# serycjon/MFT

Measured on AMD Instinct MI355X. Metric: tracked frames/sec at 512x512, 12 RAFT iters; flow EPE vs reference, higher is better.
Workload: dtype f32 (update-block products as split fp16 x 3 on the fp16 matrix cores, fp32 accumulation; error per product <= ~2^-23, see DESIGN.md section 4 and parity below); 1 GPU; MFT.track on synthetic 512x512 video, deltas [inf,1,2,4,8,16,32], 7/7.00/7 (min/mean/max) flow pairs per timed frame, 12 RAFT iters, seeded synthetic weights (BASELINE.json configs[1]); parallelism=single GPU, frames_resident_in_hbm=True, preroll_frames=32

## Files before the change

### include/mftx.h

```cpp
#ifndef MFTX_H
#define MFTX_H

#include <stddef.h>
#include <stdint.h>

#ifdef __cplusplus
extern "C" {
#endif

#define MFTX_VERSION 400

#define MFTX_E_ARG (-1)
#define MFTX_E_ALIGN (-2)
#define MFTX_E_WORKSPACE (-3)
#define MFTX_E_STATE (-4)

#define MFTX_MAX_CANDIDATES 16

int mftx_version(void);
const char *mftx_last_error_string(void);

#define MFTX_PROFILE_CATEGORIES 14
int mftx_profile_begin(void);
int mftx_profile_end(double *ms, double *work, long long *count, int n);
// ... 27 lines not shown
typedef struct mftx_conv_desc {
    const float *a0; int lda0; int c0;
    const float *a1; int lda1; int c1;
    const float *wpk; const float *bias;
    float *out; int ldo;
    int P, h, w;
    int N;
    int kh, kw;
    int act;
    float out_scale;
    const float *addend; int ld_addend;
    int stride, hin, win, pad_y, pad_x, residual_mode;
    int arith;
    int a_split, out_split;
} mftx_conv_desc;
#define MFTX_ARITH_F32 0
#define MFTX_ARITH_SPLIT 1
int mftx_conv2d(const mftx_conv_desc *d, void *stream);
int mftx_conv2d_tile(const mftx_conv_desc *d, int tile, void *stream);

int mftx_pack_tile_conv_weights(const float *wpk, int N, int taps, int cin, int cin_pad, void *wtile, void *stream);
int mftx_tile_conv2d(const mftx_conv_desc *d, const void *wtile, void *stream);
#define MFTX_OU_HEADS_WTILE_BYTES 6635520
int mftx_pack_ou_heads_weights(const float *w1pk, int cin_pad, const float *w2pk, void *wtile, void *wproj, void *stream);
int mftx_ou_heads(const float *a_split, int lda, int P, int h, int w, const void *wtile, const float *b1, const void *wproj, const float *b2,
                  float *T, float *out, int ld_out, void *stream);
int mftx_gru_half(const float *h_in, int ld_hin, const float *motion, int ld_mo, const void *wzr, const void *wq, const float *pre_zr,
                  const float *pre_q, float *z, const float *hf_in, float *hf_out, float *h_out, int ld_hout, int P, int h, int w, int pass,
                  void *stream);
int mftx_tile_conv_fills_chip(int P, int h, int w);
#define MFTX_FLOW_HEAD_WEIGHT_BYTES 32768
int mftx_pack_flow_head_weights(const float *w2pk, void *wproj, void *stream);
int mftx_flow_head(const float *hsplit, int ld_h, int P, int h, int w, const void *wtile, const float *b1, const void *wproj,
                   const float *b2, float *T, float *delta, float *coords, void *stream);
int mftx_split_weights(const float *wpk, void *out, long long n_floats, void *stream);
#define MFTX_SPLIT_LIMIT 65504.0f
int mftx_count_not_below(const float *x, long long n, float limit, unsigned *count, void *stream);

typedef struct mftx_raft mftx_raft;
#define MFTX_RAFT_NUM_WEIGHTS 34
int mftx_raft_create(const float *const *weights, int n_weights, mftx_raft **out);
void mftx_raft_destroy(mftx_raft *r);
size_t mftx_raft_workspace_bytes(int P, int h, int w);
int mftx_raft_set_ondemand(mftx_raft *r, int on);
int mftx_raft_set_split_weights(mftx_raft *r, const void *const *split, int n);
int mftx_raft_arith(const mftx_raft *r);
int mftx_raft_set_lookup_fused(mftx_raft *r, const void *wfused);
int mftx_raft_set_flow_fused(mftx_raft *r, const void *wflow);
int mftx_raft_set_tile_weights(mftx_raft *r, const void *const *tile, int n);
int mftx_raft_set_flow_head(mftx_raft *r, const void *wproj);
int mftx_raft_set_ou_heads(mftx_raft *r, const void *wtile, const void *wproj);
int mftx_raft_set_coords_trace(mftx_raft *r, float *trace);
#define MFTX_RAFT_OPT_FORK 0
#define MFTX_RAFT_OPT_PRESPLIT 1
#define MFTX_RAFT_OPT_GROUP 2
#define MFTX_RAFT_OPT_FUSE_LOOKUP 3
#define MFTX_RAFT_OPT_GRAPH 4
#define MFTX_RAFT_OPT_FUSE_FLOW 5
#define MFTX_RAFT_OPT_TILE_CONV 6
#define MFTX_RAFT_OPT_FUSE_HEAD 7
#define MFTX_RAFT_OPT_TILE_VOLUME 8
#define MFTX_RAFT_OPT_FUSE_GRU 9
#define MFTX_RAFT_OPT_TILE_CELLS 10
#define MFTX_RAFT_OPT_FUSE_OU 11
#define MFTX_RAFT_OPT_TILE_CONV2P 12
int mftx_raft_set_option(mftx_raft *r, int option, int value);
int mftx_raft_set_nonfinite_counter(mftx_raft *r, unsigned *counter);
int mftx_raft_clear_graphs(mftx_raft *r);
int mftx_raft_graph_stats(const mftx_raft *r, unsigned long long *captures, unsigned long long *replays);
size_t mftx_raft_workspace_bytes_for(const mftx_raft *r, int P, int h, int w);
int mftx_raft_workspace_layout(int P, int h, int w, size_t *offsets, int n);
int mftx_raft_workspace_layout_for(const mftx_raft *r, int P, int h, int w, size_t *offsets, int n);
int mftx_raft_refine(mftx_raft *r, int P, int h, int w, int iters,
                     const float *fmap1, const float *fmap2, const float *net, const float *inp,
                     const float *flow_init,
                     int pad_left, int pad_right, int pad_top, int pad_bottom,
                     float *flow, float *occl, float *sigma, float *packed, float *flow_lr,
                     void *workspace, size_t workspace_bytes, void *stream);
int mftx_raft_refine_gather(mftx_raft *r, int P, int h, int w, int iters, const float *const *fmap1,
                            const float *const *fmap2, const float *const *net, const float *const *inp,
                            const float *flow_init, int pad_left, int pad_right, int pad_top, int pad_bottom,
                            float *flow, float *occl, float *sigma, float *packed, float *flow_lr_out,
                            void *workspace, size_t workspace_bytes, void *stream);

typedef struct mftx_encoder mftx_encoder;
int mftx_encoder_create(const float *const *weights, int n_weights, int instance_norm, mftx_encoder **out);
int mftx_encoder_set_split_weights(mftx_encoder *e, const void *const *split, int n);
int mftx_encoder_set_graph(mftx_encoder *e, int on);
void mftx_encoder_destroy(mftx_encoder *e);
size_t mftx_encoder_workspace_bytes(int H0, int W0);
int mftx_encoder_forward(mftx_encoder *e, const uint8_t *img, int H0, int W0, float *out0, float *out1,
                         void *workspace, size_t workspace_bytes, void *stream);

int mftx_convex_upsample(const float *flow_lr, const float *ou, int ld_ou, const float *mask,
                         int P, int h, int w,
                         int pad_left, int pad_right, int pad_top, int pad_bottom,
                         float *flow, float *occl, float *sigma, float *packed, void *stream);

int mftx_chain(const float *flowL, const float *occlL, const float *sigmaL,
               const float *flowR, const float *occlR, const float *sigmaR,
               int H, int W, float *flowO, float *occlO, float *sigmaO, void *stream);

int mftx_warp_backward(const float *flow, const float *img, int C, int H, int W, float *out, void *stream);

int mftx_select(int K, const float *const *flow, const float *const *occl, const float *const *sigma,
                float thr, int H, int W,
                float *flowO, float *occlO, float *sigmaO, int8_t *chosen, void *stream);

int mftx_chain_select(int K,
                      const float *const *flowL, const float *const *occlL, const float *const *sigmaL,
                      const float *const *flowR, const float *const *occlR, const float *const *sigmaR,
                      float thr, int H, int W,
                      float *flowO, float *occlO, float *sigmaO, int8_t *chosen, void *stream);

int mftx_chain_select_packed(int K,
                             const float *const *flowL, const float *const *occlL, const float *const *sigmaL,
                             const float *const *packedR,
                             float thr, int H, int W,
                             float *flowO, float *occlO, float *sigmaO, int8_t *chosen, void *stream);

int mftx_chain_select_multi(int T, const int *K,
                            const float *const *flowL, const float *const *occlL, const float *const *sigmaL,
                            const float *const *packedR,
                            float thr, int H, int W,
                            float *const *flowO, float *const *occlO, float *const *sigmaO, int8_t *const *chosen,
                            void *stream);

int mftx_sample_points(int T, const float *const *flow, const float *const *occl, const float *const *sigma,
                       int H, int W, int N, const int *tmpl, const float *xy,
                       float *table, long long row_stride, int column, void *stream);

size_t mftx_quantize_workspace_bytes(void);
int mftx_quantize_u16(const float *x, long long n, uint16_t *q, float *lohi,
                      void *workspace, size_t workspace_bytes, void *stream);
int mftx_dequantize_u16(const uint16_t *q, long long n, float lo, float hi, float *x, void *stream);

int mftx_copy_bytes(const void *src, void *dst, long long n, void *stream);

int mftx_png_unfilter(uint8_t *rows, int height, int row_bytes, int bpp);

#ifdef __cplusplus
}
#endif
#endif
```

### mft_amd/_lib.py

```python
from __future__ import annotations

import ctypes as C
import os
from pathlib import Path

_HERE = Path(__file__).resolve().parent
LIB_PATH = _HERE / "libmftx.so"

MAX_CANDIDATES = 16
NUM_RAFT_WEIGHTS = 34
LOOKUP_CONVC1_WEIGHT_BYTES = 393216
FLOW_BRANCH_WEIGHT_BYTES = 352256
FLOW_HEAD_WEIGHT_BYTES = 32768
OU_HEADS_WTILE_BYTES = 6635520
SPLIT_LIMIT = 65504.0


class ConvDesc(C.Structure):
    _fields_ = [("a0", C.c_void_p), ("lda0", C.c_int), ("c0", C.c_int),
                ("a1", C.c_void_p), ("lda1", C.c_int), ("c1", C.c_int),
                ("wpk", C.c_void_p), ("bias", C.c_void_p),
                ("out", C.c_void_p), ("ldo", C.c_int),
                ("P", C.c_int), ("h", C.c_int), ("w", C.c_int),
                ("N", C.c_int), ("kh", C.c_int), ("kw", C.c_int),
                ("act", C.c_int), ("out_scale", C.c_float),
                ("addend", C.c_void_p), ("ld_addend", C.c_int),
                ("stride", C.c_int), ("hin", C.c_int), ("win", C.c_int), ("pad_y", C.c_int), ("pad_x", C.c_int),
                ("residual_mode", C.c_int), ("arith", C.c_int), ("a_split", C.c_int), ("out_split", C.c_int)]


_PP = C.POINTER(C.c_void_p)

SIGNATURES = {
    "mftx_version": (C.c_int, []),
    "mftx_last_error_string": (C.c_char_p, []),
    "mftx_profile_begin": (C.c_int, []),
    "mftx_profile_end": (C.c_int, [C.POINTER(C.c_double), C.POINTER(C.c_double), C.POINTER(C.c_longlong), C.c_int]),
    "mftx_corr_pyramid": (C.c_int, [C.c_void_p, C.c_void_p, C.c_int, C.c_int, C.c_int, C.c_int,
                                    C.c_void_p, C.c_void_p, C.c_void_p, C.c_void_p, C.c_void_p]),
    "mftx_corr_pyramid_split": (C.c_int, [C.c_void_p, C.c_void_p, C.c_int, C.c_int, C.c_int, C.c_int,
                                          C.c_void_p, C.c_void_p, C.c_void_p, C.c_void_p, C.c_void_p, C.c_void_p]),
    "mftx_corr_pyramid_layout": (C.c_int, [C.c_int, C.c_int, C.POINTER(C.c_longlong), C.POINTER(C.c_int)]),
    "mftx_corr_lookup": (C.c_int, [C.c_void_p] * 5 + [C.c_int] * 4 + [C.c_void_p, C.c_int, C.c_void_p]),
    "mftx_fmap_pyramid": (C.c_int, [C.c_void_p] + [C.c_int] * 4 + [C.c_void_p] * 4),
    "mftx_corr_lookup_ondemand": (C.c_int, [C.c_void_p] * 6 + [C.c_int] * 5 + [C.c_void_p, C.c_int, C.c_void_p]),
    "mftx_raft_set_ondemand": (C.c_int, [C.c_void_p, C.c_int]),
    "mftx_raft_workspace_bytes_for": (C.c_size_t, [C.c_void_p, C.c_int, C.c_int, C.c_int]),
    "mftx_conv2d": (C.c_int, [C.POINTER(ConvDesc), C.c_void_p]),
    "mftx_conv2d_tile": (C.c_int, [C.POINTER(ConvDesc), C.c_int, C.c_void_p]),
    "mftx_encoder_set_split_weights": (C.c_int, [C.c_void_p, _PP, C.c_int]),
    "mftx_raft_set_split_weights": (C.c_int, [C.c_void_p, _PP, C.c_int]),
    "mftx_raft_arith": (C.c_int, [C.c_void_p]),
    "mftx_raft_set_lookup_fused": (C.c_int, [C.c_void_p, C.c_void_p]),
    "mftx_raft_set_flow_fused": (C.c_int, [C.c_void_p, C.c_void_p]),
    "mftx_raft_set_tile_weights": (C.c_int, [C.c_void_p, _PP, C.c_int]),
    "mftx_raft_set_flow_head": (C.c_int, [C.c_void_p, C.c_void_p]),
    "mftx_raft_set_ou_heads": (C.c_int, [C.c_void_p, C.c_void_p, C.c_void_p]),
    "mftx_pack_ou_heads_weights": (C.c_int, [C.c_void_p, C.c_int, C.c_void_p, C.c_void_p, C.c_void_p, C.c_void_p]),
    "mftx_ou_heads": (C.c_int, [C.c_void_p, C.c_int, C.c_int, C.c_int, C.c_int, C.c_void_p, C.c_void_p, C.c_void_p, C.c_void_p, C.c_void_p,
                                C.c_void_p, C.c_int, C.c_void_p]),
    "mftx_pack_flow_head_weights": (C.c_int, [C.c_void_p, C.c_void_p, C.c_void_p]),
    "mftx_flow_head": (C.c_int, [C.c_void_p, C.c_int, C.c_int, C.c_int, C.c_int] + [C.c_void_p] * 8),
    "mftx_pack_tile_conv_weights": (C.c_int, [C.c_void_p, C.c_int, C.c_int, C.c_int, C.c_int, C.c_void_p, C.c_void_p]),
    "mftx_tile_conv2d": (C.c_int, [C.POINTER(ConvDesc), C.c_void_p, C.c_void_p]),
    "mftx_pack_flow_branch_weights": (C.c_int, [C.c_void_p, C.c_void_p, C.c_void_p, C.c_void_p]),
    "mftx_flow_branch": (C.c_int, [C.c_void_p, C.c_int, C.c_int, C.c_int, C.c_void_p, C.c_void_p, C.c_void_p, C.c_void_p,
                                   C.c_int, C.c_void_p, C.c_int, C.c_void_p]),
    "mftx_raft_set_option": (C.c_int, [C.c_void_p, C.c_int, C.c_int]),
    "mftx_raft_set_coords_trace": (C.c_int, [C.c_void_p, C.c_void_p]),
    "mftx_gru_half": (C.c_int, [C.c_void_p, C.c_int, C.c_void_p, C.c_int, C.c_void_p, C.c_void_p, C.c_void_p, C.c_void_p, C.c_void_p, C.c_void_p,
                                C.c_void_p, C.c_void_p, C.c_int, C.c_int, C.c_int, C.c_int, C.c_int, C.c_void_p]),
    "mftx_tile_conv_fills_chip": (C.c_int, [C.c_int, C.c_int, C.c_int]),
    "mftx_raft_clear_graphs": (C.c_int, [C.c_void_p]),
    "mftx_raft_set_nonfinite_counter": (C.c_int, [C.c_void_p, C.c_void_p]),
    "mftx_raft_graph_stats": (C.c_int, [C.c_void_p, C.POINTER(C.c_ulonglong), C.POINTER(C.c_ulonglong)]),
    "mftx_pack_lookup_convc1_weights": (C.c_int, [C.c_void_p, C.c_int, C.c_void_p, C.c_void_p]),
    "mftx_corr_lookup_convc1": (C.c_int, [C.c_void_p] * 5 + [C.c_int] * 3 + [C.c_void_p, C.c_void_p, C.c_void_p,
                                                                            C.c_int, C.c_int, C.c_void_p]),
    "mftx_split_weights": (C.c_int, [C.c_void_p, C.c_void_p, C.c_longlong, C.c_void_p]),
    "mftx_count_not_below": (C.c_int, [C.c_void_p, C.c_longlong, C.c_float, C.c_void_p, C.c_void_p]),
    "mftx_raft_create": (C.c_int, [_PP, C.c_int, C.POINTER(C.c_void_p)]),
    "mftx_raft_destroy": (None, [C.c_void_p]),
    "mftx_raft_workspace_bytes": (C.c_size_t, [C.c_int, C.c_int, C.c_int]),
    "mftx_raft_workspace_layout": (C.c_int, [C.c_int, C.c_int, C.c_int, C.POINTER(C.c_size_t), C.c_int]),
    "mftx_raft_workspace_layout_for": (C.c_int, [C.c_void_p, C.c_int, C.c_int, C.c_int, C.POINTER(C.c_size_t), C.c_int]),
    "mftx_raft_refine": (C.c_int, [C.c_void_p, C.c_int, C.c_int, C.c_int, C.c_int,
                                   C.c_void_p, C.c_void_p, C.c_void_p, C.c_void_p, C.c_void_p,
                                   C.c_int, C.c_int, C.c_int, C.c_int,
                                   C.c_void_p, C.c_void_p, C.c_void_p, C.c_void_p, C.c_void_p,
                                   C.c_void_p, C.c_size_t, C.c_void_p]),
    "mftx_raft_refine_gather": (C.c_int, [C.c_void_p, C.c_int, C.c_int, C.c_int, C.c_int,
                                          _PP, _PP, _PP, _PP, C.c_void_p,
                                          C.c_int, C.c_int, C.c_int, C.c_int,
                                          C.c_void_p, C.c_void_p, C.c_void_p, C.c_void_p, C.c_void_p,
                                          C.c_void_p, C.c_size_t, C.c_void_p]),
    "mftx_encoder_create": (C.c_int, [_PP, C.c_int, C.c_int, C.POINTER(C.c_void_p)]),
    "mftx_encoder_destroy": (None, [C.c_void_p]),
    "mftx_encoder_set_graph": (C.c_int, [C.c_void_p, C.c_int]),
    "mftx_encoder_workspace_bytes": (C.c_size_t, [C.c_int, C.c_int]),
    "mftx_encoder_forward": (C.c_int, [C.c_void_p, C.c_void_p, C.c_int, C.c_int, C.c_void_p, C.c_void_p,
                                       C.c_void_p, C.c_size_t, C.c_void_p]),
    "mftx_convex_upsample": (C.c_int, [C.c_void_p, C.c_void_p, C.c_int, C.c_void_p] + [C.c_int] * 7
                             + [C.c_void_p] * 5),
    "mftx_chain": (C.c_int, [C.c_void_p] * 6 + [C.c_int, C.c_int] + [C.c_void_p] * 4),
    "mftx_warp_backward": (C.c_int, [C.c_void_p, C.c_void_p, C.c_int, C.c_int, C.c_int, C.c_void_p, C.c_void_p]),
    "mftx_select": (C.c_int, [C.c_int, _PP, _PP, _PP, C.c_float, C.c_int, C.c_int] + [C.c_void_p] * 5),
    "mftx_chain_select": (C.c_int, [C.c_int] + [_PP] * 6 + [C.c_float, C.c_int, C.c_int] + [C.c_void_p] * 5),
    "mftx_chain_select_packed": (C.c_int, [C.c_int] + [_PP] * 4 + [C.c_float, C.c_int, C.c_int] + [C.c_void_p] * 5),
    "mftx_chain_select_multi": (C.c_int, [C.c_int, C.POINTER(C.c_int)] + [_PP] * 4 + [C.c_float, C.c_int, C.c_int] + [_PP] * 4
                                + [C.c_void_p]),
    "mftx_sample_points": (C.c_int, [C.c_int, _PP, _PP, _PP, C.c_int, C.c_int, C.c_int, C.c_void_p, C.c_void_p,
                                     C.c_void_p, C.c_longlong, C.c_int, C.c_void_p]),
    "mftx_quantize_workspace_bytes": (C.c_size_t, []),
    "mftx_quantize_u16": (C.c_int, [C.c_void_p, C.c_longlong, C.c_void_p, C.c_void_p, C.c_void_p, C.c_size_t, C.c_void_p]),
    "mftx_dequantize_u16": (C.c_int, [C.c_void_p, C.c_longlong, C.c_float, C.c_float, C.c_void_p, C.c_void_p]),
    "mftx_png_unfilter": (C.c_int, [C.c_void_p, C.c_int, C.c_int, C.c_int]),
    "mftx_copy_bytes": (C.c_int, [C.c_void_p, C.c_void_p, C.c_longlong, C.c_void_p]),
}

_lib = None


class MftxError(RuntimeError):
    pass


def load():
    global _lib
    if _lib is not None:
        return _lib
    path = Path(os.environ.get("MFTX_LIB", LIB_PATH))
    if not path.exists():
        raise MftxError(f"{path} not found: build it with `python -c 'import __graft_entry__ as g; g.build()'` "
                        "(there is no CPU fallback for the MFT hot path)")
    lib = C.CDLL(str(path))
    for name, (res, args) in SIGNATURES.items():
        fn = getattr(lib, name)
        fn.restype = res
        fn.argtypes = args
    _lib = lib
    return lib


def check(code, what):
    if code != 0:
        msg = load().mftx_last_error_string().decode(errors="replace")
        raise MftxError(f"{what} failed ({code}): {msg}")


def ptr_array(ptrs):
    arr = (C.c_void_p * len(ptrs))(*ptrs)
    return C.cast(arr, _PP), arr
```

### mft_amd/csrc/common.h

```cpp
#pragma once
#include <hip/hip_runtime.h>
#include <cstdarg>
#include <cstdio>
#include <cstdint>
#include <cstdlib>
#include "../../include/mftx.h"

namespace mftx {

void set_error(const char *fmt, ...);

inline int fail(int code, const char *fmt, ...) {
    char buf[512];
    va_list ap;
    va_start(ap, fmt);
    vsnprintf(buf, sizeof buf, fmt, ap);
    va_end(ap);
    set_error("%s", buf);
    return code;
}

inline int check_launch(const char *what) {
    hipError_t e = hipGetLastError();
    if (e != hipSuccess) {
// ... 9 lines not shown
    return e ? atoi(e) : dflt;
#else
    (void)name;
    return dflt;
#endif
}

inline bool aligned16(const void *p) { return (reinterpret_cast<uintptr_t>(p) & 15u) == 0; }
inline int cdiv(int a, int b) { return (a + b - 1) / b; }
inline int round_up(int a, int b) { return cdiv(a, b) * b; }

struct PyramidLayout {
    int h[4], w[4];
    int hb[2], wb[2];
    int sbh, sbw;
    long long stride[4];
};
inline PyramidLayout pyramid_layout(int h, int w) {
    PyramidLayout L;
    for (int l = 0; l < 4; ++l) { L.h[l] = h >> l; L.w[l] = w >> l; }
    L.sbh = (h + 7) / 8; L.sbw = (w + 15) / 16;
    L.hb[0] = 2 * L.sbh; L.wb[0] = 2 * L.sbw; L.hb[1] = L.sbh; L.wb[1] = L.sbw;
    L.stride[0] = (long long)L.hb[0] * L.wb[0] * 32;
    L.stride[1] = (long long)L.hb[1] * L.wb[1] * 32;
    L.stride[2] = ((long long)L.h[2] * L.w[2] + 3) / 4 * 4;
    L.stride[3] = ((long long)L.h[3] * L.w[3] + 3) / 4 * 4;
    return L;
}

__host__ __device__ inline int split_row_offset(int c) { return (c >> 3) * 32 + (c & 7) * 2; }
#ifdef __HIPCC__
__device__ __forceinline__ unsigned split_halves(float v) {
    const _Float16 h = (_Float16)v;
    const _Float16 l = (_Float16)((v - (float)h) * 2048.f);
    return (unsigned)__builtin_bit_cast(unsigned short, h) | ((unsigned)__builtin_bit_cast(unsigned short, l) << 16);
}
__device__ __forceinline__ void store_split_pairwise(float *row, int c, float v, bool store) {
    const unsigned mine = split_halves(v);
    const unsigned other = (unsigned)__shfl_xor((int)mine, 1);
    const bool odd = (c & 1) != 0;
    const unsigned word = odd ? ((other >> 16) | (mine & 0xffff0000u)) : ((mine & 0xffffu) | (other << 16));
    char *dst = reinterpret_cast<char *>(row) + split_row_offset(c & ~1) + (odd ? 16 : 0);
    if (store) *reinterpret_cast<unsigned *>(dst) = word;
}
__device__ __forceinline__ float4 load_split4(const float *row, int c) {
    const char *src = reinterpret_cast<const char *>(row) + split_row_offset(c);
    const uint2 h = *reinterpret_cast<const uint2 *>(src), l = *reinterpret_cast<const uint2 *>(src + 16);
    auto dec = [](unsigned hh, unsigned ll, int hi) {
        const _Float16 a = __builtin_bit_cast(_Float16, (unsigned short)(hi ? hh >> 16 : hh));
        const _Float16 b = __builtin_bit_cast(_Float16, (unsigned short)(hi ? ll >> 16 : ll));
        return (float)a + (float)b * (1.f / 2048.f);
    };
    return make_float4(dec(h.x, l.x, 0), dec(h.x, l.x, 1), dec(h.y, l.y, 0), dec(h.y, l.y, 1));
}
__device__ __forceinline__ void store_split4v(float *row, int c, float4 v) {
    const unsigned a = split_halves(v.x), b = split_halves(v.y), cc = split_halves(v.z), d = split_halves(v.w);
    char *dst = reinterpret_cast<char *>(row) + split_row_offset(c);
    *reinterpret_cast<uint2 *>(dst) = make_uint2((a & 0xffffu) | (b << 16), (cc & 0xffffu) | (d << 16));
    *reinterpret_cast<uint2 *>(dst + 16) = make_uint2((a >> 16) | (b & 0xffff0000u), (cc >> 16) | (d & 0xffff0000u));
}
#endif
__host__ __device__ inline float relu_keep_nan(float v) { return v < 0.f ? 0.f : v; }
int launch_conv(const mftx_conv_desc &d, hipStream_t s, int tile = -1);
int launch_conv_pair(const mftx_conv_desc &a, const mftx_conv_desc &b, hipStream_t s);
struct GruEpilogue {
    int mode;
    float *hx;
    int ld_hx;
    float *z;
    float *rh;
    float *hf = nullptr;
    int ld_hf = 0;
};
int launch_conv_gru(const mftx_conv_desc &d, const GruEpilogue &g, hipStream_t s);
int launch_split_weights(const float *wpk, void *out, long long n_floats, hipStream_t s);
bool conv_small_applicable(const mftx_conv_desc &d);
int launch_conv_small(const mftx_conv_desc &d, hipStream_t s, float *accum = nullptr, int ld_accum = 0);
int launch_corr_pyramid(const float *f1, const float *f2, int P, int C, int h, int w, float *const lvl[4], hipStream_t s,
                        float *f2_split = nullptr, int tile_resident = 1);
bool volume_tile_applicable(int C);
constexpr int MFTX_MAX_GATHER = 16;
struct PairPtrs { const float *p[MFTX_MAX_GATHER]; };
int launch_volume_tile(const float *f1, const float *f2s, int P, int h, int w, float *const lvl[4], hipStream_t s,
                       const PairPtrs *f1p = nullptr, long long f2_bstride = -1);
int launch_corr_lookup(const float *const lvl[4], const float *coords, int P, int h, int w,
                       float *out, int ld_out, hipStream_t s);
int launch_pack_lookup_convc1(const float *w, int ld_w, void *out, hipStream_t s);
bool lookup_convc1_applicable(int P, int h, int w, int ld_out);
int launch_lookup_convc1(const float *const lvl[4], const float *coords, int P, int h, int w, const void *wf,
                         const float *bias, float *out, int ld_out, int out_split, hipStream_t s);
int launch_pack_flow_branch(const float *w98, const float *w2pk, void *out, hipStream_t s);
int launch_flow_branch(const float *coords, int P, int h, int w, const void *wf, const float *b1, const float *b2, float *out,
                       int ld_out, float *hx, int ld_hx, hipStream_t s, const float *T = nullptr, const float *b2h = nullptr,
                       float *coords_out = nullptr, float *delta_out = nullptr);
struct TileConvLaunch {
    const float *a0; int lda0;
    const float *a1; int lda1;
    int cin;
    const void *wf;
    const float *bias;
    const float *addend; int ld_addend;
    float *out; int ldo; int out_split;
    float *z, *rh, *hf, *hx; int ld_hf, ld_hx;
    const void *wproj; float *tout;
    int P, h, w, N, kh, kw, epi;
    int cells;
};
struct GruHalfLaunch {
    const float *h_in; int ld_hin; const float *mo; int ld_mo;
    const void *wzr, *wq;
    const float *pre_zr, *pre_q;
    float *z; const float *hf_in; float *hf_out;
    float *h_out; int ld_hout;
    int P, h, w, pass;
    int cells;
};
int launch_gru_half(const GruHalfLaunch &d, hipStream_t s);
int launch_pack_flow_head(const float *w2pk, void *out, hipStream_t s);
int launch_pack_tile_conv2p(const float *wpk, int N, int cin_pad, void *out, hipStream_t s);
int launch_tile_conv2p(const float *a, int lda, const void *wf, const float *bias, float *out, int ldo, int n_valid, int P, int h, int w, int cells,
                       hipStream_t s);
constexpr size_t OU_HEAD_WTILE_BYTES = 8ull * 5 * 9 * 9 * 128 * 16, OU_HEAD_WPROJ_BYTES = 32768;
int launch_pack_ou_head(const float *w1pk, int cin_pad, const float *w2pk, void *wtile, void *wproj, hipStream_t s);
struct OuGather { const float *hx, *corr; int ld_corr; const float *coords1, *delta; float *flow_lr; };
int launch_ou_heads(const float *a, int lda, int P, int h, int w, const void *wtile, const float *b1, const void *wproj, const float *b2, float *T,
                    float *out, int ld_out, int cells, hipStream_t s, const OuGather *ga = nullptr);
int launch_flow_head_sum(const float *T, const float *b2, float *delta, const float *coords_in, float *coords_out, int P, int h, int w, hipStream_t s);
bool tile_conv_applicable(int kh, int kw, int cin, int N);
bool tile_conv_small_tiles_fill(int P, int h, int w);
bool tile_conv_fills_chip(int P, int h, int w, int kh, int kw);
int launch_pack_tile_conv(const float *wpk, int N, int taps, int cin, int cin_pad, void *out, hipStream_t s);
int launch_tile_conv(const TileConvLaunch &d, hipStream_t s);
int launch_fmap_pyramid(const float *f2, int P, int C, int h, int w, float *const lvl[3], hipStream_t s);
int launch_corr_ondemand(const float *f1, const float *const f2lvl[4], const float *coords, int P, int h, int w,
                         float *out, int ld_out, hipStream_t s);
int launch_convex_upsample(const float *flow_lr, const float *ou, int ld_ou, const float *mask,
                           int P, int h, int w, int pl, int pr, int pt, int pb,
                           float *flow, float *occl, float *sigma, float *packed, hipStream_t s, unsigned *nonfinite = nullptr);

}
```

### mft_amd/csrc/raft_engine.hip

```cpp
#include "common.h"
#include "profile.h"
#include "motion_front.h"
#include "graph_cache.h"
#include <cstdlib>
#include <new>

namespace mftx {


struct InitGather { int on; PairPtrs netp, inpp; };
__global__ void init_state_kernel(const float *__restrict__ net, const float *__restrict__ inp,
                                  const float *__restrict__ flow_init, float *hx, float *hf, float *coords1, int M, int h,
                                  int w, InitGather ga) {
    const long long i = (long long)blockIdx.x * blockDim.x + threadIdx.x;
    if (i >= (long long)M * 64) return;
    const int m = (int)(i >> 6), q = (int)(i & 63);
    if (ga.on) {
        const int b = m / (h * w);
        net = ga.netp.p[b] - (long long)b * h * w * 128;
        inp = ga.inpp.p[b] - (long long)b * h * w * 128;
    }
    const float4 v = (q < 32) ? reinterpret_cast<const float4 *>(net)[(long long)m * 32 + q]
                              : reinterpret_cast<const float4 *>(inp)[(long long)m * 32 + (q - 32)];
    if (hf != nullptr) {
        store_split4v(hx + (long long)m * 384, 4 * q, v);
        if (q < 32) reinterpret_cast<float4 *>(hf + (long long)m * 128)[q] = v;
    } else {
        reinterpret_cast<float4 *>(hx + (long long)m * 384)[q] = v;
    }
    if (q == 0) {
        const int rem = m % (h * w);
        float cx = (float)(rem % w), cy = (float)(rem / w);
        if (flow_init != nullptr) {
            cx += flow_init[2 * (long long)m];
            cy += flow_init[2 * (long long)m + 1];
        }
        coords1[2 * (long long)m] = cx;
        coords1[2 * (long long)m + 1] = cy;
    }
}

__global__ __launch_bounds__(256) void convf1_kernel(ConvF1Args q) {
    __shared__ __attribute__((aligned(16))) float patch[2][7][48];
    const int half = threadIdx.x >> 7;
    convf1_strip(q, blockIdx.x * 2 + half, patch[half], threadIdx.x & 127);
}

__global__ __launch_bounds__(256) void lookup_convf1_kernel(LookupArgs lp, ConvF1Args q, int lookup_blocks, int f1_blocks) {
    __shared__ __attribute__((aligned(16))) float patch[2][7][48];
    const int total = lookup_blocks + f1_blocks;
    const int b = blockIdx.x;
    const int f_lo = (int)((long long)b * f1_blocks / total), f_hi = (int)((long long)(b + 1) * f1_blocks / total);
    if (f_hi > f_lo) {
        const int half = threadIdx.x >> 7;
        convf1_strip(q, f_lo * 2 + half, patch[half], threadIdx.x & 127);
    } else {
        lookup_block_body<2>(lp, b - f_lo, lookup_blocks);
    }
}

__global__ void ou_gather_kernel(const float *__restrict__ hx, const float *__restrict__ corr, int ld_corr,
                                 const float *__restrict__ coords1, const float *__restrict__ delta,
                                 float *__restrict__ ouin, float *__restrict__ flow_lr, int M, int h, int w, int split) {
    const long long i = (long long)blockIdx.x * blockDim.x + threadIdx.x;
    if (i >= (long long)M * 178) return;
    const int m = (int)(i / 178), q = (int)(i - (long long)m * 178);
    float4 v;
    if (split) {
        if (q < 64) v = load_split4(hx + (long long)m * 384, 4 * q);
        else if (q < 145) v = reinterpret_cast<const float4 *>(corr + (long long)m * ld_corr)[q - 64];
        else if (q == 145) {
            const int rem = m % (h * w);
            const float fx = coords1[2 * (long long)m] - (float)(rem % w);
            const float fy = coords1[2 * (long long)m + 1] - (float)(rem / w);
            v = make_float4(fx, fy, delta[2 * (long long)m], delta[2 * (long long)m + 1]);
            flow_lr[2 * (long long)m] = fx;
            flow_lr[2 * (long long)m + 1] = fy;
        } else v = load_split4(hx + (long long)m * 384 + 256, 4 * (q - 146));
        store_split4v(ouin + (long long)m * 712, 4 * q, v);
        return;
    }
    if (q < 64) v = reinterpret_cast<const float4 *>(hx + (long long)m * 384)[q];
    else if (q < 145) v = reinterpret_cast<const float4 *>(corr + (long long)m * ld_corr)[q - 64];
    else if (q == 145) {
        const int rem = m % (h * w);
        const float fx = coords1[2 * (long long)m] - (float)(rem % w);
        const float fy = coords1[2 * (long long)m + 1] - (float)(rem / w);
        v = make_float4(fx, fy, delta[2 * (long long)m], delta[2 * (long long)m + 1]);
        flow_lr[2 * (long long)m] = fx;
        flow_lr[2 * (long long)m + 1] = fy;
    } else v = reinterpret_cast<const float4 *>(hx + (long long)m * 384 + 256)[q - 146];
    reinterpret_cast<float4 *>(ouin + (long long)m * 712)[q] = v;
}

enum WeightSlot {
    W_CONVC1, B_CONVC1, W_CONVC2, B_CONVC2, W_CONVF1, B_CONVF1, W_CONVF2, B_CONVF2, W_CONV, B_CONV,
    W_ZR1_DYN, W_ZR1_INP, B_ZR1, W_Q1_DYN, W_Q1_INP, B_Q1, W_ZR2_DYN, W_ZR2_INP, B_ZR2, W_Q2_DYN, W_Q2_INP, B_Q2,
    W_FH1, B_FH1, W_FH2, B_FH2, W_MASK0, B_MASK0, W_MASK2, B_MASK2,
    W_OU1, B_OU1, W_OU2, B_OU2, W_COUNT
};

struct Workspace {
    float *lvl[4];
    float *f2l[3];
    float *coords1, *corr, *cor1, *corflo, *flo1, *hx, *z, *rh, *fh, *delta, *mask, *ouin, *ouh, *ou, *flow_lr;
    float *pre_zr[2], *pre_q[2];
    float *f2s;
    float *hf;
    float *hb, *hfb;
    int ld_corr;
    size_t bytes;
};

static Workspace carve(void *base, int P, int h, int w, bool ondemand = false, bool split = false) {
    Workspace ws{};
    const size_t N = (size_t)h * w, M = (size_t)P * N;
    size_t off = 0;
    auto take = [&](size_t floats) {
        float *p = base ? reinterpret_cast<float *>(static_cast<char *>(base) + off) : nullptr;
        off += (floats * sizeof(float) + 255) & ~size_t(255);
        return p;
    };
    const PyramidLayout L = pyramid_layout(h, w);
    for (int l = 0; l < 4; ++l) ws.lvl[l] = take(ondemand ? 0 : M * (size_t)L.stride[l]);
    for (int l = 1; l < 4; ++l) ws.f2l[l - 1] = take(ondemand ? (size_t)P * (h >> l) * (w >> l) * 256 : 0);
    ws.coords1 = take(M * 2);
    ws.ld_corr = 324;
    ws.corr = take(M * ws.ld_corr);
    ws.cor1 = take(M * 256);
    ws.corflo = take(M * 256);
    ws.flo1 = take(M * 128);
    ws.hx = take(M * 384);
    ws.z = take(M * 128);
    ws.rh = take(M * 128);
    ws.fh = take(M * 256);
    ws.delta = take(M * 2);
    ws.mask = take(M * 576);
    ws.ouin = take(M * 712);
    ws.ouh = take(M * 256);
    ws.ou = take(M * 4);
    ws.flow_lr = take(M * 2);
    for (int pass = 0; pass < 2; ++pass) { ws.pre_zr[pass] = take(M * 256); ws.pre_q[pass] = take(M * 128); }
    ws.f2s = take(ondemand || !split ? 0 : M * 256);
    ws.hf = take(split ? M * 128 : 0);
    ws.hb = take(split ? M * 128 : 0);
    ws.hfb = take(split ? M * 128 : 0);
    ws.bytes = off;
    return ws;
}

}

using namespace mftx;

struct mftx_raft {
    uint32_t magic;
    int ondemand;
    int arith;
    const float *w[W_COUNT];
    const float *wg[W_COUNT];
    hipStream_t side;
    hipEvent_t ev_fork, ev_join;
    float *coords_trace;
    GraphCache *graphs;
    const void *wfused;
    const void *wflow;
    const void *wproj;
    const void *wt[W_COUNT];
    const void *wou, *wouproj;
    int opt[13];
    unsigned *nonfinite;
};
static constexpr int GEMM_SLOTS[] = {W_CONVC1, W_CONVC2, W_CONVF2, W_CONV, W_ZR1_DYN, W_ZR1_INP, W_Q1_DYN, W_Q1_INP,
                                     W_ZR2_DYN, W_ZR2_INP, W_Q2_DYN, W_Q2_INP, W_FH1, W_MASK0, W_MASK2, W_OU1};
static constexpr uint32_t RAFT_MAGIC = 0x4d465458;

extern "C" int mftx_raft_create(const float *const *weights, int n_weights, mftx_raft **out) {
    if (!weights || !out) return fail(MFTX_E_ARG, "raft_create: null pointer");
    if (n_weights != W_COUNT) return fail(MFTX_E_ARG, "raft_create: expected %d weight tensors, got %d", (int)W_COUNT, n_weights);
    for (int i = 0; i < W_COUNT; ++i) {
        if (!weights[i]) return fail(MFTX_E_ARG, "raft_create: weight %d is null", i);
        if (!aligned16(weights[i])) return fail(MFTX_E_ALIGN, "raft_create: weight %d not 16-byte aligned", i);
    }
    mftx_raft *r = new (std::nothrow) mftx_raft;
    if (!r) return fail(MFTX_E_ARG, "raft_create: out of host memory");
    r->magic = RAFT_MAGIC;
    r->ondemand = 0;
    r->arith = MFTX_ARITH_F32;
    r->side = nullptr; r->ev_fork = nullptr; r->ev_join = nullptr;
    r->wfused = nullptr;
    r->wflow = nullptr;
    r->wproj = nullptr;
    r->wou = nullptr; r->wouproj = nullptr;
    for (int i = 0; i < W_COUNT; ++i) r->wt[i] = nullptr;
    r->coords_trace = nullptr;
    r->nonfinite = nullptr;
    r->graphs = new (std::nothrow) GraphCache;
    r->opt[MFTX_RAFT_OPT_FORK] = -1; r->opt[MFTX_RAFT_OPT_PRESPLIT] = 1; r->opt[MFTX_RAFT_OPT_GROUP] = 1; r->opt[MFTX_RAFT_OPT_FUSE_LOOKUP] = 1; r->opt[MFTX_RAFT_OPT_GRAPH] = 1; r->opt[MFTX_RAFT_OPT_FUSE_FLOW] = 1; r->opt[MFTX_RAFT_OPT_TILE_CONV] = 1; r->opt[MFTX_RAFT_OPT_FUSE_HEAD] = 1; r->opt[MFTX_RAFT_OPT_TILE_VOLUME] = 1; r->opt[MFTX_RAFT_OPT_FUSE_GRU] = 1; r->opt[MFTX_RAFT_OPT_TILE_CELLS] = 0; r->opt[MFTX_RAFT_OPT_FUSE_OU] = 1; r->opt[MFTX_RAFT_OPT_TILE_CONV2P] = 1;
    for (int i = 0; i < W_COUNT; ++i) r->w[i] = r->wg[i] = weights[i];
    *out = r;
    return 0;
}

extern "C" void mftx_raft_destroy(mftx_raft *r) {
    if (r && r->magic == RAFT_MAGIC) {
        r->magic = 0;
        if (r->ev_fork) (void)hipEventDestroy(r->ev_fork);
        if (r->ev_join) (void)hipEventDestroy(r->ev_join);
        if (r->side) (void)hipStreamDestroy(r->side);
        delete r->graphs;
        delete r;
    }
}

static int ensure_side_stream(mftx_raft *r) {
    if (r->side) return 0;
    hipError_t e = hipStreamCreateWithFlags(&r->side, hipStreamNonBlocking);
    if (e == hipSuccess) e = hipEventCreateWithFlags(&r->ev_fork, hipEventDisableTiming);
    if (e == hipSuccess) e = hipEventCreateWithFlags(&r->ev_join, hipEventDisableTiming);
    if (e != hipSuccess) return fail((int)e, "raft_refine: side stream: %s", hipGetErrorString(e));
    return 0;
}

extern "C" size_t mftx_raft_workspace_bytes(int P, int h, int w) {
    if (P <= 0 || h <= 0 || w <= 0) return 0;
    return carve(nullptr, P, h, w).bytes;
}

extern "C" int mftx_raft_set_ondemand(mftx_raft *r, int on) {
// ... 52 lines not shown
    if (!r || r->magic != RAFT_MAGIC) return fail(MFTX_E_STATE, "raft_set_flow_head: bad handle");
    if (wproj && !aligned16(wproj)) return fail(MFTX_E_ALIGN, "raft_set_flow_head: weights not 16-byte aligned");
    r->wproj = wproj;
    if (r->graphs) r->graphs->clear();
    return 0;
}

extern "C" int mftx_raft_set_ou_heads(mftx_raft *r, const void *wtile, const void *wproj) {
    if (!r || r->magic != RAFT_MAGIC) return fail(MFTX_E_STATE, "raft_set_ou_heads: bad handle");
    if ((wtile == nullptr) != (wproj == nullptr)) return fail(MFTX_E_ARG, "raft_set_ou_heads: both weight streams, or neither");
    if (wtile && (!aligned16(wtile) || !aligned16(wproj))) return fail(MFTX_E_ALIGN, "raft_set_ou_heads: weights not 16-byte aligned");
    r->wou = wtile; r->wouproj = wproj;
    if (r->graphs) r->graphs->clear();
    return 0;
}

extern "C" int mftx_raft_set_coords_trace(mftx_raft *r, float *trace) {
    if (!r || r->magic != RAFT_MAGIC) return fail(MFTX_E_STATE, "raft_set_coords_trace: bad handle");
    r->coords_trace = trace;
    return 0;
}

extern "C" int mftx_raft_clear_graphs(mftx_raft *r) {
    if (!r || r->magic != RAFT_MAGIC) return fail(MFTX_E_STATE, "raft_clear_graphs: bad handle");
    if (r->graphs) r->graphs->clear();
    return 0;
}

extern "C" int mftx_raft_set_nonfinite_counter(mftx_raft *r, unsigned *counter) {
    if (!r || r->magic != RAFT_MAGIC) return fail(MFTX_E_STATE, "raft_set_nonfinite_counter: bad handle");
    if (counter && (reinterpret_cast<uintptr_t>(counter) & 3)) return fail(MFTX_E_ALIGN, "raft_set_nonfinite_counter: counter not 4-byte aligned");
    r->nonfinite = counter;
    return 0;
}

extern "C" int mftx_raft_set_option(mftx_raft *r, int option, int value) {
    if (!r || r->magic != RAFT_MAGIC) return fail(MFTX_E_STATE, "raft_set_option: bad handle");
    if (option < 0 || option > MFTX_RAFT_OPT_TILE_CONV2P) return fail(MFTX_E_ARG, "raft_set_option: unknown option %d", option);
    r->opt[option] = value;
    if (r->graphs) r->graphs->clear();
    return 0;
}

extern "C" int mftx_raft_arith(const mftx_raft *r) {
    return (r && r->magic == RAFT_MAGIC) ? r->arith : -1;
}

extern "C" size_t mftx_raft_workspace_bytes_for(const mftx_raft *r, int P, int h, int w) {
    if (!r || r->magic != RAFT_MAGIC || P <= 0 || h <= 0 || w <= 0) return 0;
    return carve(nullptr, P, h, w, r->ondemand != 0, r->arith == MFTX_ARITH_SPLIT).bytes;
}

static int workspace_layout(const mftx_raft *r, int P, int h, int w, size_t *offsets, int n) {
    if (P <= 0 || h <= 0 || w <= 0 || !offsets || n != 19) return fail(MFTX_E_ARG, "workspace_layout: need 19 slots");
    char *base = reinterpret_cast<char *>(uintptr_t(1) << 40);
    Workspace ws = carve(base, P, h, w, r && r->ondemand != 0, r && r->arith == MFTX_ARITH_SPLIT);
    float *ptrs[19] = {ws.lvl[0], ws.lvl[1], ws.lvl[2], ws.lvl[3], ws.coords1, ws.corr, ws.cor1, ws.corflo, ws.flo1,
                       ws.hx, ws.z, ws.rh, ws.fh, ws.delta, ws.mask, ws.ouin, ws.ouh, ws.ou, ws.flow_lr};
    for (int i = 0; i < 19; ++i) offsets[i] = (size_t)(reinterpret_cast<char *>(ptrs[i]) - base);
    return 0;
}
extern "C" int mftx_raft_workspace_layout(int P, int h, int w, size_t *offsets, int n) {
    return workspace_layout(nullptr, P, h, w, offsets, n);
}
extern "C" int mftx_raft_workspace_layout_for(const mftx_raft *r, int P, int h, int w, size_t *offsets, int n) {
    if (!r || r->magic != RAFT_MAGIC) return fail(MFTX_E_STATE, "workspace_layout_for: bad handle");
    return workspace_layout(r, P, h, w, offsets, n);
}

#define TRY(expr) do { int _e = (expr); if (_e) return _e; } while (0)

static mftx_conv_desc conv_desc(const float *a0, int lda0, int c0, const float *a1, int lda1, int c1,
                                const float *w, const float *b, float *out, int ldo, int P, int h, int wd, int N,
                                int kh, int kw, int act, float scale = 1.f, const float *addend = nullptr,
                                int ld_addend = 0) {
    mftx_conv_desc d{};
    d.addend = addend; d.ld_addend = ld_addend;
    d.a0 = a0; d.lda0 = lda0; d.c0 = c0; d.a1 = a1; d.lda1 = lda1; d.c1 = c1;
    d.wpk = w; d.bias = b; d.out = out; d.ldo = ldo; d.P = P; d.h = h; d.w = wd; d.N = N;
    d.kh = kh; d.kw = kw; d.act = act; d.out_scale = scale;
    return d;
}

struct RefineGather { PairPtrs f1, f2, net, inp; bool f2_shared; };
static int refine_impl(mftx_raft *r, int P, int h, int w, int iters, const float *fmap1,
                                const float *fmap2, const float *net, const float *inp, const float *flow_init,
                                int pad_left,
                                int pad_right, int pad_top, int pad_bottom, float *flow, float *occl,
                                float *sigma, float *packed, float *flow_lr_out, void *workspace,
                                size_t workspace_bytes, void *stream, const RefineGather *gather) {
    if (!r || r->magic != RAFT_MAGIC) return fail(MFTX_E_STATE, "raft_refine: bad handle");
    const bool planar = flow && occl && sigma;
    if (gather) { fmap1 = gather->f1.p[0]; fmap2 = gather->f2.p[0]; net = gather->net.p[0]; inp = gather->inp.p[0]; }
    if (!fmap1 || !fmap2 || !net || !inp || !workspace || (!planar && (flow || occl || sigma || !packed)))
        return fail(MFTX_E_ARG, "raft_refine: null pointer (outputs: flow + occl + sigma, or packed, or both)");
    if (P <= 0 || h < 16 || w < 16 || iters < 1)
        return fail(MFTX_E_ARG, "raft_refine: need P >= 1, h, w >= 16 (level 3 of the pyramid needs >= 2 cells), iters >= 1");
    if ((long long)P * h * w > (1ll << 24)) return fail(MFTX_E_ARG, "raft_refine: batch too large");
    if (!aligned16(fmap1) || !aligned16(fmap2) || !aligned16(net) || !aligned16(inp) ||
        (reinterpret_cast<uintptr_t>(workspace) & 255))
        return fail(MFTX_E_ALIGN, "raft_refine: inputs must be 16-byte and the workspace 256-byte aligned");
    if (pad_left < 0 || pad_right < 0 || pad_top < 0 || pad_bottom < 0 || pad_left + pad_right >= 8 ||
        pad_top + pad_bottom >= 8)
        return fail(MFTX_E_ARG, "raft_refine: bad padding");
    const bool ondemand = r->ondemand != 0;
    const bool SP = r->arith == MFTX_ARITH_SPLIT && r->opt[MFTX_RAFT_OPT_PRESPLIT] != 0;
    const bool fuse_lookup = SP && !ondemand && r->wfused != nullptr && r->opt[MFTX_RAFT_OPT_FUSE_LOOKUP] != 0 &&
                             lookup_convc1_applicable(P, h, w, 256);
    Workspace ws = carve(workspace, P, h, w, ondemand, r->arith == MFTX_ARITH_SPLIT);
    if (ws.bytes > workspace_bytes)
        return fail(MFTX_E_WORKSPACE, "raft_refine: workspace %zu < %zu bytes", workspace_bytes, ws.bytes);
    hipStream_t s = (hipStream_t)stream;
    const bool use_graph = r->graphs && r->opt[MFTX_RAFT_OPT_GRAPH] != 0 && !prof_enabled() && !r->coords_trace && !ondemand;
    hipStream_t caller = s;
    bool proxied = false;
    if (use_graph && s == nullptr) {
        hipStream_t own = r->graphs->proxy.enter(s);
        if (own) { s = own; proxied = true; }
    }
    struct Leave { GraphCache *g; hipStream_t caller; bool on; ~Leave() { if (on) g->proxy.leave(caller); } } leave{r->graphs, caller, proxied};
    const int N = h * w, M = P * N;
    const float *const *W = r->w;
    const float *const *G = r->wg;
    const int AR = r->arith;
    auto gemm = [AR, SP](mftx_conv_desc d, bool a = true, bool o = false) { d.arith = AR; d.a_split = SP && a; d.out_split = SP && o; return d; };

    const float *f2lv[4] = {fmap2, ws.f2l[0], ws.f2l[1], ws.f2l[2]};
    if (ondemand) TRY(launch_fmap_pyramid(fmap2, P, 256, h, w, ws.f2l, s));
    else if (gather) {
        const long long pair_floats = (long long)N * 256;
        if (gather->f2_shared) TRY(launch_split_weights(gather->f2.p[0], ws.f2s, pair_floats, s));
        else for (int b = 0; b < P; ++b) TRY(launch_split_weights(gather->f2.p[b], ws.f2s + b * pair_floats, pair_floats, s));
        TRY(launch_volume_tile(nullptr, ws.f2s, P, h, w, ws.lvl, s, &gather->f1, gather->f2_shared ? 0 : pair_floats));
    }
    else TRY(launch_corr_pyramid(fmap1, fmap2, P, 256, h, w, ws.lvl, s, r->arith == MFTX_ARITH_SPLIT ? ws.f2s : nullptr, r->opt[MFTX_RAFT_OPT_TILE_VOLUME]));
    {
        const long long slots = (long long)M * 64;
        ProfScope prof(PC_GLUE, s, 0);
        InitGather ga{};
        if (gather) { ga.on = 1; ga.netp = gather->net; ga.inpp = gather->inp; }
        hipLaunchKernelGGL(init_state_kernel, dim3((unsigned)((slots + 255) / 256)), dim3(256), 0, s, net, inp,
                           flow_init, ws.hx, SP ? ws.hf : nullptr, ws.coords1, M, h, w, ga);
        TRY(check_launch("init_state"));
    }
    float *flow_lr = flow_lr_out ? flow_lr_out : ws.flow_lr;
    auto core = [&]() -> int {
    const bool tiles_on = SP && r->opt[MFTX_RAFT_OPT_TILE_CONV] != 0 &&
                          (r->opt[MFTX_RAFT_OPT_TILE_CONV] == 2 ||
                           (tile_conv_fills_chip(P, h, w, 3, 3) && tile_conv_fills_chip(P, h, w, 1, 5) && tile_conv_fills_chip(P, h, w, 5, 1)));
    auto tile_w = [&](int slot) -> const void * { return tiles_on ? r->wt[slot] : nullptr; };
    auto tile_layer = [&](const float *a0, int lda0, const float *a1, int lda1, const void *wf, const float *bias, int N, int kh, int kw, int epi) {
        TileConvLaunch t{};
        t.a0 = a0; t.lda0 = lda0; t.a1 = a1; t.lda1 = lda1; t.cin = a1 ? 256 : 128; t.wf = wf; t.bias = bias;
        t.P = P; t.h = h; t.w = w; t.N = N; t.kh = kh; t.kw = kw; t.epi = epi;
        t.cells = r->opt[MFTX_RAFT_OPT_TILE_CELLS];
        return t;
    };
    for (int pass = 0; pass < 2; ++pass) {
        const int kh = pass ? 5 : 1, kw = pass ? 1 : 5;
        const int szr = pass ? W_ZR2_INP : W_ZR1_INP, sq = pass ? W_Q2_INP : W_Q1_INP;
        if (tile_w(szr)) {
            TileConvLaunch t = tile_layer(ws.hx + 128, 384, nullptr, 0, tile_w(szr), W[pass ? B_ZR2 : B_ZR1], 256, kh, kw, 0);
            t.out = ws.pre_zr[pass]; t.ldo = 256;
            TRY(launch_tile_conv(t, s));
        } else TRY(launch_conv(gemm(conv_desc(ws.hx + 128, 384, 128, nullptr, 0, 0, G[szr], W[pass ? B_ZR2 : B_ZR1], ws.pre_zr[pass], 256, P, h, w, 256, kh, kw, 0), true, false), s));
        if (tile_w(sq)) {
            TileConvLaunch t = tile_layer(ws.hx + 128, 384, nullptr, 0, tile_w(sq), W[pass ? B_Q2 : B_Q1], 128, kh, kw, 0);
            t.out = ws.pre_q[pass]; t.ldo = 128;
            TRY(launch_tile_conv(t, s));
        } else TRY(launch_conv(gemm(conv_desc(ws.hx + 128, 384, 128, nullptr, 0, 0, G[sq], W[pass ? B_Q2 : B_Q1], ws.pre_q[pass], 128, P, h, w, 128, kh, kw, 0), true, false), s));
    }
    const float *lv[4] = {ws.lvl[0], ws.lvl[1], ws.lvl[2], ws.lvl[3]};
    const int strips = cdiv(w, F1_CELLS);
    float *ccur = ws.coords1, *calt = ws.flo1;
    bool pending = false;
    for (int it = 0; it < iters; ++it) {
        const bool last = (it == iters - 1);
        if (r->coords_trace &&
            hipMemcpyAsync(r->coords_trace + (size_t)it * M * 2, ccur, (size_t)M * 8, hipMemcpyDeviceToDevice, s) != hipSuccess)
            return fail(MFTX_E_STATE, "raft_refine: coords trace copy failed");
        const ConvF1Args f1{ccur, W[W_CONVF1], W[B_CONVF1], ws.flo1, ws.hx, h, w, strips, P * h * strips, SP ? 1 : 0};
        const int f1_blocks = cdiv(f1.n_strips, 2);
        const bool nofuse = r->opt[MFTX_RAFT_OPT_GROUP] == 0, nopair = nofuse;
        const mftx_conv_desc c2 = gemm(conv_desc(ws.cor1, 256, 256, nullptr, 0, 0, G[W_CONVC2], W[B_CONVC2], ws.corflo, 256, P, h, w, 192, 3, 3, 1), true, true);
        const mftx_conv_desc f2 = gemm(conv_desc(ws.flo1, 128, 128, nullptr, 0, 0, G[W_CONVF2], W[B_CONVF2], ws.corflo + 192, 256, P, h, w, 64, 3, 3, 1), true, true);
        const int fork_env = r->opt[MFTX_RAFT_OPT_FORK];
        const bool fuse_flow = SP && r->wflow != nullptr && r->opt[MFTX_RAFT_OPT_FUSE_FLOW] != 0 && !nofuse;
        if (fuse_flow) {
            if (pending) {
                TRY(launch_flow_branch(ccur, P, h, w, r->wflow, W[B_CONVF1], W[B_CONVF2], ws.corflo + 192, 256, ws.hx, 384, s, ws.fh, W[B_FH2], calt, ws.delta));
                float *t = ccur; ccur = calt; calt = t;
                pending = false;
            } else TRY(launch_flow_branch(ccur, P, h, w, r->wflow, W[B_CONVF1], W[B_CONVF2], ws.corflo + 192, 256, ws.hx, 384, s));
        }
        const bool serial = fuse_flow || prof_enabled() || nofuse || (AR == MFTX_ARITH_SPLIT && (fork_env == 0 || fork_env == 2));
        const bool forked = !serial && AR == MFTX_ARITH_SPLIT;
        const bool flow_first = !fuse_flow && serial && fuse_lookup && fork_env == 2 && !prof_enabled() && !nofuse;
        if (flow_first) {
            hipLaunchKernelGGL(convf1_kernel, dim3(f1_blocks), dim3(256), 0, s, f1);
            TRY(check_launch("convf1"));
            TRY(launch_conv(f2, s));
        }
        if (forked) {
            TRY(ensure_side_stream(r));
            if (hipEventRecord(r->ev_fork, s) != hipSuccess || hipStreamWaitEvent(r->side, r->ev_fork, 0) != hipSuccess)
                return fail(MFTX_E_STATE, "raft_refine: fork onto the side stream failed");
            hipLaunchKernelGGL(convf1_kernel, dim3(f1_blocks), dim3(256), 0, r->side, f1);
            TRY(check_launch("convf1"));
            TRY(launch_conv(f2, r->side));
            if (fuse_lookup && last) TRY(launch_corr_lookup(lv, ccur, P, h, w, ws.corr, ws.ld_corr, r->side));
            if (hipEventRecord(r->ev_join, r->side) != hipSuccess) return fail(MFTX_E_STATE, "raft_refine: join event failed");
        }
        if (fuse_lookup) {
            if (last && !forked) TRY(launch_corr_lookup(lv, ccur, P, h, w, ws.corr, ws.ld_corr, s));
            TRY(launch_lookup_convc1(lv, ccur, P, h, w, r->wfused, W[B_CONVC1], ws.cor1, 256, 1, s));
            if (!forked && !flow_first && !fuse_flow) {
                ProfScope prof(PC_CONVF1, s, 2.0 * M * 128 * 98);
                hipLaunchKernelGGL(convf1_kernel, dim3(f1_blocks), dim3(256), 0, s, f1);
            }
        } else if (prof_enabled() || nofuse || forked || ondemand || fuse_flow) {
            if (ondemand) TRY(launch_corr_ondemand(fmap1, f2lv, ccur, P, h, w, ws.corr, ws.ld_corr, s));
            else TRY(launch_corr_lookup(lv, ccur, P, h, w, ws.corr, ws.ld_corr, s));
            if (!forked && !fuse_flow) {
                ProfScope prof(PC_CONVF1, s, 2.0 * M * 128 * 98);
                hipLaunchKernelGGL(convf1_kernel, dim3(f1_blocks), dim3(256), 0, s, f1);
            }
        } else {
            const LookupArgs la = make_lookup_args(lv, ccur, P, h, w, ws.corr, ws.ld_corr);
            const int lookup_blocks = cdiv(cdiv(la.cells, 2), LK_WAVES);
            hipLaunchKernelGGL(lookup_convf1_kernel, dim3(lookup_blocks + f1_blocks), dim3(256), 0, s, la, f1,
                               lookup_blocks, f1_blocks);
        }
        TRY(check_launch("lookup + convf1"));
        if (!fuse_lookup) TRY(launch_conv(gemm(conv_desc(ws.corr, ws.ld_corr, ws.ld_corr, nullptr, 0, 0, G[W_CONVC1], W[B_CONVC1], ws.cor1, 256, P, h, w, 256, 1, 1, 1), false, true), s));
        const bool two_pass = tiles_on && r->opt[MFTX_RAFT_OPT_TILE_CONV2P] != 0 && r->wt[W_CONVC2] && r->wt[W_CONV];
        auto run_c2 = [&]() -> int {
            if (two_pass) return launch_tile_conv2p(ws.cor1, 256, r->wt[W_CONVC2], W[B_CONVC2], ws.corflo, 256, 192, P, h, w, r->opt[MFTX_RAFT_OPT_TILE_CELLS], s);
            return launch_conv(c2, s);
        };
        if (forked) {
            TRY(run_c2());
            if (hipStreamWaitEvent(s, r->ev_join, 0) != hipSuccess) return fail(MFTX_E_STATE, "raft_refine: join failed");
        } else if (nopair || AR != MFTX_ARITH_F32) {
            TRY(run_c2());
            if (!flow_first && !fuse_flow) TRY(launch_conv(f2, s));
        } else {
            TRY(launch_conv_pair(c2, f2, s));
        }
        if (two_pass) TRY(launch_tile_conv2p(ws.corflo, 256, r->wt[W_CONV], W[B_CONV], ws.hx + 256, 384, 126, P, h, w, r->opt[MFTX_RAFT_OPT_TILE_CELLS], s));
        else TRY(launch_conv(gemm(conv_desc(ws.corflo, 256, 256, nullptr, 0, 0, G[W_CONV], W[B_CONV], ws.hx + 256, 384, P, h, w, 126, 3, 3, 1), true, true), s));
        const bool gru_fused = tile_w(W_ZR1_DYN) && tile_w(W_Q1_DYN) && tile_w(W_ZR2_DYN) && tile_w(W_Q2_DYN) &&
                               r->opt[MFTX_RAFT_OPT_FUSE_GRU] != 0;
        for (int pass = 0; pass < 2; ++pass) {
            const int kh = pass ? 5 : 1, kw = pass ? 1 : 5;
            const int szr = pass ? W_ZR2_DYN : W_ZR1_DYN, sq = pass ? W_Q2_DYN : W_Q1_DYN;
            if (gru_fused) {
                GruHalfLaunch g{};
                g.h_in = pass ? ws.hb : ws.hx; g.ld_hin = pass ? 128 : 384; g.h_out = pass ? ws.hx : ws.hb; g.ld_hout = pass ? 384 : 128;
                g.mo = ws.hx + 256; g.ld_mo = 384; g.wzr = tile_w(szr); g.wq = tile_w(sq); g.pre_zr = ws.pre_zr[pass]; g.pre_q = ws.pre_q[pass];
                g.z = ws.z; g.hf_in = pass ? ws.hfb : ws.hf; g.hf_out = pass ? ws.hf : ws.hfb; g.P = P; g.h = h; g.w = w; g.pass = pass; g.cells = r->opt[MFTX_RAFT_OPT_TILE_CELLS];
                TRY(launch_gru_half(g, s));
                continue;
            }
            if (tile_w(szr)) {
                TileConvLaunch t = tile_layer(ws.hx, 384, ws.hx + 256, 384, tile_w(szr), nullptr, 256, kh, kw, 2);
                t.addend = ws.pre_zr[pass]; t.ld_addend = 256; t.z = ws.z; t.rh = ws.rh; t.hf = ws.hf; t.ld_hf = 128;
                TRY(launch_tile_conv(t, s));
            } else {
                GruEpilogue g1{1, ws.hx, 384, ws.z, ws.rh, SP ? ws.hf : nullptr, 128};
                TRY(launch_conv_gru(gemm(conv_desc(ws.hx, 384, 128, ws.hx + 256, 384, 128, G[szr], nullptr, ws.z, 128, P, h, w, 256, kh, kw, 2, 1.f, ws.pre_zr[pass], 256), true, true), g1, s));
            }
            if (tile_w(sq)) {
                TileConvLaunch t = tile_layer(ws.rh, 128, ws.hx + 256, 384, tile_w(sq), nullptr, 128, kh, kw, 3);
                t.addend = ws.pre_q[pass]; t.ld_addend = 128; t.z = ws.z; t.hf = ws.hf; t.ld_hf = 128; t.hx = ws.hx; t.ld_hx = 384;
                TRY(launch_tile_conv(t, s));
            } else {
                GruEpilogue g2{2, ws.hx, 384, ws.z, ws.rh, SP ? ws.hf : nullptr, 128};
                TRY(launch_conv_gru(gemm(conv_desc(ws.rh, 128, 128, ws.hx + 256, 384, 128, G[sq], nullptr, ws.hx, 384, P, h, w, 128, kh, kw, 3, 1.f, ws.pre_q[pass], 128), true, true), g2, s));
            }
        }
        const bool head_fused = tile_w(W_FH1) && r->wproj != nullptr && r->opt[MFTX_RAFT_OPT_FUSE_HEAD] != 0;
        if (head_fused) {
            TileConvLaunch t = tile_layer(ws.hx, 384, nullptr, 0, tile_w(W_FH1), W[B_FH1], 256, 3, 3, 4);
            t.wproj = r->wproj; t.tout = ws.fh;
            TRY(launch_tile_conv(t, s));
            const bool defer = !last && fuse_flow && r->opt[MFTX_RAFT_OPT_FUSE_HEAD] != 2 && !r->coords_trace;
            if (defer) pending = true;
            else {
                float *dst = last ? ws.coords1 : ccur;
                TRY(launch_flow_head_sum(ws.fh, W[B_FH2], ws.delta, ccur, dst, P, h, w, s));
                ccur = dst;
            }
        } else if (tile_w(W_FH1)) {
            TileConvLaunch t = tile_layer(ws.hx, 384, nullptr, 0, tile_w(W_FH1), W[B_FH1], 256, 3, 3, 1);
            t.out = ws.fh; t.ldo = 256;
            TRY(launch_tile_conv(t, s));
        } else TRY(launch_conv(gemm(conv_desc(ws.hx, 384, 128, nullptr, 0, 0, G[W_FH1], W[B_FH1], ws.fh, 256, P, h, w, 256, 3, 3, 1), true, false), s));
        if (!head_fused) {
            const mftx_conv_desc fh2 = conv_desc(ws.fh, 256, 256, nullptr, 0, 0, W[W_FH2], W[B_FH2], ws.delta, 2, P, h, w, 2, 3, 3, 0);
            if (!conv_small_applicable(fh2)) return fail(MFTX_E_STATE, "raft_refine: flow-head layer does not fit the small-N kernel");
            TRY(launch_conv_small(fh2, s, ccur, 2));
        }
        if (!last) continue;
        if (r->coords_trace &&
            hipMemcpyAsync(r->coords_trace + (size_t)iters * M * 2, ccur, (size_t)M * 8, hipMemcpyDeviceToDevice, s) != hipSuccess)
            return fail(MFTX_E_STATE, "raft_refine: coords trace copy failed");
        if (tile_w(W_MASK0)) {
            TileConvLaunch t = tile_layer(ws.hx, 384, nullptr, 0, tile_w(W_MASK0), W[B_MASK0], 256, 3, 3, 1);
            t.out = ws.fh; t.ldo = 256; t.out_split = SP ? 1 : 0;
            TRY(launch_tile_conv(t, s));
        } else TRY(launch_conv(gemm(conv_desc(ws.hx, 384, 128, nullptr, 0, 0, G[W_MASK0], W[B_MASK0], ws.fh, 256, P, h, w, 256, 3, 3, 1), true, true), s));
        TRY(launch_conv(gemm(conv_desc(ws.fh, 256, 256, nullptr, 0, 0, G[W_MASK2], W[B_MASK2], ws.mask, 576, P, h, w, 576, 1, 1, 0, 0.25f), true, false), s));
        const bool ou_fused = tiles_on && r->wou != nullptr && r->opt[MFTX_RAFT_OPT_FUSE_OU] != 0;
        if (!ou_fused || r->opt[MFTX_RAFT_OPT_FUSE_OU] == 2) {
            const long long slots = (long long)M * 178;
            ProfScope prof(PC_GLUE, s, 0);
            hipLaunchKernelGGL(ou_gather_kernel, dim3((unsigned)((slots + 255) / 256)), dim3(256), 0, s, ws.hx,
                               ws.corr, ws.ld_corr, ccur, ws.delta, ws.ouin, flow_lr, M, h, w, SP ? 1 : 0);
            TRY(check_launch("ou_gather"));
        }
        if (ou_fused) {
            const OuGather ga{ws.hx, ws.corr, ws.ld_corr, ccur, ws.delta, flow_lr};
            const bool mat = r->opt[MFTX_RAFT_OPT_FUSE_OU] == 2;
            TRY(launch_ou_heads(mat ? ws.ouin : nullptr, 712, P, h, w, r->wou, W[B_OU1], r->wouproj, W[B_OU2], ws.ouh, ws.ou, 4, r->opt[MFTX_RAFT_OPT_TILE_CELLS], s,
                                mat ? nullptr : &ga));
        } else {
            TRY(launch_conv(gemm(conv_desc(ws.ouin, 712, 712, nullptr, 0, 0, G[W_OU1], W[B_OU1], ws.ouh, 256, P, h, w, 256, 3, 3, 1), true, false), s));
            TRY(launch_conv(conv_desc(ws.ouh, 256, 256, nullptr, 0, 0, W[W_OU2], W[B_OU2], ws.ou, 4, P, h, w, 3, 3, 3, 0), s));
        }
    }
    return 0;
    };
    if (use_graph) {
        if (AR == MFTX_ARITH_SPLIT && r->opt[MFTX_RAFT_OPT_FORK] != 0) TRY(ensure_side_stream(r));
        GraphKey key{};
        key.v[0] = (uintptr_t)P; key.v[1] = (uintptr_t)h; key.v[2] = (uintptr_t)w; key.v[3] = (uintptr_t)iters;
        key.v[4] = reinterpret_cast<uintptr_t>(workspace); key.v[5] = reinterpret_cast<uintptr_t>(flow_lr_out);
        key.v[6] = (uintptr_t)AR; key.v[7] = reinterpret_cast<uintptr_t>(r->wfused); key.v[8] = reinterpret_cast<uintptr_t>(s);
        key.v[9] = reinterpret_cast<uintptr_t>(r->wflow); key.v[10] = reinterpret_cast<uintptr_t>(r->wt[W_ZR1_DYN]); key.v[11] = reinterpret_cast<uintptr_t>(r->wproj);
        key.v[12] = reinterpret_cast<uintptr_t>(r->wou);
        TRY(r->graphs->run(key, s, core));
    } else {
        TRY(core());
    }
    return launch_convex_upsample(flow_lr, ws.ou, 4, ws.mask, P, h, w, pad_left, pad_right, pad_top, pad_bottom,
                                  flow, occl, sigma, packed, s, r->nonfinite);
}

extern "C" int mftx_raft_refine(mftx_raft *r, int P, int h, int w, int iters, const float *fmap1,
                                const float *fmap2, const float *net, const float *inp, const float *flow_init,
                                int pad_left, int pad_right, int pad_top, int pad_bottom, float *flow, float *occl,
                                float *sigma, float *packed, float *flow_lr_out, void *workspace,
                                size_t workspace_bytes, void *stream) {
    return refine_impl(r, P, h, w, iters, fmap1, fmap2, net, inp, flow_init, pad_left, pad_right, pad_top, pad_bottom, flow, occl, sigma,
                       packed, flow_lr_out, workspace, workspace_bytes, stream, nullptr);
}

extern "C" int mftx_raft_refine_gather(mftx_raft *r, int P, int h, int w, int iters, const float *const *fmap1,
                                       const float *const *fmap2, const float *const *net, const float *const *inp,
                                       const float *flow_init, int pad_left, int pad_right, int pad_top, int pad_bottom,
                                       float *flow, float *occl, float *sigma, float *packed, float *flow_lr_out,
                                       void *workspace, size_t workspace_bytes, void *stream) {
    if (!r || r->magic != RAFT_MAGIC) return fail(MFTX_E_STATE, "raft_refine_gather: bad handle");
    if (!fmap1 || !fmap2 || !net || !inp) return fail(MFTX_E_ARG, "raft_refine_gather: null pointer");
    if (P < 1 || P > MFTX_MAX_GATHER) return fail(MFTX_E_ARG, "raft_refine_gather: 1 .. %d pairs", MFTX_MAX_GATHER);
    if (r->arith != MFTX_ARITH_SPLIT || r->ondemand || r->opt[MFTX_RAFT_OPT_TILE_VOLUME] == 0)
        return fail(MFTX_E_STATE, "raft_refine_gather: needs the split arithmetic with the stored, tile-resident correlation volume (use mftx_raft_refine)");
    RefineGather g{};
    g.f2_shared = true;
    for (int b = 0; b < P; ++b) {
        if (!fmap1[b] || !fmap2[b] || !net[b] || !inp[b]) return fail(MFTX_E_ARG, "raft_refine_gather: pair %d has a null map", b);
        if (!aligned16(fmap1[b]) || !aligned16(fmap2[b]) || !aligned16(net[b]) || !aligned16(inp[b])) return fail(MFTX_E_ALIGN, "raft_refine_gather: maps must be 16-byte aligned");
        g.f1.p[b] = fmap1[b]; g.f2.p[b] = fmap2[b]; g.net.p[b] = net[b]; g.inp.p[b] = inp[b];
        if (fmap2[b] != fmap2[0]) g.f2_shared = false;
    }
    return refine_impl(r, P, h, w, iters, nullptr, nullptr, nullptr, nullptr, flow_init, pad_left, pad_right, pad_top, pad_bottom, flow, occl,
                       sigma, packed, flow_lr_out, workspace, workspace_bytes, stream, &g);
}

extern "C" int mftx_raft_graph_stats(const mftx_raft *r, unsigned long long *captures, unsigned long long *replays) {
    if (!r || r->magic != RAFT_MAGIC || !captures || !replays) return fail(MFTX_E_STATE, "raft_graph_stats: bad arguments");
    *captures = r->graphs ? r->graphs->captures : 0;
    *replays = r->graphs ? r->graphs->replays : 0;
    return 0;
}

extern "C" int mftx_corr_pyramid(const float *f1, const float *f2, int P, int C, int h, int w, float *lvl0,
                                 float *lvl1, float *lvl2, float *lvl3, void *stream) {
    if (!f1 || !f2 || !lvl0 || !lvl1 || !lvl2 || !lvl3) return fail(MFTX_E_ARG, "corr_pyramid: null pointer");
    if (P <= 0 || C <= 0 || C % 32 || h < 8 || w < 8) return fail(MFTX_E_ARG, "corr_pyramid: need C %% 32 == 0, h, w >= 8");
    if (!aligned16(f1) || !aligned16(f2)) return fail(MFTX_E_ALIGN, "corr_pyramid: features must be 16-byte aligned");
    if (!aligned16(lvl0) || !aligned16(lvl1) || !aligned16(lvl2) || !aligned16(lvl3))
        return fail(MFTX_E_ALIGN, "corr_pyramid: levels must be 16-byte aligned");
    float *const lv[4] = {lvl0, lvl1, lvl2, lvl3};
    return launch_corr_pyramid(f1, f2, P, C, h, w, lv, (hipStream_t)stream);
}

extern "C" int mftx_corr_pyramid_split(const float *f1, const float *f2, int P, int C, int h, int w, float *lvl0,
                                       float *lvl1, float *lvl2, float *lvl3, float *f2_scratch, void *stream) {
    if (!f1 || !f2 || !lvl0 || !lvl1 || !lvl2 || !lvl3 || !f2_scratch) return fail(MFTX_E_ARG, "corr_pyramid_split: null pointer");
    if (P <= 0 || C <= 0 || C % 32 || h < 8 || w < 8) return fail(MFTX_E_ARG, "corr_pyramid_split: need C %% 32 == 0, h, w >= 8");
    if (!aligned16(f1) || !aligned16(f2) || (reinterpret_cast<uintptr_t>(f2_scratch) & 31))
        return fail(MFTX_E_ALIGN, "corr_pyramid_split: features must be 16-byte aligned, the scratch 32-byte aligned");
    if (!aligned16(lvl0) || !aligned16(lvl1) || !aligned16(lvl2) || !aligned16(lvl3))
        return fail(MFTX_E_ALIGN, "corr_pyramid_split: levels must be 16-byte aligned");
    float *const lv[4] = {lvl0, lvl1, lvl2, lvl3};
    return launch_corr_pyramid(f1, f2, P, C, h, w, lv, (hipStream_t)stream, f2_scratch);
}

extern "C" int mftx_corr_pyramid_layout(int h, int w, long long *stride, int *block_grid) {
    if (h < 8 || w < 8 || !stride || !block_grid) return fail(MFTX_E_ARG, "corr_pyramid_layout: bad arguments");
    const PyramidLayout L = pyramid_layout(h, w);
    for (int l = 0; l < 4; ++l) stride[l] = L.stride[l];
    block_grid[0] = L.hb[0]; block_grid[1] = L.wb[0]; block_grid[2] = L.hb[1]; block_grid[3] = L.wb[1];
    return 0;
}

extern "C" int mftx_corr_lookup(const float *lvl0, const float *lvl1, const float *lvl2, const float *lvl3,
                                const float *coords, int P, int h, int w, int r, float *out, int ld_out,
                                void *stream) {
    if (!lvl0 || !lvl1 || !lvl2 || !lvl3 || !coords || !out) return fail(MFTX_E_ARG, "corr_lookup: null pointer");
    if (r != 4) return fail(MFTX_E_ARG, "corr_lookup: only radius 4 (RAFT basic) is built");
    if (P <= 0 || h < 8 || w < 8 || ld_out < 324) return fail(MFTX_E_ARG, "corr_lookup: bad sizes");
    if (!aligned16(lvl0) || !aligned16(lvl1)) return fail(MFTX_E_ALIGN, "corr_lookup: levels 0 and 1 must be 16-byte aligned");
    const float *lv[4] = {lvl0, lvl1, lvl2, lvl3};
    return launch_corr_lookup(lv, coords, P, h, w, out, ld_out, (hipStream_t)stream);
}

extern "C" int mftx_pack_lookup_convc1_weights(const float *wpk, int ld_w, void *wfused, void *stream) {
    if (!wpk || !wfused) return fail(MFTX_E_ARG, "pack_lookup_convc1_weights: null pointer");
    if (ld_w < 324) return fail(MFTX_E_ARG, "pack_lookup_convc1_weights: need ld_w >= 324");
    if (!aligned16(wfused)) return fail(MFTX_E_ALIGN, "pack_lookup_convc1_weights: output must be 16-byte aligned");
    return launch_pack_lookup_convc1(wpk, ld_w, wfused, (hipStream_t)stream);
}

extern "C" int mftx_corr_lookup_convc1(const float *lvl0, const float *lvl1, const float *lvl2, const float *lvl3,
                                       const float *coords, int P, int h, int w, const void *wfused, const float *bias,
                                       float *out, int ld_out, int out_split, void *stream) {
    if (!lvl0 || !lvl1 || !lvl2 || !lvl3 || !coords || !wfused || !bias || !out) return fail(MFTX_E_ARG, "corr_lookup_convc1: null pointer");
    if (P <= 0 || h < 8 || w < 8 || ld_out < 256 || ld_out % 4) return fail(MFTX_E_ARG, "corr_lookup_convc1: bad sizes");
    if (!lookup_convc1_applicable(P, h, w, ld_out)) return fail(MFTX_E_ARG, "corr_lookup_convc1: batch too large");
    if (!aligned16(wfused) || !aligned16(bias) || !aligned16(out) || !aligned16(coords) ||
        (out_split && (ld_out % 8 || (reinterpret_cast<uintptr_t>(out) & 31))))
        return fail(MFTX_E_ALIGN, "corr_lookup_convc1: operands must be 16-byte aligned (a split-form output: 32-byte rows)");
    const float *lv[4] = {lvl0, lvl1, lvl2, lvl3};
    return launch_lookup_convc1(lv, coords, P, h, w, wfused, bias, out, ld_out, out_split ? 1 : 0, (hipStream_t)stream);
}

extern "C" int mftx_pack_tile_conv_weights(const float *wpk, int N, int taps, int cin, int cin_pad, void *wtile, void *stream) {
    if (taps == 9 && cin == 256) return launch_pack_tile_conv2p(wpk, N, cin_pad, wtile, (hipStream_t)stream);
    return launch_pack_tile_conv(wpk, N, taps, cin, cin_pad, wtile, (hipStream_t)stream);
}

extern "C" int mftx_tile_conv2d(const mftx_conv_desc *d, const void *wtile, void *stream) {
    if (!d || !wtile) return fail(MFTX_E_ARG, "tile_conv2d: null pointer");
    if (d->arith != MFTX_ARITH_SPLIT || !d->a_split) return fail(MFTX_E_ARG, "tile_conv2d: split arithmetic with a split-form input only");
    if (d->act != 0 && d->act != 1) return fail(MFTX_E_ARG, "tile_conv2d: activation none or relu");
    if (d->stride > 1 || d->residual_mode != 0 || d->out_scale != 1.f || (d->hin && d->hin != d->h) || (d->win && d->win != d->w) || d->pad_y != 0 || d->pad_x != 0)
        return fail(MFTX_E_ARG, "tile_conv2d: stride 1, same padding, no output scale");
    if (d->kh == 3 && d->kw == 3 && d->c0 == 256 && d->c1 == 0) {
// ... 108 lines not shown
```

### mft_amd/csrc/tile_conv.hip

```cpp
#include "common.h"
#include "profile.h"

namespace mftx {

typedef float tc_f32x16 __attribute__((ext_vector_type(16)));
typedef float tc_f32x4 __attribute__((ext_vector_type(4)));
typedef unsigned tc_u32x4 __attribute__((ext_vector_type(4)));
typedef _Float16 tc_f16x8 __attribute__((ext_vector_type(8)));

enum TcEpi { TC_LINEAR = 0, TC_RELU = 1, TC_GRU_ZR = 2, TC_GRU_Q = 3,
             TC_RELU_PROJ = 4 };

#ifdef MFTX_LF_TRACE
__device__ unsigned long long tc_trace_buf[8][16];
#define TC_T(code) do { if (blockIdx.x == 0 && tcount < 16) { unsigned long long t_; asm volatile("s_memtime %0\n\ts_waitcnt lgkmcnt(0)" : "=s"(t_) :: "memory"); \
                        if ((threadIdx.x & 63) == 0) tc_trace_buf[threadIdx.x >> 6][tcount] = ((unsigned long long)(code) << 56) | (t_ & 0x00ffffffffffffffull); ++tcount; } } while (0)
__device__ unsigned long long tc_clock_buf[4096][4];
#define TC_CLK(slot) do { if (wv == ((slot) ? 7 : 0) && blockIdx.x < 4096) { unsigned long long t_, r_; \
                          asm volatile("s_waitcnt vmcnt(0) lgkmcnt(0)\n\ts_memtime %0\n\ts_memrealtime %1\n\ts_waitcnt lgkmcnt(0)" : "=s"(t_), "=s"(r_) :: "memory"); \
                          if (lane == 0) { tc_clock_buf[blockIdx.x][slot] = t_; tc_clock_buf[blockIdx.x][2 + slot] = r_; } } } while (0)
#else
#define TC_T(code) do { } while (0)
#define TC_CLK(slot) do { } while (0)
#endif
// ... 260 lines not shown
    }

    constexpr int GPC = N / 8, ITEMS = G::CELLS * GPC;
#pragma unroll
    for (int it = 0; it < ITEMS / 512; ++it) {
        const int item = tid + 512 * it, m = item / GPC, n0 = (item % GPC) * 8;
        const int yy = y0 + m / TW, xx = x0 + m % TW;
        const float *src = red + m * G::RED_ROW + n0;
        tc_f32x4 u = *reinterpret_cast<const tc_f32x4 *>(src), v = *reinterpret_cast<const tc_f32x4 *>(src + 4);
        if constexpr (G::KS == 2) {
            u += *reinterpret_cast<const tc_f32x4 *>(src + G::CELLS * G::RED_ROW);
            v += *reinterpret_cast<const tc_f32x4 *>(src + G::CELLS * G::RED_ROW + 4);
        }
        if (yy >= p.h || xx >= p.w) continue;
        const long long cell = img_base + (long long)yy * p.w + xx;
        if (p.bias) {
            u += *reinterpret_cast<const tc_f32x4 *>(p.bias + n0);
            v += *reinterpret_cast<const tc_f32x4 *>(p.bias + n0 + 4);
        }
        if (p.addend) {
            u += *reinterpret_cast<const tc_f32x4 *>(p.addend + cell * p.ld_addend + n0);
            v += *reinterpret_cast<const tc_f32x4 *>(p.addend + cell * p.ld_addend + n0 + 4);
        }
        auto store_split = [&](float *row, int c0) {
            tc_u32x4 hi, lo;
            tc_split8(u, v, k2048, hi, lo);
            uint4 *dst = reinterpret_cast<uint4 *>(reinterpret_cast<char *>(row) + (c0 >> 3) * 32);
            dst[0] = __builtin_bit_cast(uint4, hi);
            dst[1] = __builtin_bit_cast(uint4, lo);
        };
        if constexpr (EPI == TC_GRU_ZR) {
#pragma unroll
            for (int e = 0; e < 4; ++e) { u[e] = tc_sigmoid(u[e]); v[e] = tc_sigmoid(v[e]); }
            if (n0 < 128) {
                *reinterpret_cast<tc_f32x4 *>(p.z + cell * 128 + n0) = u;
                *reinterpret_cast<tc_f32x4 *>(p.z + cell * 128 + n0 + 4) = v;
            } else {
                u *= *reinterpret_cast<const tc_f32x4 *>(p.hf + cell * p.ld_hf + n0 - 128);
                v *= *reinterpret_cast<const tc_f32x4 *>(p.hf + cell * p.ld_hf + n0 - 128 + 4);
                store_split(p.rh + cell * 128, n0 - 128);
            }
        } else if constexpr (EPI == TC_GRU_Q) {
            const tc_f32x4 z0 = *reinterpret_cast<const tc_f32x4 *>(p.z + cell * 128 + n0), z1 = *reinterpret_cast<const tc_f32x4 *>(p.z + cell * 128 + n0 + 4);
            float *hrow = p.hf + cell * p.ld_hf + n0;
            const tc_f32x4 h0 = *reinterpret_cast<const tc_f32x4 *>(hrow), h1 = *reinterpret_cast<const tc_f32x4 *>(hrow + 4);
#pragma unroll
            for (int e = 0; e < 4; ++e) { u[e] = tc_blend(z0[e], h0[e], tc_tanh(u[e])); v[e] = tc_blend(z1[e], h1[e], tc_tanh(v[e])); }
            *reinterpret_cast<tc_f32x4 *>(hrow) = u;
            *reinterpret_cast<tc_f32x4 *>(hrow + 4) = v;
            store_split(p.hx + cell * p.ld_hx, n0);
        } else {
            if constexpr (EPI == TC_RELU) {
#pragma unroll
                for (int e = 0; e < 4; ++e) { u[e] = relu_keep_nan(u[e]); v[e] = relu_keep_nan(v[e]); }
            }
            if (p.out_split) store_split(p.out + cell * p.ldo, n0);
            else {
                *reinterpret_cast<tc_f32x4 *>(p.out + cell * p.ldo + n0) = u;
                *reinterpret_cast<tc_f32x4 *>(p.out + cell * p.ldo + n0 + 4) = v;
            }
        }
    }
    TC_T(8);
    TC_CLK(1);
}

#ifdef MFTX_LF_TRACE
extern "C" int mftx_debug_tc_clock(unsigned long long *out, int n_wg) {
    if (n_wg < 0 || n_wg > 4096) return -1;
    return hipMemcpyFromSymbol(out, HIP_SYMBOL(tc_clock_buf), sizeof(unsigned long long) * 4 * n_wg) == hipSuccess ? 0 : -1;
}
extern "C" int mftx_debug_tc_trace(unsigned long long *out) {
    if (hipMemcpyFromSymbol(out, HIP_SYMBOL(tc_trace_buf), sizeof(unsigned long long) * 8 * 16) != hipSuccess) return -1;
    unsigned long long z[8 * 16] = {};
    return hipMemcpyToSymbol(HIP_SYMBOL(tc_trace_buf), z, sizeof z) == hipSuccess ? 0 : -1;
}
#endif

struct GruHalfArgs {
    const float *h_in; int ld_hin;
    const float *mo; int ld_mo;
    const void *wzr, *wq;
    const float *pre_zr, *pre_q;
    float *z;
    const float *hf_in; float *hf_out;
    float *h_out; int ld_hout;
    int P, h, w, tiles_x, tiles_y, step;
};

template <class G, int KW>
__device__ __forceinline__ void tc_kloop(const unsigned char *const (&abase)[G::RT], const uint4 *__restrict__ w2, uint4 (&bq)[3][2],
                                         tc_f32x16 (&acc)[G::RT], tc_f32x16 (&accx)[G::RT]) {
    constexpr int PF = 3;
    tc_f16x8 ah[2][G::RT], al[2][G::RT];
    auto read_a = [&](int s, int set) {
        const int tap = s / G::GPW, gg = s % G::GPW;
        const int off = ((tap / KW) * G::HWD + tap % KW) * G::CELLB + gg * 64 * G::KS;
#pragma unroll
        for (int i = 0; i < G::RT; ++i) {
            ah[set][i] = *reinterpret_cast<const tc_f16x8 *>(abase[i] + off);
            al[set][i] = *reinterpret_cast<const tc_f16x8 *>(abase[i] + off + 16);
        }
    };
    read_a(0, 0);
#pragma unroll
    for (int s = 0; s < G::STEPS; ++s) {
        const int set = s & 1;
        const tc_f16x8 bh = __builtin_bit_cast(tc_f16x8, bq[s % PF][0]), bl = __builtin_bit_cast(tc_f16x8, bq[s % PF][1]);
        __builtin_amdgcn_sched_barrier(0);
        if (s + 1 < G::STEPS) read_a(s + 1, set ^ 1);
        if (s + PF < G::STEPS) { bq[s % PF][0] = w2[(s + PF) * 128]; bq[s % PF][1] = w2[(s + PF) * 128 + 64]; }
        __builtin_amdgcn_sched_barrier(0);
#pragma unroll
        for (int i = 0; i < G::RT; ++i) acc[i] = tc_mfma(bh, ah[set][i], acc[i]);
#pragma unroll
        for (int i = 0; i < G::RT; ++i) accx[i] = tc_mfma(bl, ah[set][i], accx[i]);
#pragma unroll
        for (int i = 0; i < G::RT; ++i) accx[i] = tc_mfma(bh, al[set][i], accx[i]);
        __builtin_amdgcn_sched_barrier(0);
    }
}

template <int TH, int TW, int KH, int KW>
__global__ __launch_bounds__(512, 2) void gru_half_kernel(GruHalfArgs p) {
    using G1 = TcGeom<TH, TW, KH, KW, 256, 256>;
    using G2 = TcGeom<TH, TW, KH, KW, 256, 128>;
    static_assert(G1::CELLB == G2::CELLB && G1::HWD == G2::HWD, "one tile, two GEMMs");
    constexpr int CELLB = G1::CELLB, HWD = G1::HWD, PF = 3, RT = G1::RT, CELLS = G1::CELLS;
    constexpr bool HORIZ = KW > 1;
    extern __shared__ __attribute__((aligned(16))) unsigned char tc_lds[];
    unsigned char *lds = tc_lds;
    const int tid = (int)threadIdx.x, lane = tid & 63, wv = __builtin_amdgcn_readfirstlane(tid >> 6);
    const int tile = (int)blockIdx.x;
    const int tx_ = tile % p.tiles_x, ty_ = (tile / p.tiles_x) % p.tiles_y, img = tile / (p.tiles_x * p.tiles_y);
    const int n_along = HORIZ ? p.tiles_x : p.tiles_y, t_along = HORIZ ? tx_ : ty_, len_along = HORIZ ? p.w : p.h;
    const int r0 = n_along > 1 ? t_along * p.step - 2 : 0;
    const int olo = n_along > 1 ? t_along * p.step : 0, ohi = n_along > 1 ? min(len_along, olo + p.step) : len_along;
    const int x0 = HORIZ ? r0 : tx_ * TW, y0 = HORIZ ? ty_ * TH : r0;
    const long long img_base = (long long)img * p.h * p.w;
    const uint4 *__restrict__ w1 = reinterpret_cast<const uint4 *>(p.wzr) + (long long)((wv ^ 4) * G1::STEPS) * 128 + lane;
    const int nt2 = wv % G2::NT, ks2 = wv / G2::NT;
    const uint4 *__restrict__ w2 = reinterpret_cast<const uint4 *>(p.wq) + (long long)((nt2 * G2::KS + ks2) * G2::STEPS) * 128 + lane;

#ifdef MFTX_LF_TRACE
    int tcount = 0;
#endif
    TC_T(1);
    TC_CLK(0);
    uint4 bq[PF][2];
#pragma unroll
    for (int s = 0; s < PF; ++s) { bq[s][0] = w1[s * 128]; bq[s][1] = w1[s * 128 + 64]; }

    {
        constexpr int PPC = 64, TOTAL = G1::HCELLS * PPC, ROUNDS = (TOTAL + 511) / 512, B = 6;
#pragma unroll 1
        for (int rr = 0; rr < ROUNDS; rr += B) {
            uint4 v[B];
#pragma unroll
            for (int k = 0; k < B; ++k) {
                const int q = (rr + k) * 512 + tid;
                v[k] = make_uint4(0u, 0u, 0u, 0u);
                if (rr + k < ROUNDS && q < TOTAL) {
                    const int c = q / PPC, pc = q - c * PPC;
                    const int cy = c / HWD, cx = c - cy * HWD;
                    const int yy = y0 - KH / 2 + cy, xx = x0 - KW / 2 + cx;
                    if (yy >= 0 && yy < p.h && xx >= 0 && xx < p.w) {
                        const long long cell = img_base + (long long)yy * p.w + xx;
                        const float *src = pc >= 32 ? p.mo + cell * p.ld_mo + (pc - 32) * 4 : p.h_in + cell * p.ld_hin + pc * 4;
                        v[k] = *reinterpret_cast<const uint4 *>(src);
                    }
                }
            }
#pragma unroll
            for (int k = 0; k < B; ++k) {
                const int q = (rr + k) * 512 + tid;
                if (rr + k < ROUNDS && q < TOTAL) {
                    const int c = q / PPC, pc = q - c * PPC;
                    *reinterpret_cast<uint4 *>(lds + c * CELLB + pc * 16) = v[k];
                }
            }
        }
    }
    TC_T(2);
    tc_barrier();
    TC_T(3);

    tc_f32x16 acc[RT], accx[RT];
    const unsigned char *abase[RT];
    auto zero_acc = [&]() {
#pragma unroll
        for (int i = 0; i < RT; ++i)
#pragma unroll
            for (int r = 0; r < 16; ++r) { acc[i][r] = 0.f; accx[i][r] = 0.f; }
    };
    auto set_abase = [&](int ks) {
        const int r = lane & 31;
#pragma unroll
        for (int i = 0; i < RT; ++i) {
            const int m = 32 * i + r;
            abase[i] = lds + ((m / TW) * HWD + (m % TW)) * CELLB + (lane >> 5) * 32 + ks * 64;
        }
    };
    auto slot = [&](int m) { return lds + ((m / TW + KH / 2) * HWD + (m % TW + KW / 2)) * CELLB; };
    const float inv2048 = 1.f / 2048.f;
    const float k2048 = __builtin_bit_cast(float, __builtin_amdgcn_readfirstlane(0x45000000));

    const int nt1 = wv ^ 4;
    zero_acc();
    set_abase(0);
    tc_kloop<G1, KW>(abase, w1, bq, acc, accx);
    TC_T(4);
#pragma unroll
    for (int s = 0; s < PF; ++s) { bq[s][0] = w2[s * 128]; bq[s][1] = w2[s * 128 + 64]; }
    unsigned rh_hi[RT][4][2], rh_lo[RT][4][2];
    if (wv < 4) {
#pragma unroll
        for (int i = 0; i < RT; ++i) {
            const int m = 32 * i + (lane & 31);
            const int yy = y0 + m / TW, xx = x0 + m % TW;
            const bool inside = yy >= 0 && yy < p.h && xx >= 0 && xx < p.w;
            const int yc = yy < 0 ? 0 : (yy >= p.h ? p.h - 1 : yy), xc = xx < 0 ? 0 : (xx >= p.w ? p.w - 1 : xx);
            const long long cell = img_base + (long long)yc * p.w + xc;
            const int n0 = 32 * wv + 4 * (lane >> 5);
            tc_f32x4 a[4], hh[4];
#pragma unroll
            for (int b = 0; b < 4; ++b) {
                a[b] = *reinterpret_cast<const tc_f32x4 *>(p.pre_zr + cell * 256 + 128 + n0 + 8 * b);
                hh[b] = *reinterpret_cast<const tc_f32x4 *>(p.hf_in + cell * 128 + n0 + 8 * b);
            }
#pragma unroll
            for (int b = 0; b < 4; ++b) {
                tc_f32x4 v;
#pragma unroll
                for (int e = 0; e < 4; ++e) v[e] = acc[i][4 * b + e] + accx[i][4 * b + e] * inv2048;
                v += a[b];
#pragma unroll
                for (int e = 0; e < 4; ++e) v[e] = tc_sigmoid(v[e]);
                v *= hh[b];
                tc_split4(v, k2048, rh_hi[i][b], rh_lo[i][b]);
                if (!inside) { rh_hi[i][b][0] = rh_hi[i][b][1] = rh_lo[i][b][0] = rh_lo[i][b][1] = 0u; }
            }
        }
    }
    TC_T(5);
    tc_barrier();
    if (wv < 4) {
#pragma unroll
        for (int i = 0; i < RT; ++i) {
            unsigned char *dst = slot(32 * i + (lane & 31)) + (4 * wv) * 32 + (lane >> 5) * 8;
#pragma unroll
            for (int b = 0; b < 4; ++b) {
                *reinterpret_cast<uint2 *>(dst + 32 * b) = make_uint2(rh_hi[i][b][0], rh_hi[i][b][1]);
                *reinterpret_cast<uint2 *>(dst + 32 * b + 16) = make_uint2(rh_lo[i][b][0], rh_lo[i][b][1]);
            }
        }
    }
    tc_barrier();
    TC_T(6);
    if (wv >= 4) {
#pragma unroll
        for (int i = 0; i < RT; ++i) {
            const int m = 32 * i + (lane & 31);
            const int yy = y0 + m / TW, xx = x0 + m % TW, along = HORIZ ? xx : yy;
            const bool own = yy >= 0 && yy < p.h && xx >= 0 && xx < p.w && along >= olo && along < ohi;
            const long long cell = img_base + (long long)yy * p.w + xx;
            const int n0 = 32 * nt1 + 4 * (lane >> 5);
#pragma unroll
            for (int b = 0; b < 4; ++b) {
                tc_f32x4 v;
#pragma unroll
                for (int e = 0; e < 4; ++e) v[e] = acc[i][4 * b + e] + accx[i][4 * b + e] * inv2048;
                if (own) *reinterpret_cast<tc_f32x4 *>(p.z + cell * 128 + n0 + 8 * b) = v;
            }
        }
    }

    zero_acc();
    set_abase(ks2);
    tc_kloop<G2, KW>(abase, w2, bq, acc, accx);
    TC_T(7);
    asm volatile("s_waitcnt vmcnt(0)" ::: "memory");
    tc_barrier();
    float *red = reinterpret_cast<float *>(lds);
#pragma unroll
    for (int i = 0; i < RT; ++i)
#pragma unroll
        for (int b = 0; b < 4; ++b) {
            tc_f32x4 v;
#pragma unroll
            for (int e = 0; e < 4; ++e) v[e] = acc[i][4 * b + e] + accx[i][4 * b + e] * inv2048;
            *reinterpret_cast<tc_f32x4 *>(red + (ks2 * CELLS + 32 * i + (lane & 31)) * G2::RED_ROW + 32 * nt2 + 8 * b + 4 * (lane >> 5)) = v;
        }
    tc_barrier();
#pragma unroll
    for (int it = 0; it < RT; ++it) {
        const int item = tid + 512 * it, m = item >> 4, n0 = (item & 15) * 8;
        const int yy = y0 + m / TW, xx = x0 + m % TW, along = HORIZ ? xx : yy;
        const float *src = red + m * G2::RED_ROW + n0;
        tc_f32x4 u = *reinterpret_cast<const tc_f32x4 *>(src), v = *reinterpret_cast<const tc_f32x4 *>(src + 4);
        u += *reinterpret_cast<const tc_f32x4 *>(src + CELLS * G2::RED_ROW);
        v += *reinterpret_cast<const tc_f32x4 *>(src + CELLS * G2::RED_ROW + 4);
        if (yy < 0 || yy >= p.h || xx < 0 || xx >= p.w || along < olo || along >= ohi) continue;
        const long long cell = img_base + (long long)yy * p.w + xx;
        u += *reinterpret_cast<const tc_f32x4 *>(p.pre_q + cell * 128 + n0);
        v += *reinterpret_cast<const tc_f32x4 *>(p.pre_q + cell * 128 + n0 + 4);
        tc_f32x4 z0 = *reinterpret_cast<const tc_f32x4 *>(p.z + cell * 128 + n0), z1 = *reinterpret_cast<const tc_f32x4 *>(p.z + cell * 128 + n0 + 4);
        z0 += *reinterpret_cast<const tc_f32x4 *>(p.pre_zr + cell * 256 + n0);
        z1 += *reinterpret_cast<const tc_f32x4 *>(p.pre_zr + cell * 256 + n0 + 4);
#pragma unroll
        for (int e = 0; e < 4; ++e) { z0[e] = tc_sigmoid(z0[e]); z1[e] = tc_sigmoid(z1[e]); }
        const float *hrow = p.hf_in + cell * 128 + n0;
        const tc_f32x4 h0 = *reinterpret_cast<const tc_f32x4 *>(hrow), h1 = *reinterpret_cast<const tc_f32x4 *>(hrow + 4);
#pragma unroll
        for (int e = 0; e < 4; ++e) { u[e] = tc_blend(z0[e], h0[e], tc_tanh(u[e])); v[e] = tc_blend(z1[e], h1[e], tc_tanh(v[e])); }
        *reinterpret_cast<tc_f32x4 *>(p.hf_out + cell * 128 + n0) = u;
        *reinterpret_cast<tc_f32x4 *>(p.hf_out + cell * 128 + n0 + 4) = v;
        tc_u32x4 hi, lo;
        tc_split8(u, v, k2048, hi, lo);
        uint4 *dst = reinterpret_cast<uint4 *>(reinterpret_cast<char *>(p.h_out + cell * p.ld_hout) + (n0 >> 3) * 32);
        dst[0] = __builtin_bit_cast(uint4, hi);
        dst[1] = __builtin_bit_cast(uint4, lo);
    }
    TC_T(8);
    TC_CLK(1);
}

template <int TH, int TW, int KH, int KW>
static int gru_half_launch(GruHalfArgs a, hipStream_t s) {
    using G1 = TcGeom<TH, TW, KH, KW, 256, 256>;
    using G2 = TcGeom<TH, TW, KH, KW, 256, 128>;
    constexpr int lds_bytes = G1::A_BYTES > G2::RED_BYTES ? G1::A_BYTES : G2::RED_BYTES;
    static_assert(lds_bytes <= 160 * 1024, "gru_half: LDS");
    constexpr bool HORIZ = KW > 1;
    const int along = HORIZ ? a.w : a.h, T = HORIZ ? TW : TH;
    a.step = T - 4;
    const int n_along = along <= T ? 1 : cdiv(along, a.step);
    a.tiles_x = HORIZ ? n_along : cdiv(a.w, TW);
    a.tiles_y = HORIZ ? cdiv(a.h, TH) : n_along;
    const long long tiles = (long long)a.P * a.tiles_x * a.tiles_y;
    if (tiles > 0x7fffffffLL) return fail(MFTX_E_ARG, "gru_half: too many tiles");
    auto kern = gru_half_kernel<TH, TW, KH, KW>;
    static bool attr_set = false;
    if (!attr_set) {
        if (hipFuncSetAttribute(reinterpret_cast<const void *>(kern), hipFuncAttributeMaxDynamicSharedMemorySize, lds_bytes) != hipSuccess)
            return fail(MFTX_E_STATE, "gru_half: cannot reserve %d bytes of LDS", lds_bytes);
        attr_set = true;
    }
    ProfScope prof(PC_GRU_FUSED, s, 2.0 * a.P * a.h * a.w * 384.0 * KH * KW * 256);
    hipLaunchKernelGGL(kern, dim3((unsigned)tiles), dim3(512), lds_bytes, s, a);
    return check_launch("gru_half");
}

static int tc_num_cus();
static bool tc_fills(long long tiles);
int tile_conv_cells(int P, int h, int w, int kh);
long long gru_half_tiles(int P, int h, int w, int th, int tw, bool horiz) {
    const int along = horiz ? w : h, T = horiz ? tw : th;
    const int n_along = along <= T ? 1 : cdiv(along, T - 4);
    return (long long)P * (horiz ? n_along * cdiv(h, th) : n_along * cdiv(w, tw));
}

int launch_gru_half(const GruHalfLaunch &d, hipStream_t s) {
    if (!d.h_in || !d.mo || !d.wzr || !d.wq || !d.pre_zr || !d.pre_q || !d.z || !d.hf_in || !d.hf_out || !d.h_out) return fail(MFTX_E_ARG, "gru_half: null pointer");
    if (d.P <= 0 || d.h <= 0 || d.w <= 0 || (d.pass != 0 && d.pass != 1)) return fail(MFTX_E_ARG, "gru_half: bad sizes");
    if (d.h_in == d.h_out || d.hf_in == d.hf_out) return fail(MFTX_E_ARG, "gru_half: h is read from one buffer and written to another");
    auto bad_split = [](const float *p, int ld) { return (reinterpret_cast<uintptr_t>(p) & 31) != 0 || (ld % 8) != 0; };
    if (bad_split(d.h_in, d.ld_hin) || bad_split(d.mo, d.ld_mo) || bad_split(d.h_out, d.ld_hout) || !aligned16(d.wzr) || !aligned16(d.wq) ||
        !aligned16(d.pre_zr) || !aligned16(d.pre_q) || !aligned16(d.z) || !aligned16(d.hf_in) || !aligned16(d.hf_out))
        return fail(MFTX_E_ALIGN, "gru_half: split-form rows are 32-byte aligned with strides in multiples of 8; the rest 16-byte aligned");
    GruHalfArgs a{};
    a.h_in = d.h_in; a.ld_hin = d.ld_hin; a.mo = d.mo; a.ld_mo = d.ld_mo; a.wzr = d.wzr; a.wq = d.wq; a.pre_zr = d.pre_zr; a.pre_q = d.pre_q;
    a.z = d.z; a.hf_in = d.hf_in; a.hf_out = d.hf_out; a.h_out = d.h_out; a.ld_hout = d.ld_hout; a.P = d.P; a.h = d.h; a.w = d.w;
    const bool hz = d.pass == 0;
    auto best = [&](int cells, int &th, int &tw) {
        const int ta = hz ? cells / 64 : 64, tb = hz ? 64 : cells / 64;
        const int sa = hz ? cells / 32 : 32, sb = hz ? 32 : cells / 32;
        const long long nl = cells >= 64 ? gru_half_tiles(d.P, d.h, d.w, ta, tb, hz) : (1ll << 62), ns = gru_half_tiles(d.P, d.h, d.w, sa, sb, hz);
        if (nl <= ns) { th = ta; tw = tb; return nl; }
        th = sa; tw = sb; return ns;
    };
    int th = 0, tw = 0, cells = d.cells;
    if (!cells) {
        cells = 128;
        if (!tc_fills(best(128, th, tw))) cells = 64;
    }
    if (cells != 128 && cells != 64 && cells != 32) return fail(MFTX_E_ARG, "gru_half: 128, 64 or 32 cells per tile");
    if (cells == 32) cells = 64;
    best(cells, th, tw);
#define GH(TH, TW, KH, KW) if (th == TH && tw == TW) return gru_half_launch<TH, TW, KH, KW>(a, s)
    if (hz) { GH(2, 64, 1, 5); GH(4, 32, 1, 5); GH(1, 64, 1, 5); GH(2, 32, 1, 5); }
    else { GH(64, 2, 5, 1); GH(32, 4, 5, 1); GH(64, 1, 5, 1); GH(32, 2, 5, 1); }
#undef GH
    return fail(MFTX_E_STATE, "gru_half: no kernel for tiles of %d x %d cells", th, tw);
}

struct OuHeadArgs {
    const float *a; int lda;
    const float *hx; const float *corr; int ld_corr; const float *coords1; const float *delta; float *flow_lr;
    const void *wf;
    const float *bias;
    const void *wproj; float *tout;
    int P, h, w, tiles_x, tiles_y;
};
constexpr int OU_C = 712, OU_PASSES = 5, OU_CP = 144, OU_PROJ_ROW = 28;

template <int TH, int TW, bool GATHER>
__global__ __launch_bounds__(512, 2) void ou_head_kernel(OuHeadArgs p) {
    using G = TcGeom<TH, TW, 3, 3, OU_CP, 256>;
    constexpr int RT = G::RT, CELLS = G::CELLS, PF = 3;
    extern __shared__ __attribute__((aligned(16))) unsigned char tc_lds[];
    unsigned char *lds = tc_lds;
    const int tid = (int)threadIdx.x, lane = tid & 63, wv = __builtin_amdgcn_readfirstlane(tid >> 6);
    const int tile = (int)blockIdx.x;
    const int tx_ = tile % p.tiles_x, ty_ = (tile / p.tiles_x) % p.tiles_y, img = tile / (p.tiles_x * p.tiles_y);
    const int x0 = tx_ * TW, y0 = ty_ * TH;
    const long long img_base = (long long)img * p.h * p.w;
    const uint4 *__restrict__ w2 = reinterpret_cast<const uint4 *>(p.wf) + (long long)(wv * OU_PASSES * G::STEPS) * 128 + lane;
    tc_f32x16 acc[RT], accx[RT];
#pragma unroll
    for (int i = 0; i < RT; ++i)
#pragma unroll
        for (int r = 0; r < 16; ++r) { acc[i][r] = 0.f; accx[i][r] = 0.f; }
    const unsigned char *abase[RT];
    {
        const int r = lane & 31;
#pragma unroll
        for (int i = 0; i < RT; ++i) {
            const int m = 32 * i + r;
            abase[i] = lds + ((m / TW) * G::HWD + (m % TW)) * G::CELLB + (lane >> 5) * 32;
        }
    }
#pragma unroll 1
    for (int pass = 0; pass < OU_PASSES; ++pass) {
        uint4 bq[PF][2];
        const uint4 *__restrict__ wp = w2 + (long long)pass * G::STEPS * 128;
#pragma unroll
        for (int s = 0; s < PF; ++s) { bq[s][0] = wp[s * 128]; bq[s][1] = wp[s * 128 + 64]; }
        if (pass) tc_barrier();
        if constexpr (!GATHER) {
            constexpr int PPC = OU_CP / 4, TOTAL = G::HCELLS * PPC, ROUNDS = (TOTAL + 511) / 512, B = 7;
            const int pc_valid = pass == OU_PASSES - 1 ? (OU_C - (OU_PASSES - 1) * OU_CP) / 4 : PPC;
#pragma unroll 1
            for (int rr = 0; rr < ROUNDS; rr += B) {
                uint4 v[B];
#pragma unroll
                for (int k = 0; k < B; ++k) {
                    const int q = (rr + k) * 512 + tid;
                    v[k] = make_uint4(0u, 0u, 0u, 0u);
                    if (rr + k < ROUNDS && q < TOTAL) {
                        const int c = q / PPC, pc = q - c * PPC;
                        const int cy = c / G::HWD, cx = c - cy * G::HWD;
                        const int yy = y0 - 1 + cy, xx = x0 - 1 + cx;
                        if (yy >= 0 && yy < p.h && xx >= 0 && xx < p.w && pc < pc_valid)
                            v[k] = *reinterpret_cast<const uint4 *>(p.a + (img_base + (long long)yy * p.w + xx) * p.lda + pass * OU_CP + pc * 4);
// ... 646 lines not shown
```

### mft_amd/csrc/volume_tile.hip

```cpp
#include "common.h"
#include "profile.h"

namespace mftx {

typedef float vt_f32x16 __attribute__((ext_vector_type(16)));
typedef float vt_f32x4 __attribute__((ext_vector_type(4)));
typedef float vt_f32x2 __attribute__((ext_vector_type(2)));
typedef unsigned vt_u32x4 __attribute__((ext_vector_type(4)));
typedef _Float16 vt_f16x8 __attribute__((ext_vector_type(8)));

constexpr int VT_C = 256;
constexpr int VT_ROW = VT_C * 4 + 16;
constexpr int VT_TARGETS = 128 * VT_ROW;
constexpr int VT_LDS = VT_TARGETS + 8 * 1024;

struct VolTileArgs {
    const float *f1;
    const float *f2s;
    float *lvl0, *lvl1, *lvl2, *lvl3;
    long long s0, s1, s2, s3;
    int P, N, h, w, sbw, n_sb, wb0;
    float scale;
    int qchunks, blocks_per_chunk;
    int ablate;
    int gathered;
    long long f2_bstride;
    PairPtrs f1p;
};

__device__ __forceinline__ vt_f32x16 vt_mfma(const vt_f16x8 &a, const vt_f16x8 &b, const vt_f32x16 &c) {
    return __builtin_amdgcn_mfma_f32_32x32x16_f16(a, b, c, 0, 0, 0);
}

__device__ __forceinline__ void vt_split8(const vt_f32x4 &u, const vt_f32x4 &v, float k2048, vt_f16x8 &hi, vt_f16x8 &lo) {
    unsigned h0, h1, h2, h3, l0, l1, l2, l3;
    float r0, r1, r2, r3, r4, r5, r6, r7;
    asm("v_cvt_pk_f16_f32 %0, %16, %17\n\t"
        "v_cvt_pk_f16_f32 %1, %18, %19\n\t"
        "v_cvt_pk_f16_f32 %2, %20, %21\n\t"
        "v_cvt_pk_f16_f32 %3, %22, %23\n\t"
        "v_fma_mix_f32 %8, %0, -1.0, %16 op_sel_hi:[1,0,0]\n\t"
        "v_fma_mix_f32 %9, %0, -1.0, %17 op_sel:[1,0,0] op_sel_hi:[1,0,0]\n\t"
        "v_fma_mix_f32 %10, %1, -1.0, %18 op_sel_hi:[1,0,0]\n\t"
        "v_fma_mix_f32 %11, %1, -1.0, %19 op_sel:[1,0,0] op_sel_hi:[1,0,0]\n\t"
        "v_fma_mix_f32 %12, %2, -1.0, %20 op_sel_hi:[1,0,0]\n\t"
        "v_fma_mix_f32 %13, %2, -1.0, %21 op_sel:[1,0,0] op_sel_hi:[1,0,0]\n\t"
        "v_fma_mix_f32 %14, %3, -1.0, %22 op_sel_hi:[1,0,0]\n\t"
        "v_fma_mix_f32 %15, %3, -1.0, %23 op_sel:[1,0,0] op_sel_hi:[1,0,0]\n\t"
        "v_fma_mixlo_f16 %4, %8, %24, 0\n\t"
        "v_fma_mixlo_f16 %5, %10, %24, 0\n\t"
        "v_fma_mixlo_f16 %6, %12, %24, 0\n\t"
        "v_fma_mixlo_f16 %7, %14, %24, 0\n\t"
        "v_fma_mixhi_f16 %4, %9, %24, 0\n\t"
        "v_fma_mixhi_f16 %5, %11, %24, 0\n\t"
        "v_fma_mixhi_f16 %6, %13, %24, 0\n\t"
        "v_fma_mixhi_f16 %7, %15, %24, 0\n\t"
        "s_nop 1"
        : "=&v"(h0), "=&v"(h1), "=&v"(h2), "=&v"(h3), "=&v"(l0), "=&v"(l1), "=&v"(l2), "=&v"(l3),
          "=&v"(r0), "=&v"(r1), "=&v"(r2), "=&v"(r3), "=&v"(r4), "=&v"(r5), "=&v"(r6), "=&v"(r7)
        : "v"(u[0]), "v"(u[1]), "v"(u[2]), "v"(u[3]), "v"(v[0]), "v"(v[1]), "v"(v[2]), "v"(v[3]), "s"(k2048));
    hi = __builtin_bit_cast(vt_f16x8, vt_u32x4{h0, h1, h2, h3});
    lo = __builtin_bit_cast(vt_f16x8, vt_u32x4{l0, l1, l2, l3});
}

template <int N>
__device__ __forceinline__ float vt_shl(float v) {
    return __builtin_bit_cast(float, __builtin_amdgcn_update_dpp(0, __builtin_bit_cast(int, v), 0x100 + N, 0xf, 0xf, true));
}
template <int N>
__device__ __forceinline__ float vt_shr(float v) {
    return __builtin_bit_cast(float, __builtin_amdgcn_update_dpp(0, __builtin_bit_cast(int, v), 0x110 + N, 0xf, 0xf, true));
}

__device__ __forceinline__ float vt_pool4(float a, float b, float c, float d) { return (((a + b) + c) + d) * 0.25f; }

__global__ __launch_bounds__(512, 2) void volume_tile_kernel(VolTileArgs p) {
    extern __shared__ __attribute__((aligned(16))) unsigned char vt_lds[];
    unsigned char *lds = vt_lds;
    const int tid = (int)threadIdx.x, lane = tid & 63, wv = __builtin_amdgcn_readfirstlane(tid >> 6);
    const int wg = (int)blockIdx.x;
    const int qc = wg % p.qchunks, sb = (wg / p.qchunks) % p.n_sb, bz = wg / (p.qchunks * p.n_sb);
    const int sby = sb / p.sbw, sbx = sb - sby * p.sbw;
    const float k2048 = __builtin_bit_cast(float, __builtin_amdgcn_readfirstlane(0x45000000));

    {
        const float *f2p = p.f2s + (long long)bz * p.f2_bstride;
#pragma unroll 4
        for (int k = 0; k < 16; ++k) {
            const int q = k * 512 + tid, m = q >> 6, pc = q & 63;
            const int j = m >> 5, mm = m & 31;
            const int ty = 8 * sby + 4 * (j >> 1) + (mm >> 3), tx = 16 * sbx + 8 * (j & 1) + (mm & 7);
            uint4 v = make_uint4(0u, 0u, 0u, 0u);
            if (ty < p.h && tx < p.w) v = *reinterpret_cast<const uint4 *>(f2p + ((long long)ty * p.w + tx) * VT_C + pc * 4);
            *reinterpret_cast<uint4 *>(lds + m * VT_ROW + pc * 16) = v;
        }
    }
    asm volatile("s_waitcnt lgkmcnt(0)" ::: "memory");
    __builtin_amdgcn_s_barrier();
    asm volatile("" ::: "memory");

    const unsigned char *abase = lds + (lane & 31) * VT_ROW + (lane >> 5) * 32;
    const int n_blocks = (p.N + 31) >> 5;
    const int b_lo = qc * p.blocks_per_chunk, b_hi = (b_lo + p.blocks_per_chunk < n_blocks) ? b_lo + p.blocks_per_chunk : n_blocks;
    const long long qbase = (long long)bz * p.N;
    const float inv2048 = 1.f / 2048.f;
    const int hf = lane >> 5;
    const int h2 = p.h >> 2, w2 = p.w >> 2, h3 = p.h >> 3, w3 = p.w >> 3;

    const int pp = lane & 31;
    const int l1_src = 4 * (32 * hf + 2 * (pp & 3) + 16 * ((pp >> 3) & 1) + ((pp >> 2) & 1) + 8 * (pp >> 4));
    const int l3_src = 4 * ((lane + 16) & 63);
    constexpr int PF = 3;
    vt_f32x4 raw[PF][2];
    const float *f1base = p.gathered ? p.f1p.p[bz] : p.f1 + qbase * VT_C;
    auto row_of = [&](int qb) {
        const int q = qb * 32 + (lane & 31);
        return f1base + (long long)(q < p.N ? q : p.N - 1) * VT_C + 8 * hf;
    };
    auto prefetch = [&](const float *src) {
#pragma unroll
        for (int g = 0; g < PF; ++g) {
            raw[g][0] = *reinterpret_cast<const vt_f32x4 *>(src + 16 * g);
            raw[g][1] = *reinterpret_cast<const vt_f32x4 *>(src + 16 * g + 4);
        }
    };
    if (b_lo + wv < b_hi) prefetch(row_of(b_lo + wv));
    for (int qb = b_lo + wv; qb < b_hi; qb += 8) {
        const float *src = row_of(qb);
        vt_f32x16 acc[4], accx[4];
#pragma unroll
        for (int j = 0; j < 4; ++j)
#pragma unroll
            for (int r = 0; r < 16; ++r) { acc[j][r] = 0.f; accx[j][r] = 0.f; }
        vt_f16x8 ah[2][4], al[2][4];
        auto read_a = [&](int g, int set) {
#pragma unroll
            for (int j = 0; j < 4; ++j) {
                ah[set][j] = *reinterpret_cast<const vt_f16x8 *>(abase + j * 32 * VT_ROW + g * 64);
                al[set][j] = *reinterpret_cast<const vt_f16x8 *>(abase + j * 32 * VT_ROW + g * 64 + 16);
            }
        };
        read_a(0, 0);
#pragma unroll
        for (int g = 0; g < 16; ++g) {
            const int set = g & 1;
            vt_f16x8 bh, bl;
            vt_split8(raw[g % PF][0], raw[g % PF][1], k2048, bh, bl);
            __builtin_amdgcn_sched_barrier(0);
            if (g + 1 < 16) read_a(g + 1, set ^ 1);
            if (g + PF < 16) {
                raw[g % PF][0] = *reinterpret_cast<const vt_f32x4 *>(src + 16 * (g + PF));
                raw[g % PF][1] = *reinterpret_cast<const vt_f32x4 *>(src + 16 * (g + PF) + 4);
            }
            __builtin_amdgcn_sched_barrier(0);
#pragma unroll
            for (int j = 0; j < 4; ++j) acc[j] = vt_mfma(bh, ah[set][j], acc[j]);
#pragma unroll
            for (int j = 0; j < 4; ++j) accx[j] = vt_mfma(bh, al[set][j], accx[j]);
#pragma unroll
            for (int j = 0; j < 4; ++j) accx[j] = vt_mfma(bl, ah[set][j], accx[j]);
            __builtin_amdgcn_sched_barrier(0);
        }

        if (qb + 8 < b_hi) prefetch(row_of(qb + 8));
        __builtin_amdgcn_sched_barrier(0);

        const int m = lane & 31;
        const int q0 = qb * 32;
        const long long blk0 = ((long long)(2 * sby) * p.wb0 + 2 * sbx) * 32 + m;
        const int rows_ok = p.N - q0 < 32 ? p.N - q0 : 32;
        const __amdgpu_buffer_rsrc_t r0 = __builtin_amdgcn_make_buffer_rsrc(p.lvl0 + (qbase + q0) * p.s0, 0, (unsigned)((long long)rows_ok * p.s0 * 4), 0x00020000);
        const __amdgpu_buffer_rsrc_t r1 = __builtin_amdgcn_make_buffer_rsrc(p.lvl1 + (qbase + q0) * p.s1, 0, (unsigned)((long long)rows_ok * p.s1 * 4), 0x00020000);
        const unsigned v1off = (unsigned)((4 * hf * p.s1 + ((long long)sby * p.sbw + sbx) * 32 + m) * 4);
        const unsigned s0b = (unsigned)(p.s0 * 4), s1b = (unsigned)(p.s1 * 4), jrow = (unsigned)(p.wb0 * 128);
        int le = lane;
        asm volatile("" : "+v"(le));
        const int d2c = le & 7, d2hf = (le >> 3) & 1, d2i = le >> 4;
        const int l2_pull = 4 * (32 * d2hf + 16 * (d2c >> 2) + 2 * (d2c & 3));
        const int l2_y = 2 * sby + (d2c >> 2), l2_x = 4 * sbx + (d2c & 3);
        const bool l2_ok = l2_y < h2 && l2_x < w2;
        const int l2_off = l2_y * w2 + l2_x, l2_row = 4 * d2hf + d2i;
        const int d3c = le & 1, d3hf = (le >> 1) & 1, d3r = le >> 2;
        const int l3_pull = 4 * (32 * d3hf + 4 * d3c);
        const int l3_x = 2 * sbx + d3c;
        const bool l3_ok = sby < h3 && l3_x < w3;
        const int l3_off = sby * w3 + l3_x, l3_row = 8 * (d3r >> 2) + 4 * d3hf + (d3r & 3);
        float *slab = reinterpret_cast<float *>(lds + VT_TARGETS + wv * 1024);
        const unsigned v0off4 = (unsigned)((le >> 3) * s0b) + (unsigned)((blk0 - m) * 4) + (unsigned)(le & 7) * 16u;
        float acc2 = 0.f, acc3 = 0.f;
#pragma unroll
        for (int g = 0; g < 4; ++g) {
#ifdef MFTX_TUNING
            const bool st0g = !(p.ablate & 1);
#else
            const bool st0g = true;
#endif
            float vv[4][4];
#pragma unroll
            for (int i = 0; i < 4; ++i)
#pragma unroll
                for (int j = 0; j < 4; ++j) vv[i][j] = (acc[j][4 * g + i] + accx[j][4 * g + i] * inv2048) * p.scale;
            vt_f32x4 line[4];
#pragma unroll
            for (int j = 0; j < 4; ++j) {
#pragma unroll
                for (int i = 0; i < 4; ++i) slab[(4 * hf + i) * 32 + m] = vv[i][j];
                line[j] = *reinterpret_cast<const vt_f32x4 *>(slab + (le >> 3) * 32 + (le & 7) * 4);
            }
            if (st0g) {
#pragma unroll
                for (int j = 0; j < 4; ++j)
                    __builtin_amdgcn_raw_buffer_store_b128(__builtin_bit_cast(vt_u32x4, line[j]), r0, v0off4 + (j >> 1) * jrow + (j & 1) * 128u, (unsigned)(8 * g) * s0b, 0);
            }
#pragma unroll
        for (int i = 0; i < 4; ++i) {
            const int r = 4 * g + i;
            const int qrow = q0 + 8 * (r >> 2) + 4 * hf + (r & 3);
            const bool row_ok = qrow < p.N;
#ifdef MFTX_TUNING
            const bool st1 = row_ok && !(p.ablate & 2);
#define MFTX_VT_ST23 (!(p.ablate & 10))
#else
            const bool st1 = row_ok;
#define MFTX_VT_ST23 true
#endif
            float merged = 0.f;
#pragma unroll
            for (int j = 0; j < 4; ++j) {
                const float v = vv[i][j];
                float t = v + vt_shl<1>(v);
                t = t + vt_shl<8>(v);
                t = (t + vt_shl<9>(v)) * 0.25f;
                if (j == 0) merged = t;
                else {
                    float sh = j == 1 ? vt_shr<1>(t) : (j == 2 ? vt_shr<8>(t) : vt_shr<9>(t));
                    asm volatile("" : "+v"(sh));
                    const bool take = j == 1 ? (m & 1) != 0 : (j == 2 ? ((m >> 3) & 1) && !(m & 1) : ((m >> 3) & 1) && (m & 1));
                    merged = take ? sh : merged;
                }
            }
            const float l1 = __builtin_bit_cast(float, __builtin_amdgcn_ds_bpermute(l1_src, __builtin_bit_cast(int, merged)));
            if (st1) __builtin_amdgcn_raw_buffer_store_b32(__builtin_bit_cast(unsigned, l1), r1, v1off, (unsigned)(8 * (r >> 2) + (r & 3)) * s1b, 0);
            float t2 = l1 + vt_shl<1>(l1);
            t2 = t2 + vt_shl<8>(l1);
            t2 = (t2 + vt_shl<9>(l1)) * 0.25f;
            asm volatile("" : "+v"(t2));
            {
                const float pulled = __builtin_bit_cast(float, __builtin_amdgcn_ds_bpermute(l2_pull, __builtin_bit_cast(int, t2)));
                acc2 = d2i == (r & 3) ? pulled : acc2;
                if ((r & 3) == 3) {
                    const int row2 = q0 + 8 * (r >> 2) + l2_row;
                    if (MFTX_VT_ST23 && l2_ok && row2 < p.N) p.lvl2[(qbase + row2) * p.s2 + l2_off] = acc2;
                }
            }
            const float bq = vt_shl<2>(t2);
            const float cq = __builtin_bit_cast(float, __builtin_amdgcn_ds_bpermute(l3_src, __builtin_bit_cast(int, t2)));
            const float dq = __builtin_bit_cast(float, __builtin_amdgcn_ds_bpermute(l3_src + 8, __builtin_bit_cast(int, t2)));
            float v3 = (((t2 + bq) + cq) + dq) * 0.25f;
            asm volatile("" : "+v"(v3));
            {
                const float pulled = __builtin_bit_cast(float, __builtin_amdgcn_ds_bpermute(l3_pull, __builtin_bit_cast(int, v3)));
                acc3 = d3r == r ? pulled : acc3;
                if (r == 15) {
                    const int row3 = q0 + l3_row;
                    if (MFTX_VT_ST23 && l3_ok && row3 < p.N) p.lvl3[(qbase + row3) * p.s3 + l3_off] = acc3;
                }
            }
        }
        }
    }
}

static int vt_num_cus() {
    static const int n = [] {
        int dev = 0, cus = 256;
        hipDeviceProp_t prop;
        if (hipGetDevice(&dev) == hipSuccess && hipGetDeviceProperties(&prop, dev) == hipSuccess && prop.multiProcessorCount > 0) cus = prop.multiProcessorCount;
        return cus;
    }();
    return n;
}

bool volume_tile_applicable(int C) { return C == VT_C; }

int launch_volume_tile(const float *f1, const float *f2s, int P, int h, int w, float *const lvl[4], hipStream_t s, const PairPtrs *f1p, long long f2_bstride) {
    if (f1p && P > MFTX_MAX_GATHER) return fail(MFTX_E_ARG, "corr_pyramid: at most %d gathered pairs", MFTX_MAX_GATHER);
    const PyramidLayout L = pyramid_layout(h, w);
    VolTileArgs a{};
    a.f1 = f1; a.f2s = f2s; a.lvl0 = lvl[0]; a.lvl1 = lvl[1]; a.lvl2 = lvl[2]; a.lvl3 = lvl[3];
    a.s0 = L.stride[0]; a.s1 = L.stride[1]; a.s2 = L.stride[2]; a.s3 = L.stride[3];
    a.P = P; a.N = h * w; a.h = h; a.w = w; a.sbw = L.sbw; a.n_sb = L.sbh * L.sbw; a.wb0 = L.wb[0];
    a.scale = 1.0f / sqrtf((float)VT_C);
    a.gathered = f1p ? 1 : 0;
    if (f1p) a.f1p = *f1p;
    a.f2_bstride = f2_bstride >= 0 ? f2_bstride : (long long)a.N * VT_C;
    const int n_blocks = (a.N + 31) / 32;
    const long long base = (long long)P * a.n_sb;
    a.ablate = tune_env("MFTX_VT_ABLATE", 0);
    static const int q_forced = tune_env("MFTX_VT_QCHUNKS", 0);
    int qchunks = q_forced > 0 ? q_forced : (base * 4 >= 3LL * vt_num_cus() ? 1 : (int)((vt_num_cus() + base - 1) / base));
    if (qchunks < 1) qchunks = 1;
    if (qchunks > (n_blocks + 7) / 8) qchunks = (n_blocks + 7) / 8;
    a.blocks_per_chunk = (n_blocks + qchunks - 1) / qchunks;
    a.qchunks = (n_blocks + a.blocks_per_chunk - 1) / a.blocks_per_chunk;
    const long long wgs = base * a.qchunks;
    if (wgs > 0x7fffffffLL) return fail(MFTX_E_ARG, "corr_pyramid: too many workgroups");
    static bool attr_set = false;
    if (!attr_set) {
        if (hipFuncSetAttribute(reinterpret_cast<const void *>(volume_tile_kernel), hipFuncAttributeMaxDynamicSharedMemorySize, VT_LDS) != hipSuccess)
            return fail(MFTX_E_STATE, "corr_pyramid: cannot reserve %d bytes of LDS", VT_LDS);
        attr_set = true;
    }
    ProfScope prof(PC_CORR_VOLUME, s, 2.0 * a.N * a.N * (double)VT_C * P);
    hipLaunchKernelGGL(volume_tile_kernel, dim3((unsigned)wgs), dim3(512), VT_LDS, s, a);
    return check_launch("volume_tile");
}

}
```

### mft_amd/ops.py

```python
from __future__ import annotations

import ctypes as C

import torch

from . import _lib
from ._lib import ConvDesc, MftxError, check

ACT = {None: 0, "none": 0, "relu": 1, "sigmoid": 2, "tanh": 3}


def _stream():
    return C.c_void_p(torch.cuda.current_stream().cuda_stream)


def _device_visible(t):
    return isinstance(t, torch.Tensor) and (t.is_cuda or t.is_pinned())


def copy_bytes(src: torch.Tensor, dst: torch.Tensor):
    if not (_device_visible(src) and _device_visible(dst)):
        raise MftxError("copy_bytes: tensors must be on the device or in pinned host memory")
    if not (src.is_contiguous() and dst.is_contiguous()) or src.numel() * src.element_size() != dst.numel() * dst.element_size():
        raise MftxError("copy_bytes: contiguous tensors of the same size in bytes")
# ... 693 lines not shown
                _lib.load().mftx_raft_destroy(self._h)
                self._h = None
        except Exception:
            pass

    def debug_refine(self, fmap1, fmap2, net, inp, h, w, iters, pads=(0, 0, 0, 0), flow_init=None):
        lib = _lib.load()
        P = fmap1.shape[0]
        M = P * h * w
        trace = torch.empty(iters + 1, M, 2, dtype=torch.float32, device=self.device)
        check(lib.mftx_raft_set_coords_trace(self._h, trace.data_ptr()), "mftx_raft_set_coords_trace")
        try:
            out = self.refine(fmap1, fmap2, net, inp, h, w, iters, pads=pads, flow_init=flow_init)
        finally:
            check(lib.mftx_raft_set_coords_trace(self._h, None), "mftx_raft_set_coords_trace")
        if self.ondemand_corr:
            pyramid = None
        else:
            stride, _ = pyramid_layout(h, w)
            pyramid = []
            for l in range(4):
                lvl = self.region(f"lvl{l}", P, h, w, stride[l]).reshape(P, h * w, stride[l])
                pyramid.append(unblock_level(lvl, l, h, w).reshape(M, 1, h >> l, w >> l).cpu())
        to_map = lambda t: t.reshape(P, h, w, 2).permute(0, 3, 1, 2).contiguous().cpu()
        ys, xs = torch.meshgrid(torch.arange(h, dtype=torch.float32), torch.arange(w, dtype=torch.float32), indexing="ij")
        debug = {"costvolume_pyramid": pyramid,
                 "coords_left": torch.stack([xs, ys])[None].repeat(P, 1, 1, 1),
                 "iterations": [{"coords": to_map(trace[i])} for i in range(iters + 1)]}
        return out, debug

    def graph_stats(self):
        c, r = C.c_ulonglong(), C.c_ulonglong()
        check(_lib.load().mftx_raft_graph_stats(self._h, C.byref(c), C.byref(r)), "mftx_raft_graph_stats")
        return int(c.value), int(r.value)

    def nonfinite_count(self, reset=False):
        n = int(self._nonfinite[0].item())
        if reset and n:
            self._nonfinite.zero_()
        return n

    def nonfinite_snapshot(self, host_words):
        copy_bytes(self._nonfinite, host_words)

    def set_option(self, name, value):
        if name not in self.OPTIONS:
            raise MftxError(f"unknown engine option {name!r} (known: {', '.join(sorted(self.OPTIONS))}, gather)")
        check(_lib.load().mftx_raft_set_option(self._h, self.OPTIONS[name], int(value)), "mftx_raft_set_option")
        if name == "tile_conv":
            self._tile_conv = int(value)
        if name == "tile_volume":
            self._tile_volume = int(value)

    def workspace(self, P, h, w):
        need = _lib.load().mftx_raft_workspace_bytes_for(self._h, P, h, w)
        if self._ws is None or self._ws.numel() < need:
            if self._ws is not None:
                check(_lib.load().mftx_raft_clear_graphs(self._h), "mftx_raft_clear_graphs")
            self._ws = torch.empty(need, dtype=torch.uint8, device=self.device)
        return self._ws

    REGIONS = ("lvl0", "lvl1", "lvl2", "lvl3", "coords1", "corr", "cor1", "corflo", "flo1", "hx", "z", "rh", "fh",
               "delta", "mask", "ouin", "ouh", "ou", "flow_lr")

    SPLIT_REGIONS = {"cor1": 256, "corflo": 256, "flo1": 128, "hx": 384, "rh": 128, "ouin": 712}

    def region(self, name, P, h, w, cols):
        offs = (C.c_size_t * 19)()
        check(_lib.load().mftx_raft_workspace_layout_for(self._h, P, h, w, offs, 19), "mftx_raft_workspace_layout_for")
        off = offs[self.REGIONS.index(name)]
        M = P * h * w
        if self.arith == ARITH_SPLIT and name in self.SPLIT_REGIONS:
            ld = self.SPLIT_REGIONS[name]
            raw = self._ws[off: off + 4 * M * ld].view(torch.float32).reshape(M, ld)
            return unsplit_activations(raw)[:, :cols]
        return self._ws[off: off + 4 * M * cols].view(torch.float32).reshape(M, cols)

    MAX_GATHER = 16

    def can_gather(self, P):
        return (self.arith == ARITH_SPLIT and not self.ondemand_corr and P <= self.MAX_GATHER and
                getattr(self, "_tile_volume", 1) != 0 and getattr(self, "_gather", True))

    def refine(self, fmap1, fmap2, net, inp, h, w, iters, pads=(0, 0, 0, 0), want_flow_lr=False, flow_init=None,
               packed=None, planar=True):
        lib = _lib.load()
        gathered = isinstance(fmap1, (list, tuple))
        P = len(fmap1) if gathered else fmap1.shape[0]
        pl, pr, pt, pb = pads
        H0, W0 = 8 * h - pt - pb, 8 * w - pl - pr
        dev = self.device
        if not planar and packed is None:
            raise MftxError("refine: planar=False needs a packed output")
        flow = torch.empty(P, 2, H0, W0, dtype=torch.float32, device=dev) if planar else None
        occl = torch.empty(P, 1, H0, W0, dtype=torch.float32, device=dev) if planar else None
        sigma = torch.empty(P, 1, H0, W0, dtype=torch.float32, device=dev) if planar else None
        flow_lr = torch.empty(P, h * w, 2, dtype=torch.float32, device=dev) if want_flow_lr else None
        if flow_init is not None and tuple(flow_init.shape) != (P, h * w, 2):
            raise MftxError("flow_init must be [P, h*w, 2]")
        if packed is not None and tuple(packed.shape) != (P, H0, W0, 4):
            raise MftxError("packed must be [P, H0, W0, 4]")
        ws = self.workspace(P, h, w)
        if gathered:
            if not self.can_gather(P) or not (len(fmap2) == len(net) == len(inp) == P):
                raise MftxError("refine: per-pair map lists need the split arithmetic with the tile-resident volume and P <= 16")
            arrs = [_lib.ptr_array([_chk(t, "map") for t in lst]) for lst in (fmap1, fmap2, net, inp)]
            check(lib.mftx_raft_refine_gather(self._h, P, h, w, iters, arrs[0][0], arrs[1][0], arrs[2][0], arrs[3][0],
                                              _chk(flow_init, "flow_init") if flow_init is not None else None,
                                              pl, pr, pt, pb,
                                              flow.data_ptr() if planar else None, occl.data_ptr() if planar else None,
                                              sigma.data_ptr() if planar else None,
                                              _chk(packed, "packed") if packed is not None else None,
                                              flow_lr.data_ptr() if want_flow_lr else None,
                                              ws.data_ptr(), ws.numel(), _stream()), "mftx_raft_refine_gather")
            return (flow, occl, sigma, flow_lr) if want_flow_lr else (flow, occl, sigma)
        check(lib.mftx_raft_refine(self._h, P, h, w, iters, _chk(fmap1, "fmap1"), _chk(fmap2, "fmap2"),
                                   _chk(net, "net"), _chk(inp, "inp"),
                                   _chk(flow_init, "flow_init") if flow_init is not None else None,
                                   pl, pr, pt, pb,
                                   flow.data_ptr() if planar else None, occl.data_ptr() if planar else None,
                                   sigma.data_ptr() if planar else None,
                                   _chk(packed, "packed") if packed is not None else None,
                                   flow_lr.data_ptr() if want_flow_lr else None,
                                   ws.data_ptr(), ws.numel(), _stream()), "mftx_raft_refine")
        return (flow, occl, sigma, flow_lr) if want_flow_lr else (flow, occl, sigma)
```

### mft_amd/raft.py

```python
from __future__ import annotations

import logging
import os
from pathlib import Path

import numpy as np
import torch
import torch.nn.functional as F

from . import ops
from .weights import make_weights, strip_module_prefix

logger = logging.getLogger(__name__)


def pad_amounts(H0, W0):
    ph = (((H0 // 8) + 1) * 8 - H0) % 8
    pw = (((W0 // 8) + 1) * 8 - W0) % 8
    return pw // 2, pw - pw // 2, ph // 2, ph - ph // 2


_STREAMS = {}


def _shared_stream(device, kind, index=0):
    device = torch.device(device)
    dev_index = device.index if device.index is not None else torch.cuda.current_device()
    key = (dev_index, kind, index)
    st = _STREAMS.get(key)
    if st is None:
        st = _STREAMS[key] = torch.cuda.Stream(device=torch.device("cuda", dev_index))
    return st


class FrameFeatures:
    __slots__ = ("fmap", "net", "inp", "h", "w", "pads", "shape", "ready")

    def __init__(self, fmap, net, inp, h, w, pads, shape, ready=None):
        self.fmap, self.net, self.inp, self.h, self.w, self.pads, self.shape = fmap, net, inp, h, w, pads, shape
        self.ready = ready


class RAFTWrapper:
    has_packed_output = True
    STAGING_SLOTS = 4

    def __init__(self, config, device="cuda", state_dict=None):
        self.C = config
        self.device = torch.device(device)
        if self.device.type != "cuda":
            raise RuntimeError("mft_amd.RAFTWrapper runs on an MI355X (HIP) device only; there is no CPU path")
        if state_dict is None:
            state_dict = self._load_weights(config)
        sd = {k: (v if isinstance(v, torch.Tensor) else torch.from_numpy(np.asarray(v)))
              for k, v in strip_module_prefix(state_dict).items()}
        self.sd = {k: v.to(self.device) for k, v in sd.items()}
        self._ondemand = bool(getattr(getattr(config, "raft_params", None), "alternate_corr", False))
        arith = getattr(getattr(config, "raft_params", None), "arith", None) or "split"
        if arith not in ("split", "fp32"):
            raise ValueError(f"raft_params.arith must be 'split' or 'fp32', got {arith!r}")
        self._arith = ops.ARITH_SPLIT if arith == "split" else ops.ARITH_F32
        self._engine_options = dict(getattr(getattr(config, "raft_params", None), "engine_options", None) or {})
        try:
            self._build_engines()
        except ops.SplitRangeError as e:
            logger.warning("raft_params.arith = 'split' refused (%s): falling back to arith = 'fp32'", e)
            self._arith = ops.ARITH_F32
            self._build_engines()
        self._check_finite = bool(getattr(getattr(config, "raft_params", None), "check_finite", False))
        self._split_streams = int(os.environ.get("MFTX_SPLIT_STREAMS", "") or getattr(config, "split_streams", 0) or
                                  (1 if self._arith == ops.ARITH_SPLIT else 2))
        self._engines, self._side = [], []
        self._fif = self._frames_in_flight_setting(config)
        self._lanes, self._lane_next = [], 0
        self._lanes_stale = False
        self._ahead_max = max(2, int(getattr(config, "max_batches_ahead", 0) or 16))
        self._ahead = []
        self.nominal_pairs = int(getattr(config, "nominal_pairs", 0) or 7)
        self._tile_choice = {}
        self._frames = {}
        self._staging = {}
        ae = getattr(config, "__dict__", {}).get("async_encode", None)
        self._enc_waits_for_device_frames = ae is None
        if ae is None:
            ae = self._frames_in_flight_setting(config) > 1
        self._enc_stream = _shared_stream(self.device, "enc") if ae else None

    def _frames_in_flight_setting(self, config):
        return max(1, int(os.environ.get("MFTX_FRAMES_IN_FLIGHT", "") or getattr(config, "frames_in_flight", 0) or
                          (2 if self._arith == ops.ARITH_SPLIT else 1)))

    def _build_engines(self):
        graph = bool(self._engine_options.get("graph", 1))
        self.fnet_engine = ops.EncoderEngine(self.sd, "fnet", True, self.device, arith=self._arith, graph=graph)
        self.cnet_engine = ops.EncoderEngine(self.sd, "cnet", False, self.device, arith=self._arith, graph=graph)
        self.engine = ops.RaftEngine(self.sd, self.device, ondemand_corr=self._ondemand, arith=self._arith,
                                     options=self._engine_options)

    def set_nominal_pairs(self, n):
        n = max(1, int(n))
        if n != self.nominal_pairs:
            self.nominal_pairs = n
            self._tile_choice = {}

    def _pin_kernels(self, h, w):
        if self._arith != ops.ARITH_SPLIT or "tile_conv" in self._engine_options:
            return
        v = self._tile_choice.get((h, w))
        if v is None:
            v = self._tile_choice[(h, w)] = 2 if ops._lib.load().mftx_tile_conv_fills_chip(self.nominal_pairs, h, w) else 0
        for e in self._all_engines():
            if getattr(e, "_tile_conv", None) != v:
                e.set_option("tile_conv", v)

    def _all_engines(self):
        return list(dict.fromkeys([self.engine] + list(self._engines) + [e for e, _ in self._lanes]))

    def _lane(self):
        while len(self._lanes) < self._fif:
            eng = self.engine if not self._lanes else ops.RaftEngine(self.sd, self.device, ondemand_corr=self._ondemand,
                                                                      arith=self._arith, options=self._engine_options)
            self._lanes.append((eng, _shared_stream(self.device, "lane", len(self._lanes))))
            self._lanes_stale = True
        lane = self._lanes[self._lane_next % self._fif]
        self._lane_next += 1
        return lane

    def _lanes_fit(self, P, h, w):
        while self._fif > max(1, len(self._lanes)):
            k = max(1, len(self._lanes))
            need = int(ops._lib.load().mftx_raft_workspace_bytes_for(self.engine._h, P, h, w))
            free, total = torch.cuda.mem_get_info(self.device)
            cached = torch.cuda.memory_reserved(self.device) - torch.cuda.memory_allocated(self.device)
            if need <= free + cached - total // 10:
                return
            logger.warning("frames_in_flight = %d needs %.1f GB more workspace (lane %d, %d pairs of %d x %d cells) but only %.1f GB of "
                           "the device's %.1f GB are free: running with %d frame(s) in flight", self._fif, need / 1e9, k, P, h, w,
                           (free + cached) / 1e9, total / 1e9, k)
            self._fif = k

    def nonfinite_count(self, reset=False):
        return sum(e.nonfinite_count(reset=reset) for e in self._all_engines())

    def nonfinite_snapshot(self, host_words):
        for i, e in enumerate(self._all_engines()):
            e.nonfinite_snapshot(host_words[i])

    def nonfinite_error(self, bad):
        return FloatingPointError(
            f"flow network: {bad} output pixels with a non-finite value (a NaN, or an infinite flow / occlusion)" + (
                " -- an activation left the fp16 range of the split arithmetic (|x| >= 65504); "
                "set raft_params.arith = 'fp32'" if self._arith == ops.ARITH_SPLIT else ""))

    def raise_if_nonfinite(self):
        bad = self.nonfinite_count(reset=True)
        if bad:
            raise self.nonfinite_error(bad)

    @property
    def arith(self):
        return "split" if self._arith == ops.ARITH_SPLIT else "fp32"

    @staticmethod
    def _load_weights(config):
        model = getattr(config, "model", None)
        seed = getattr(config, "synthetic_weights_seed", None)
        if model:
            if not Path(str(model)).exists():
                raise FileNotFoundError(
                    f"flow checkpoint {model!r} not found (set flow_config.model = None and "
                    "flow_config.synthetic_weights_seed = <int> to run on seeded synthetic weights)")
            logger.info("loading checkpoint %s", model)
            return torch.load(model, map_location="cpu")
        if not isinstance(seed, int) or isinstance(seed, bool):
            raise ValueError("no flow checkpoint configured: set flow_config.model, or "
                             "flow_config.synthetic_weights_seed = <int> for seeded synthetic weights")
        logger.warning("no checkpoint configured: using seeded synthetic weights (seed %d)", seed)
        return make_weights(seed)

    @staticmethod
    def _geometry(H0, W0):
        pads = pad_amounts(H0, W0)
        return (H0 + pads[2] + pads[3]) // 8, (W0 + pads[0] + pads[1]) // 8, pads

    def _device_image(self, img_bgr):
        img = img_bgr if isinstance(img_bgr, torch.Tensor) else torch.from_numpy(np.ascontiguousarray(img_bgr))
        if img.is_cuda:
            return img.to(self.device, non_blocking=True).contiguous()
        if img.dtype == torch.uint8 and not (img.is_pinned() and img.is_contiguous() and img.data_ptr() % 16 == 0):
            img = self._stage_host_frame(img)
        if img.is_pinned() and img.is_contiguous() and img.dtype == torch.uint8 and img.data_ptr() % 16 == 0:
            dev = torch.empty(img.shape, dtype=torch.uint8, device=self.device)
            ops.copy_bytes(img, dev)
            st = getattr(img, "_mftx_slot", None)
            if st is not None:
                st[1] = torch.cuda.current_stream(self.device).record_event()
# ... 48 lines not shown
            img = self._device_image(img_bgr)
            buf = torch.empty(N * 512, dtype=torch.float32, device=self.device)
            self.fnet_engine.forward(img, out=(buf[: N * 256].view(N, 256), None))
            self.cnet_engine.forward(img, out=(buf[N * 256: N * 384].view(N, 128), buf[N * 384:].view(N, 128)))
            return buf

        if self._enc_stream is None or torch.cuda.current_stream(self.device) == self._enc_stream:
            cur = torch.cuda.current_stream(self.device)
            self._encode_begin(cur)
            buf = run()
            self._encode_end(cur.record_event(), cur)
            return buf, (h, w)
        main = torch.cuda.current_stream(self.device)
        self._encode_begin(self._enc_stream)
        with torch.cuda.stream(self._enc_stream):
            buf = run()
            self._encode_end(self._enc_stream.record_event(), self._enc_stream)
        if wait:
            main.wait_stream(self._enc_stream)
            buf.record_stream(main)
        return buf, (h, w)

    @torch.no_grad()
    def encode_half(self, img_bgr, part, wait=True):
        H0, W0 = img_bgr.shape[:2]
        h, w, _ = self._geometry(H0, W0)
        N = h * w

        def run():
            img = self._device_image(img_bgr)
            buf = torch.empty(N * 256, dtype=torch.float32, device=self.device)
            if part == 0:
                self.fnet_engine.forward(img, out=(buf.view(N, 256), None))
            else:
                self.cnet_engine.forward(img, out=(buf[: N * 128].view(N, 128), buf[N * 128:].view(N, 128)))
            return buf

        if self._enc_stream is None or torch.cuda.current_stream(self.device) == self._enc_stream:
            cur = torch.cuda.current_stream(self.device)
            self._encode_begin(cur)
            buf = run()
            self._encode_end(cur.record_event(), cur)
            return buf, (h, w)
        main = torch.cuda.current_stream(self.device)
        self._encode_begin(self._enc_stream)
        with torch.cuda.stream(self._enc_stream):
            buf = run()
            self._encode_end(self._enc_stream.record_event(), self._enc_stream)
        if wait:
            main.wait_stream(self._enc_stream)
            buf.record_stream(main)
        return buf, (h, w)

    def adopt_halves(self, frame_id, fbuf, cbuf, img_bgr, ready=None):
        H0, W0 = img_bgr.shape[:2]
        h, w, pads = self._geometry(H0, W0)
        N = h * w
        assert fbuf.numel() == N * 256 and cbuf.numel() == N * 256
        fbuf, cbuf = fbuf.reshape(-1), cbuf.reshape(-1)
        self._frames[frame_id] = FrameFeatures(fbuf.view(N, 256), cbuf[: N * 128].view(N, 128), cbuf[N * 128:].view(N, 128),
                                               h, w, pads, (H0, W0), ready=ready)

    def packed_numel(self, img_bgr):
        h, w, _ = self._geometry(*img_bgr.shape[:2])
        return h * w * 512

    def adopt_packed(self, frame_id, buf, img_bgr, ready=None):
        H0, W0 = img_bgr.shape[:2]
        h, w, pads = self._geometry(H0, W0)
        N = h * w
        assert buf.numel() == N * 512
        buf = buf.reshape(-1)
        self._frames[frame_id] = FrameFeatures(buf[: N * 256].view(N, 256), buf[N * 256: N * 384].view(N, 128),
                                               buf[N * 384:].view(N, 128), h, w, pads, (H0, W0), ready=ready)

    def reset_cache(self):
        self._frames = {}

    def retain(self, frame_ids):
        keep = set(frame_ids)
        for k in [k for k in self._frames if k not in keep]:
            del self._frames[k]

    def _encode(self, img):
        if self._enc_stream is None:
            cur = torch.cuda.current_stream()
            self._encode_begin(cur)
            f = self.encode(img)
            f.ready = cur.record_event()
            self._encode_end(f.ready, cur)
            return f
        main = torch.cuda.current_stream()
        if self._enc_waits_for_device_frames and isinstance(img, torch.Tensor) and img.is_cuda:
            self._encode_begin(main)
            f = self.encode(img)
            f.ready = main.record_event()
            self._encode_end(f.ready, main)
            return f
        self._encode_begin(self._enc_stream)
        with torch.cuda.stream(self._enc_stream):
            f = self.encode(img)
            f.ready = self._enc_stream.record_event()
        self._encode_end(f.ready, self._enc_stream)
        main.wait_stream(self._enc_stream)
        for t in (f.fmap, f.net, f.inp):
            if t is not None:
                t.record_stream(main)
        return f

    def _encode_begin(self, stream):
        prev = getattr(self, "_last_encode", None)
        if prev is not None and prev[1] != stream:
            stream.wait_event(prev[0])

    def _encode_end(self, event, stream):
        self._last_encode = (event, stream)

    def _features(self, key, img):
        if key is None:
            return self._encode(img)
        f = self._frames.get(key)
        if f is None or f.shape != img.shape[:2]:
            f = self._encode(img)
            self._frames[key] = f
        return f

    @torch.no_grad()
    def compute_pairs(self, pairs, iters=None, init_flow=None, packed_out=None, planar=True):
        iters = int(iters if iters is not None else self.C.flow_iters)
        fls = [self._features(lk, li) for lk, li, _, _ in pairs]
        frs = [self._features(rk, ri) for _, _, rk, ri in pairs]
        ref = fls[0]
        for f in fls + frs:
            if f.shape != ref.shape:
                raise ValueError("all frames of a batch must have the same size")
        P = len(pairs)
        gather = self.engine.can_gather(P) and not (self._split_streams > 1 and P >= 6 and init_flow is None)
        if gather:
            fmap1, fmap2 = [f.fmap for f in fls], [f.fmap for f in frs]
            net, inp = [f.net for f in fls], [f.inp for f in fls]
        else:
            fmap1 = torch.stack([f.fmap for f in fls])
            fmap2 = torch.stack([f.fmap for f in frs])
            net = torch.stack([f.net for f in fls])
            inp = torch.stack([f.inp for f in fls])
        flow_init = None
        if init_flow is not None:
            flow_init = self._init_flow_lr(init_flow, ref)
        packed = None
        H0, W0 = ref.shape
        want_planar = planar or packed_out is None or packed_out is False
        if (self._fif > 1 and gather and flow_init is None and not self._check_finite
                and (packed_out is None or isinstance(packed_out, bool))):
            return self._refine_on_lane(fls, frs, fmap1, fmap2, net, inp, ref, iters, bool(packed_out), want_planar)
        if packed_out is not None and packed_out is not False:
            packed = packed_out if isinstance(packed_out, torch.Tensor) else \
                torch.empty(P, H0, W0, 4, dtype=torch.float32, device=self.device)
        self._pin_kernels(ref.h, ref.w)
        if self._lanes:
            for _, s_ in self._lanes:
                torch.cuda.current_stream(self.device).wait_stream(s_)
            self._lanes_stale = True
        if self._split_streams > 1 and P >= 6 and flow_init is None:
            flow, occl, sigma = self._refine_split(fmap1, fmap2, net, inp, ref, iters, packed, want_planar)
        else:
            flow, occl, sigma = self.engine.refine(fmap1, fmap2, net, inp, ref.h, ref.w, iters, pads=ref.pads,
                                                   flow_init=flow_init, packed=packed, planar=want_planar)
        if self._check_finite:
            bad = sum(ops.count_not_below(t.reshape(-1), float("inf")) for t in (packed, flow, occl, sigma) if t is not None)
            if bad:
                raise FloatingPointError(
                    f"compute_flow: {bad} non-finite output values" + (
                        " -- an activation left the fp16 range of the split arithmetic (|x| >= 65504); "
                        "set raft_params.arith = 'fp32'" if self._arith == ops.ARITH_SPLIT else ""))
        if packed is not None and flow is None:
            return [(None, None, None, packed[i]) for i in range(P)]
        if packed is not None:
            return [(flow[i], occl[i], sigma[i], packed[i]) for i in range(P)]
        return [(flow[i], occl[i], sigma[i]) for i in range(P)]

    def _refine_on_lane(self, fls, frs, fmap1, fmap2, net, inp, geom, iters, want_packed, planar):
        P = len(fls)
        H0, W0 = geom.shape
        self._lanes_fit(P, geom.h, geom.w)
        eng, st = self._lane()
        main = torch.cuda.current_stream(self.device)
        self._pin_kernels(geom.h, geom.w)
        if self._lanes_stale:
            for _, s_ in self._lanes:
                s_.wait_stream(main)
            self._lanes_stale = False
        for f in dict.fromkeys(fls + frs):
            if f.ready is not None:
                st.wait_event(f.ready)
            else:
                st.wait_stream(main)
            for t in (f.fmap, f.net, f.inp):
                if t is not None:
                    t.record_stream(st)
        with torch.cuda.stream(st):
            packed = torch.empty(P, H0, W0, 4, dtype=torch.float32, device=self.device) if want_packed else None
            flow, occl, sigma = eng.refine(fmap1, fmap2, net, inp, geom.h, geom.w, iters, pads=geom.pads,
                                           flow_init=None, packed=packed, planar=planar)
            done = st.record_event()
        main.wait_event(done)
        self._ahead.append(done)
        while len(self._ahead) > self._ahead_max:
            self._ahead.pop(0).synchronize()
        for t in (packed, flow, occl, sigma):
            if t is not None:
                t.record_stream(main)
        if packed is not None and flow is None:
            return [(None, None, None, packed[i]) for i in range(P)]
        if packed is not None:
            return [(flow[i], occl[i], sigma[i], packed[i]) for i in range(P)]
        return [(flow[i], occl[i], sigma[i]) for i in range(P)]

    def _refine_split(self, fmap1, fmap2, net, inp, geom, iters, packed, planar):
        P = fmap1.shape[0]
        H0, W0 = geom.shape
        S = min(self._split_streams, P)
        while len(self._engines) < S:
            self._engines.append(ops.RaftEngine(self.sd, self.device, ondemand_corr=self._ondemand, arith=self._arith,
                                                options=self._engine_options)
                                 if self._engines else self.engine)
            self._side.append(torch.cuda.Stream(device=self.device) if self._side or len(self._engines) > 1 else None)
        self._pin_kernels(geom.h, geom.w)
        dev = self.device
        flow = torch.empty(P, 2, H0, W0, dtype=torch.float32, device=dev) if planar else None
        occl = torch.empty(P, 1, H0, W0, dtype=torch.float32, device=dev) if planar else None
        sigma = torch.empty(P, 1, H0, W0, dtype=torch.float32, device=dev) if planar else None
        bounds = [(P * k) // S for k in range(S + 1)]
        parts = [(self._engines[k], self._side[k], slice(bounds[k], bounds[k + 1])) for k in range(S)]
        for eng, _, sl in parts:
            eng.workspace(sl.stop - sl.start, geom.h, geom.w)
        main = torch.cuda.current_stream()

        def run(eng, sl):
            f, o, s_ = eng.refine(fmap1[sl], fmap2[sl], net[sl], inp[sl], geom.h, geom.w, iters, pads=geom.pads,
                                  packed=packed[sl] if packed is not None else None, planar=planar)
            if planar:
                flow[sl].copy_(f); occl[sl].copy_(o); sigma[sl].copy_(s_)

        for eng, st, sl in parts[1:]:
            st.wait_stream(main)
            with torch.cuda.stream(st):
                run(eng, sl)
        run(parts[0][0], parts[0][2])
        for _, st, _ in parts[1:]:
            main.wait_stream(st)
        return flow, occl, sigma

    def compute_flow_many(self, lefts, right, iters=None):
        return self.compute_pairs([(k, im, right[0], right[1]) for k, im in lefts], iters)

    def _init_flow_lr(self, init_flow, geom):
        x = torch.as_tensor(init_flow).to(self.device, torch.float32)
        if x.dim() == 3:
            x = x[None]
        x = F.pad(x, list(geom.pads), mode="replicate")
        x = F.interpolate(x, size=(geom.h, geom.w), mode="bilinear", align_corners=True) / 8
        return x.permute(0, 2, 3, 1).reshape(x.shape[0], geom.h * geom.w, 2).contiguous()

    @torch.no_grad()
    def compute_flow(self, src_img, dst_img, mode="TC", vis=False, src_img_identifier=None, numpy_out=False,
                     init_flow=None, vis_debug=False):
        H, W = src_img.shape[:2]
        debug = None
        if vis_debug:
            fl, fr = self._features(None, src_img), self._features(None, dst_img)
            flow_init = self._init_flow_lr(init_flow, fl) if init_flow is not None else None
            self._pin_kernels(fl.h, fl.w)
            if self._lanes:
                for _, s_ in self._lanes:
                    torch.cuda.current_stream(self.device).wait_stream(s_)
                self._lanes_stale = True
            (flow, occl, sigma), debug = self.engine.debug_refine(fl.fmap[None], fr.fmap[None], fl.net[None], fl.inp[None],
                                                                   fl.h, fl.w, int(self.C.flow_iters), pads=fl.pads,
                                                                   flow_init=flow_init)
            flow, occl, sigma = flow[0], occl[0], sigma[0]
        else:
            (flow, occl, sigma), = self.compute_pairs([(None, src_img, None, dst_img)], init_flow=init_flow)
        assert flow.shape == (2, H, W)
        conv = (lambda t: t.detach().cpu().numpy()) if numpy_out else (lambda t: t)
        if mode == "flow":
            return conv(flow), {"occlusion": conv(occl), "sigma": conv(sigma), "debug": debug}
# ... 9 lines not shown
```

Measured before the change: 187.0 frames/s.

## Precompute per-frame GRU context convolutions and split feature maps once per frame

```diff
diff --git a/include/mftx.h b/include/mftx.h
--- a/include/mftx.h
+++ b/include/mftx.h
@@ -133,6 +133,16 @@
                             const float *flow_init, int pad_left, int pad_right, int pad_top, int pad_bottom,
                             float *flow, float *occl, float *sigma, float *packed, float *flow_lr_out,
                             void *workspace, size_t workspace_bytes, void *stream);
+size_t mftx_raft_frame_prepare_bytes(int h, int w);
+int mftx_raft_frame_prepare(mftx_raft *r, int h, int w, const float *fmap, const float *inp, float *ctx_zr1, float *ctx_q1,
+                            float *ctx_zr2, float *ctx_q2, void *fmap_split, void *scratch, size_t scratch_bytes, void *stream);
+int mftx_raft_refine_gather_ex(mftx_raft *r, int P, int h, int w, int iters, const float *const *fmap1,
+                               const float *const *fmap2, const float *const *net, const float *const *inp,
+                               const float *const *ctx_parts, const void *const *fmap1_split, const void *fmap2_split,
+                               const float *flow_init, int pad_left, int pad_right, int pad_top, int pad_bottom,
+                               float *flow, float *occl, float *sigma, float *packed, float *flow_lr_out,
+                               void *workspace, size_t workspace_bytes, void *stream);
+int mftx_volume_query_split(const float *in, void *out, long long n_floats, void *stream);
 
 typedef struct mftx_encoder mftx_encoder;
 int mftx_encoder_create(const float *const *weights, int n_weights, int instance_norm, mftx_encoder **out);
diff --git a/mft_amd/_lib.py b/mft_amd/_lib.py
--- a/mft_amd/_lib.py
+++ b/mft_amd/_lib.py
@@ -94,6 +94,14 @@
                                           C.c_int, C.c_int, C.c_int, C.c_int,
                                           C.c_void_p, C.c_void_p, C.c_void_p, C.c_void_p, C.c_void_p,
                                           C.c_void_p, C.c_size_t, C.c_void_p]),
+    "mftx_raft_refine_gather_ex": (C.c_int, [C.c_void_p, C.c_int, C.c_int, C.c_int, C.c_int,
+                                             _PP, _PP, _PP, _PP, _PP, _PP, C.c_void_p, C.c_void_p,
+                                             C.c_int, C.c_int, C.c_int, C.c_int,
+                                             C.c_void_p, C.c_void_p, C.c_void_p, C.c_void_p, C.c_void_p,
+                                             C.c_void_p, C.c_size_t, C.c_void_p]),
+    "mftx_raft_frame_prepare_bytes": (C.c_size_t, [C.c_int, C.c_int]),
+    "mftx_raft_frame_prepare": (C.c_int, [C.c_void_p, C.c_int, C.c_int] + [C.c_void_p] * 8 + [C.c_size_t, C.c_void_p]),
+    "mftx_volume_query_split": (C.c_int, [C.c_void_p, C.c_void_p, C.c_longlong, C.c_void_p]),
     "mftx_encoder_create": (C.c_int, [_PP, C.c_int, C.c_int, C.POINTER(C.c_void_p)]),
     "mftx_encoder_destroy": (None, [C.c_void_p]),
     "mftx_encoder_set_graph": (C.c_int, [C.c_void_p, C.c_int]),
diff --git a/mft_amd/csrc/common.h b/mft_amd/csrc/common.h
--- a/mft_amd/csrc/common.h
+++ b/mft_amd/csrc/common.h
@@ -115,7 +115,8 @@
 constexpr int MFTX_MAX_GATHER = 16;
 struct PairPtrs { const float *p[MFTX_MAX_GATHER]; };
 int launch_volume_tile(const float *f1, const float *f2s, int P, int h, int w, float *const lvl[4], hipStream_t s,
-                       const PairPtrs *f1p = nullptr, long long f2_bstride = -1);
+                       const PairPtrs *f1p = nullptr, long long f2_bstride = -1, bool f1_split = false);
+int launch_volume_query_split(const float *in, void *out, long long n_floats, hipStream_t s);
 int launch_corr_lookup(const float *const lvl[4], const float *coords, int P, int h, int w,
                        float *out, int ld_out, hipStream_t s);
 int launch_pack_lookup_convc1(const float *w, int ld_w, void *out, hipStream_t s);
@@ -143,6 +144,7 @@
     const float *h_in; int ld_hin; const float *mo; int ld_mo;
     const void *wzr, *wq;
     const float *pre_zr, *pre_q;
+    const float *const *ctx;
     float *z; const float *hf_in; float *hf_out;
     float *h_out; int ld_hout;
     int P, h, w, pass;
diff --git a/mft_amd/csrc/raft_engine.hip b/mft_amd/csrc/raft_engine.hip
--- a/mft_amd/csrc/raft_engine.hip
+++ b/mft_amd/csrc/raft_engine.hip
@@ -9,11 +9,16 @@
 
 
 struct InitGather { int on; PairPtrs netp, inpp; };
+struct CtxTable { const float **table; const float *own[4]; int supplied; PairPtrs parts[4]; };
 __global__ void init_state_kernel(const float *__restrict__ net, const float *__restrict__ inp,
                                   const float *__restrict__ flow_init, float *hx, float *hf, float *coords1, int M, int h,
-                                  int w, InitGather ga) {
+                                  int w, InitGather ga, CtxTable ct) {
     const long long i = (long long)blockIdx.x * blockDim.x + threadIdx.x;
     if (i >= (long long)M * 64) return;
+    if (ct.table != nullptr && i < (long long)(M / (h * w)) * 4) {
+        const int b = (int)(i >> 2), k = (int)(i & 3);
+        ct.table[i] = ct.supplied ? ct.parts[k].p[b] : ct.own[k] + (long long)b * h * w * ((k & 1) ? 128 : 256);
+    }
     const int m = (int)(i >> 6), q = (int)(i & 63);
     if (ga.on) {
         const int b = m / (h * w);
@@ -108,6 +113,7 @@
     float *f2s;
     float *hf;
     float *hb, *hfb;
+    const float **ctx;
     int ld_corr;
     size_t bytes;
 };
@@ -145,6 +151,7 @@
     ws.hf = take(split ? M * 128 : 0);
     ws.hb = take(split ? M * 128 : 0);
     ws.hfb = take(split ? M * 128 : 0);
+    ws.ctx = reinterpret_cast<const float **>(take(split ? (size_t)P * 8 : 0));
     ws.bytes = off;
     return ws;
 }
@@ -363,7 +370,35 @@
     return d;
 }
 
-struct RefineGather { PairPtrs f1, f2, net, inp; bool f2_shared; };
+struct RefineGather { PairPtrs f1, f2, net, inp; bool f2_shared; bool has_ctx, has_f1s; PairPtrs ctx[4], f1s; const float *f2s; };
+
+static int launch_context_parts(const mftx_raft *r, bool tiles_on, bool sp, const float *inp, int ld, int P, int h, int w,
+                                float *const zr[2], float *const q[2], hipStream_t s) {
+    const float *const *W = r->w;
+    const float *const *G = r->wg;
+    for (int pass = 0; pass < 2; ++pass) {
+        const int kh = pass ? 5 : 1, kw = pass ? 1 : 5;
+        const int slot[2] = {pass ? W_ZR2_INP : W_ZR1_INP, pass ? W_Q2_INP : W_Q1_INP};
+        const float *bias[2] = {W[pass ? B_ZR2 : B_ZR1], W[pass ? B_Q2 : B_Q1]};
+        float *out[2] = {zr[pass], q[pass]};
+        for (int k = 0; k < 2; ++k) {
+            const int N = k ? 128 : 256;
+            if (tiles_on && r->wt[slot[k]]) {
+                TileConvLaunch t{};
+                t.a0 = inp; t.lda0 = ld; t.cin = 128; t.wf = r->wt[slot[k]]; t.bias = bias[k];
+                t.P = P; t.h = h; t.w = w; t.N = N; t.kh = kh; t.kw = kw; t.epi = 0;
+                t.cells = r->opt[MFTX_RAFT_OPT_TILE_CELLS];
+                t.out = out[k]; t.ldo = N;
+                TRY(launch_tile_conv(t, s));
+            } else {
+                mftx_conv_desc d = conv_desc(inp, ld, 128, nullptr, 0, 0, G[slot[k]], bias[k], out[k], N, P, h, w, N, kh, kw, 0);
+                d.arith = r->arith; d.a_split = sp; d.out_split = false;
+                TRY(launch_conv(d, s));
+            }
+        }
+    }
+    return 0;
+}
 static int refine_impl(mftx_raft *r, int P, int h, int w, int iters, const float *fmap1,
                                 const float *fmap2, const float *net, const float *inp, const float *flow_init,
                                 int pad_left,
@@ -410,26 +445,39 @@
     if (ondemand) TRY(launch_fmap_pyramid(fmap2, P, 256, h, w, ws.f2l, s));
     else if (gather) {
         const long long pair_floats = (long long)N * 256;
-        if (gather->f2_shared) TRY(launch_split_weights(gather->f2.p[0], ws.f2s, pair_floats, s));
+        const float *f2s = ws.f2s;
+        if (gather->f2_shared && gather->f2s) f2s = gather->f2s;
+        else if (gather->f2_shared) TRY(launch_split_weights(gather->f2.p[0], ws.f2s, pair_floats, s));
         else for (int b = 0; b < P; ++b) TRY(launch_split_weights(gather->f2.p[b], ws.f2s + b * pair_floats, pair_floats, s));
-        TRY(launch_volume_tile(nullptr, ws.f2s, P, h, w, ws.lvl, s, &gather->f1, gather->f2_shared ? 0 : pair_floats));
+        TRY(launch_volume_tile(nullptr, f2s, P, h, w, ws.lvl, s, gather->has_f1s ? &gather->f1s : &gather->f1, gather->f2_shared ? 0 : pair_floats,
+                               gather->has_f1s));
     }
     else TRY(launch_corr_pyramid(fmap1, fmap2, P, 256, h, w, ws.lvl, s, r->arith == MFTX_ARITH_SPLIT ? ws.f2s : nullptr, r->opt[MFTX_RAFT_OPT_TILE_VOLUME]));
+    const bool tiles_on = SP && r->opt[MFTX_RAFT_OPT_TILE_CONV] != 0 &&
+                          (r->opt[MFTX_RAFT_OPT_TILE_CONV] == 2 ||
+                           (tile_conv_fills_chip(P, h, w, 3, 3) && tile_conv_fills_chip(P, h, w, 1, 5) && tile_conv_fills_chip(P, h, w, 5, 1)));
+    auto tile_w = [&](int slot) -> const void * { return tiles_on ? r->wt[slot] : nullptr; };
+    const bool gru_fused = tile_w(W_ZR1_DYN) && tile_w(W_Q1_DYN) && tile_w(W_ZR2_DYN) && tile_w(W_Q2_DYN) &&
+                           r->opt[MFTX_RAFT_OPT_FUSE_GRU] != 0;
+    const bool ctx_supplied = gather && gather->has_ctx && gru_fused;
     {
         const long long slots = (long long)M * 64;
         ProfScope prof(PC_GLUE, s, 0);
         InitGather ga{};
         if (gather) { ga.on = 1; ga.netp = gather->net; ga.inpp = gather->inp; }
+        CtxTable ct{};
+        if (gru_fused) {
+            ct.table = ws.ctx;
+            ct.own[0] = ws.pre_zr[0]; ct.own[1] = ws.pre_q[0]; ct.own[2] = ws.pre_zr[1]; ct.own[3] = ws.pre_q[1];
+            ct.supplied = ctx_supplied ? 1 : 0;
+            if (ctx_supplied) for (int k = 0; k < 4; ++k) ct.parts[k] = gather->ctx[k];
+        }
         hipLaunchKernelGGL(init_state_kernel, dim3((unsigned)((slots + 255) / 256)), dim3(256), 0, s, net, inp,
-                           flow_init, ws.hx, SP ? ws.hf : nullptr, ws.coords1, M, h, w, ga);
+                           flow_init, ws.hx, SP ? ws.hf : nullptr, ws.coords1, M, h, w, ga, ct);
         TRY(check_launch("init_state"));
     }
     float *flow_lr = flow_lr_out ? flow_lr_out : ws.flow_lr;
     auto core = [&]() -> int {
-    const bool tiles_on = SP && r->opt[MFTX_RAFT_OPT_TILE_CONV] != 0 &&
-                          (r->opt[MFTX_RAFT_OPT_TILE_CONV] == 2 ||
-                           (tile_conv_fills_chip(P, h, w, 3, 3) && tile_conv_fills_chip(P, h, w, 1, 5) && tile_conv_fills_chip(P, h, w, 5, 1)));
-    auto tile_w = [&](int slot) -> const void * { return tiles_on ? r->wt[slot] : nullptr; };
     auto tile_layer = [&](const float *a0, int lda0, const float *a1, int lda1, const void *wf, const float *bias, int N, int kh, int kw, int epi) {
         TileConvLaunch t{};
         t.a0 = a0; t.lda0 = lda0; t.a1 = a1; t.lda1 = lda1; t.cin = a1 ? 256 : 128; t.wf = wf; t.bias = bias;
@@ -437,20 +485,7 @@
         t.cells = r->opt[MFTX_RAFT_OPT_TILE_CELLS];
         return t;
     };
-    for (int pass = 0; pass < 2; ++pass) {
-        const int kh = pass ? 5 : 1, kw = pass ? 1 : 5;
-        const int szr = pass ? W_ZR2_INP : W_ZR1_INP, sq = pass ? W_Q2_INP : W_Q1_INP;
-        if (tile_w(szr)) {
-            TileConvLaunch t = tile_layer(ws.hx + 128, 384, nullptr, 0, tile_w(szr), W[pass ? B_ZR2 : B_ZR1], 256, kh, kw, 0);
-            t.out = ws.pre_zr[pass]; t.ldo = 256;
-            TRY(launch_tile_conv(t, s));
-        } else TRY(launch_conv(gemm(conv_desc(ws.hx + 128, 384, 128, nullptr, 0, 0, G[szr], W[pass ? B_ZR2 : B_ZR1], ws.pre_zr[pass], 256, P, h, w, 256, kh, kw, 0), true, false), s));
-        if (tile_w(sq)) {
-            TileConvLaunch t = tile_layer(ws.hx + 128, 384, nullptr, 0, tile_w(sq), W[pass ? B_Q2 : B_Q1], 128, kh, kw, 0);
-            t.out = ws.pre_q[pass]; t.ldo = 128;
-            TRY(launch_tile_conv(t, s));
-        } else TRY(launch_conv(gemm(conv_desc(ws.hx + 128, 384, 128, nullptr, 0, 0, G[sq], W[pass ? B_Q2 : B_Q1], ws.pre_q[pass], 128, P, h, w, 128, kh, kw, 0), true, false), s));
-    }
+    if (!ctx_supplied) TRY(launch_context_parts(r, tiles_on, SP, ws.hx + 128, 384, P, h, w, ws.pre_zr, ws.pre_q, s));
     const float *lv[4] = {ws.lvl[0], ws.lvl[1], ws.lvl[2], ws.lvl[3]};
     const int strips = cdiv(w, F1_CELLS);
     float *ccur = ws.coords1, *calt = ws.flo1;
@@ -530,15 +565,13 @@
         }
         if (two_pass) TRY(launch_tile_conv2p(ws.corflo, 256, r->wt[W_CONV], W[B_CONV], ws.hx + 256, 384, 126, P, h, w, r->opt[MFTX_RAFT_OPT_TILE_CELLS], s));
         else TRY(launch_conv(gemm(conv_desc(ws.corflo, 256, 256, nullptr, 0, 0, G[W_CONV], W[B_CONV], ws.hx + 256, 384, P, h, w, 126, 3, 3, 1), true, true), s));
-        const bool gru_fused = tile_w(W_ZR1_DYN) && tile_w(W_Q1_DYN) && tile_w(W_ZR2_DYN) && tile_w(W_Q2_DYN) &&
-                               r->opt[MFTX_RAFT_OPT_FUSE_GRU] != 0;
         for (int pass = 0; pass < 2; ++pass) {
             const int kh = pass ? 5 : 1, kw = pass ? 1 : 5;
             const int szr = pass ? W_ZR2_DYN : W_ZR1_DYN, sq = pass ? W_Q2_DYN : W_Q1_DYN;
             if (gru_fused) {
                 GruHalfLaunch g{};
                 g.h_in = pass ? ws.hb : ws.hx; g.ld_hin = pass ? 128 : 384; g.h_out = pass ? ws.hx : ws.hb; g.ld_hout = pass ? 384 : 128;
-                g.mo = ws.hx + 256; g.ld_mo = 384; g.wzr = tile_w(szr); g.wq = tile_w(sq); g.pre_zr = ws.pre_zr[pass]; g.pre_q = ws.pre_q[pass];
+                g.mo = ws.hx + 256; g.ld_mo = 384; g.wzr = tile_w(szr); g.wq = tile_w(sq); g.pre_zr = ws.pre_zr[pass]; g.pre_q = ws.pre_q[pass]; g.ctx = ws.ctx;
                 g.z = ws.z; g.hf_in = pass ? ws.hfb : ws.hf; g.hf_out = pass ? ws.hf : ws.hfb; g.P = P; g.h = h; g.w = w; g.pass = pass; g.cells = r->opt[MFTX_RAFT_OPT_TILE_CELLS];
                 TRY(launch_gru_half(g, s));
                 continue;
@@ -619,7 +652,7 @@
         key.v[4] = reinterpret_cast<uintptr_t>(workspace); key.v[5] = reinterpret_cast<uintptr_t>(flow_lr_out);
         key.v[6] = (uintptr_t)AR; key.v[7] = reinterpret_cast<uintptr_t>(r->wfused); key.v[8] = reinterpret_cast<uintptr_t>(s);
         key.v[9] = reinterpret_cast<uintptr_t>(r->wflow); key.v[10] = reinterpret_cast<uintptr_t>(r->wt[W_ZR1_DYN]); key.v[11] = reinterpret_cast<uintptr_t>(r->wproj);
-        key.v[12] = reinterpret_cast<uintptr_t>(r->wou);
+        key.v[12] = reinterpret_cast<uintptr_t>(r->wou); key.v[13] = ctx_supplied ? 1 : 0;
         TRY(r->graphs->run(key, s, core));
     } else {
         TRY(core());
@@ -642,6 +675,16 @@
                                        const float *flow_init, int pad_left, int pad_right, int pad_top, int pad_bottom,
                                        float *flow, float *occl, float *sigma, float *packed, float *flow_lr_out,
                                        void *workspace, size_t workspace_bytes, void *stream) {
+    return mftx_raft_refine_gather_ex(r, P, h, w, iters, fmap1, fmap2, net, inp, nullptr, nullptr, nullptr, flow_init, pad_left, pad_right, pad_top,
+                                      pad_bottom, flow, occl, sigma, packed, flow_lr_out, workspace, workspace_bytes, stream);
+}
+
+extern "C" int mftx_raft_refine_gather_ex(mftx_raft *r, int P, int h, int w, int iters, const float *const *fmap1,
+                                          const float *const *fmap2, const float *const *net, const float *const *inp,
+                                          const float *const *ctx_parts, const void *const *fmap1_split, const void *fmap2_split,
+                                          const float *flow_init, int pad_left, int pad_right, int pad_top, int pad_bottom,
+                                          float *flow, float *occl, float *sigma, float *packed, float *flow_lr_out,
+                                          void *workspace, size_t workspace_bytes, void *stream) {
     if (!r || r->magic != RAFT_MAGIC) return fail(MFTX_E_STATE, "raft_refine_gather: bad handle");
     if (!fmap1 || !fmap2 || !net || !inp) return fail(MFTX_E_ARG, "raft_refine_gather: null pointer");
     if (P < 1 || P > MFTX_MAX_GATHER) return fail(MFTX_E_ARG, "raft_refine_gather: 1 .. %d pairs", MFTX_MAX_GATHER);
@@ -655,8 +698,77 @@
         g.f1.p[b] = fmap1[b]; g.f2.p[b] = fmap2[b]; g.net.p[b] = net[b]; g.inp.p[b] = inp[b];
         if (fmap2[b] != fmap2[0]) g.f2_shared = false;
     }
+    if (ctx_parts) {
+        for (int i = 0; i < 4 * P; ++i)
+            if (!ctx_parts[i] || !aligned16(ctx_parts[i])) return fail(MFTX_E_ALIGN, "raft_refine_gather: context part %d of pair %d null or not 16-byte aligned", i & 3, i >> 2);
+        g.has_ctx = true;
+        for (int b = 0; b < P; ++b) for (int k = 0; k < 4; ++k) g.ctx[k].p[b] = ctx_parts[4 * b + k];
+    }
+    if (fmap1_split) {
+        for (int b = 0; b < P; ++b) {
+            if (!fmap1_split[b] || !aligned16(fmap1_split[b])) return fail(MFTX_E_ALIGN, "raft_refine_gather: split map of pair %d null or not 16-byte aligned", b);
+            g.f1s.p[b] = static_cast<const float *>(fmap1_split[b]);
+        }
+        g.has_f1s = true;
+    }
+    if (fmap2_split) {
+        if (!aligned16(fmap2_split)) return fail(MFTX_E_ALIGN, "raft_refine_gather: the second map's split form must be 16-byte aligned");
+        if (!g.f2_shared) return fail(MFTX_E_ARG, "raft_refine_gather: a split second map goes with ONE second map for all pairs");
+        g.f2s = static_cast<const float *>(fmap2_split);
+    }
     return refine_impl(r, P, h, w, iters, nullptr, nullptr, nullptr, nullptr, flow_init, pad_left, pad_right, pad_top, pad_bottom, flow, occl,
                        sigma, packed, flow_lr_out, workspace, workspace_bytes, stream, &g);
+}
+
+__global__ void split_rows_kernel(const float *__restrict__ in, float *__restrict__ out, long long slots, int c4) {
+    const long long i = (long long)blockIdx.x * blockDim.x + threadIdx.x;
+    if (i >= slots) return;
+    const long long m = i / c4;
+    const int q = (int)(i - m * c4);
+    store_split4v(out + m * 4 * c4, 4 * q, reinterpret_cast<const float4 *>(in)[i]);
+}
+
+extern "C" size_t mftx_raft_frame_prepare_bytes(int h, int w) {
+    if (h <= 0 || w <= 0) return 0;
+    return ((size_t)h * w * 128 * sizeof(float) + 255) & ~size_t(255);
+}
+
+extern "C" int mftx_raft_frame_prepare(mftx_raft *r, int h, int w, const float *fmap, const float *inp, float *ctx_zr1, float *ctx_q1,
+                                       float *ctx_zr2, float *ctx_q2, void *fmap_split, void *scratch, size_t scratch_bytes, void *stream) {
+    if (!r || r->magic != RAFT_MAGIC) return fail(MFTX_E_STATE, "raft_frame_prepare: bad handle");
+    if (h < 16 || w < 16 || (long long)h * w > (1ll << 24)) return fail(MFTX_E_ARG, "raft_frame_prepare: bad size");
+    const bool want_ctx = ctx_zr1 || ctx_q1 || ctx_zr2 || ctx_q2;
+    if (!want_ctx && !fmap_split) return fail(MFTX_E_ARG, "raft_frame_prepare: nothing to write");
+    if (r->arith != MFTX_ARITH_SPLIT || r->opt[MFTX_RAFT_OPT_PRESPLIT] == 0)
+        return fail(MFTX_E_STATE, "raft_frame_prepare: needs the split arithmetic with split-form activations");
+    hipStream_t s = (hipStream_t)stream;
+    const long long N = (long long)h * w;
+    if (fmap_split) {
+        if (!fmap) return fail(MFTX_E_ARG, "raft_frame_prepare: a split map needs fmap");
+        TRY(launch_split_weights(fmap, fmap_split, N * 256, s));
+    }
+    if (!want_ctx) return 0;
+    if (!inp || !ctx_zr1 || !ctx_q1 || !ctx_zr2 || !ctx_q2 || !scratch) return fail(MFTX_E_ARG, "raft_frame_prepare: the context parts need inp, all four outputs and the scratch");
+    if (r->opt[MFTX_RAFT_OPT_TILE_CONV] == 1)
+        return fail(MFTX_E_STATE, "raft_frame_prepare: MFTX_RAFT_OPT_TILE_CONV must be pinned (0 or 2), the batch decides otherwise");
+    if (!aligned16(inp) || !aligned16(ctx_zr1) || !aligned16(ctx_q1) || !aligned16(ctx_zr2) || !aligned16(ctx_q2) ||
+        (reinterpret_cast<uintptr_t>(scratch) & 255))
+        return fail(MFTX_E_ALIGN, "raft_frame_prepare: maps must be 16-byte and the scratch 256-byte aligned");
+    if (scratch_bytes < mftx_raft_frame_prepare_bytes(h, w))
+        return fail(MFTX_E_WORKSPACE, "raft_frame_prepare: scratch %zu < %zu bytes", scratch_bytes, mftx_raft_frame_prepare_bytes(h, w));
+    float *inps = static_cast<float *>(scratch);
+    {
+        const long long slots = N * 32;
+        hipLaunchKernelGGL(split_rows_kernel, dim3((unsigned)((slots + 255) / 256)), dim3(256), 0, s, inp, inps, slots, 32);
+        TRY(check_launch("split_rows"));
+    }
+    float *const zr[2] = {ctx_zr1, ctx_zr2}, *const q[2] = {ctx_q1, ctx_q2};
+    return launch_context_parts(r, r->opt[MFTX_RAFT_OPT_TILE_CONV] == 2, true, inps, 128, 1, h, w, zr, q, s);
+}
+
+extern "C" int mftx_volume_query_split(const float *in, void *out, long long n_floats, void *stream) {
+    if (!in || !out) return fail(MFTX_E_ARG, "volume_query_split: null pointer");
+    return launch_volume_query_split(in, out, n_floats, (hipStream_t)stream);
 }
 
 extern "C" int mftx_raft_graph_stats(const mftx_raft *r, unsigned long long *captures, unsigned long long *replays) {
diff --git a/mft_amd/csrc/tile_conv.hip b/mft_amd/csrc/tile_conv.hip
--- a/mft_amd/csrc/tile_conv.hip
+++ b/mft_amd/csrc/tile_conv.hip
@@ -366,6 +366,8 @@
     const float *mo; int ld_mo;
     const void *wzr, *wq;
     const float *pre_zr, *pre_q;
+    const float *const *ctx;
+    int pass;
     float *z;
     const float *hf_in; float *hf_out;
     float *h_out; int ld_hout;
@@ -422,6 +424,11 @@
     const int olo = n_along > 1 ? t_along * p.step : 0, ohi = n_along > 1 ? min(len_along, olo + p.step) : len_along;
     const int x0 = HORIZ ? r0 : tx_ * TW, y0 = HORIZ ? ty_ * TH : r0;
     const long long img_base = (long long)img * p.h * p.w;
+    const float *pre_zr = p.pre_zr, *pre_q = p.pre_q;
+    if (p.ctx != nullptr) {
+        pre_zr = p.ctx[4 * img + 2 * p.pass] - img_base * 256;
+        pre_q = p.ctx[4 * img + 2 * p.pass + 1] - img_base * 128;
+    }
     const uint4 *__restrict__ w1 = reinterpret_cast<const uint4 *>(p.wzr) + (long long)((wv ^ 4) * G1::STEPS) * 128 + lane;
     const int nt2 = wv % G2::NT, ks2 = wv / G2::NT;
     const uint4 *__restrict__ w2 = reinterpret_cast<const uint4 *>(p.wq) + (long long)((nt2 * G2::KS + ks2) * G2::STEPS) * 128 + lane;
@@ -509,7 +516,7 @@
             tc_f32x4 a[4], hh[4];
 #pragma unroll
             for (int b = 0; b < 4; ++b) {
-                a[b] = *reinterpret_cast<const tc_f32x4 *>(p.pre_zr + cell * 256 + 128 + n0 + 8 * b);
+                a[b] = *reinterpret_cast<const tc_f32x4 *>(pre_zr + cell * 256 + 128 + n0 + 8 * b);
                 hh[b] = *reinterpret_cast<const tc_f32x4 *>(p.hf_in + cell * 128 + n0 + 8 * b);
             }
 #pragma unroll
@@ -586,11 +593,11 @@
         v += *reinterpret_cast<const tc_f32x4 *>(src + CELLS * G2::RED_ROW + 4);
         if (yy < 0 || yy >= p.h || xx < 0 || xx >= p.w || along < olo || along >= ohi) continue;
         const long long cell = img_base + (long long)yy * p.w + xx;
-        u += *reinterpret_cast<const tc_f32x4 *>(p.pre_q + cell * 128 + n0);
-        v += *reinterpret_cast<const tc_f32x4 *>(p.pre_q + cell * 128 + n0 + 4);
+        u += *reinterpret_cast<const tc_f32x4 *>(pre_q + cell * 128 + n0);
+        v += *reinterpret_cast<const tc_f32x4 *>(pre_q + cell * 128 + n0 + 4);
         tc_f32x4 z0 = *reinterpret_cast<const tc_f32x4 *>(p.z + cell * 128 + n0), z1 = *reinterpret_cast<const tc_f32x4 *>(p.z + cell * 128 + n0 + 4);
-        z0 += *reinterpret_cast<const tc_f32x4 *>(p.pre_zr + cell * 256 + n0);
-        z1 += *reinterpret_cast<const tc_f32x4 *>(p.pre_zr + cell * 256 + n0 + 4);
+        z0 += *reinterpret_cast<const tc_f32x4 *>(pre_zr + cell * 256 + n0);
+        z1 += *reinterpret_cast<const tc_f32x4 *>(pre_zr + cell * 256 + n0 + 4);
 #pragma unroll
         for (int e = 0; e < 4; ++e) { z0[e] = tc_sigmoid(z0[e]); z1[e] = tc_sigmoid(z1[e]); }
         const float *hrow = p.hf_in + cell * 128 + n0;
@@ -645,7 +652,7 @@
 }
 
 int launch_gru_half(const GruHalfLaunch &d, hipStream_t s) {
-    if (!d.h_in || !d.mo || !d.wzr || !d.wq || !d.pre_zr || !d.pre_q || !d.z || !d.hf_in || !d.hf_out || !d.h_out) return fail(MFTX_E_ARG, "gru_half: null pointer");
+    if (!d.h_in || !d.mo || !d.wzr || !d.wq || (!d.ctx && (!d.pre_zr || !d.pre_q)) || !d.z || !d.hf_in || !d.hf_out || !d.h_out) return fail(MFTX_E_ARG, "gru_half: null pointer");
     if (d.P <= 0 || d.h <= 0 || d.w <= 0 || (d.pass != 0 && d.pass != 1)) return fail(MFTX_E_ARG, "gru_half: bad sizes");
     if (d.h_in == d.h_out || d.hf_in == d.hf_out) return fail(MFTX_E_ARG, "gru_half: h is read from one buffer and written to another");
     auto bad_split = [](const float *p, int ld) { return (reinterpret_cast<uintptr_t>(p) & 31) != 0 || (ld % 8) != 0; };
@@ -653,7 +660,7 @@
         !aligned16(d.pre_zr) || !aligned16(d.pre_q) || !aligned16(d.z) || !aligned16(d.hf_in) || !aligned16(d.hf_out))
         return fail(MFTX_E_ALIGN, "gru_half: split-form rows are 32-byte aligned with strides in multiples of 8; the rest 16-byte aligned");
     GruHalfArgs a{};
-    a.h_in = d.h_in; a.ld_hin = d.ld_hin; a.mo = d.mo; a.ld_mo = d.ld_mo; a.wzr = d.wzr; a.wq = d.wq; a.pre_zr = d.pre_zr; a.pre_q = d.pre_q;
+    a.h_in = d.h_in; a.ld_hin = d.ld_hin; a.mo = d.mo; a.ld_mo = d.ld_mo; a.wzr = d.wzr; a.wq = d.wq; a.pre_zr = d.pre_zr; a.pre_q = d.pre_q; a.ctx = d.ctx; a.pass = d.pass;
     a.z = d.z; a.hf_in = d.hf_in; a.hf_out = d.hf_out; a.h_out = d.h_out; a.ld_hout = d.ld_hout; a.P = d.P; a.h = d.h; a.w = d.w;
     const bool hz = d.pass == 0;
     auto best = [&](int cells, int &th, int &tw) {
diff --git a/mft_amd/csrc/volume_tile.hip b/mft_amd/csrc/volume_tile.hip
--- a/mft_amd/csrc/volume_tile.hip
+++ b/mft_amd/csrc/volume_tile.hip
@@ -74,6 +74,7 @@
 
 __device__ __forceinline__ float vt_pool4(float a, float b, float c, float d) { return (((a + b) + c) + d) * 0.25f; }
 
+template <bool QSPLIT>
 __global__ __launch_bounds__(512, 2) void volume_tile_kernel(VolTileArgs p) {
     extern __shared__ __attribute__((aligned(16))) unsigned char vt_lds[];
     unsigned char *lds = vt_lds;
@@ -145,7 +146,10 @@
         for (int g = 0; g < 16; ++g) {
             const int set = g & 1;
             vt_f16x8 bh, bl;
-            vt_split8(raw[g % PF][0], raw[g % PF][1], k2048, bh, bl);
+            if constexpr (QSPLIT) {
+                bh = __builtin_bit_cast(vt_f16x8, raw[g % PF][0]);
+                bl = __builtin_bit_cast(vt_f16x8, raw[g % PF][1]);
+            } else vt_split8(raw[g % PF][0], raw[g % PF][1], k2048, bh, bl);
             __builtin_amdgcn_sched_barrier(0);
             if (g + 1 < 16) read_a(g + 1, set ^ 1);
             if (g + PF < 16) {
@@ -283,7 +287,27 @@
 
 bool volume_tile_applicable(int C) { return C == VT_C; }
 
-int launch_volume_tile(const float *f1, const float *f2s, int P, int h, int w, float *const lvl[4], hipStream_t s, const PairPtrs *f1p, long long f2_bstride) {
+__global__ void vt_query_split_kernel(const float *__restrict__ in, uint4 *__restrict__ out, long long n8) {
+    const long long i = (long long)blockIdx.x * blockDim.x + threadIdx.x;
+    const float k2048 = __builtin_bit_cast(float, __builtin_amdgcn_readfirstlane(0x45000000));
+    if (i >= n8) return;
+    const vt_f32x4 u = *reinterpret_cast<const vt_f32x4 *>(in + i * 8), v = *reinterpret_cast<const vt_f32x4 *>(in + i * 8 + 4);
+    vt_f16x8 hi, lo;
+    vt_split8(u, v, k2048, hi, lo);
+    out[2 * i] = __builtin_bit_cast(uint4, hi);
+    out[2 * i + 1] = __builtin_bit_cast(uint4, lo);
+}
+
+int launch_volume_query_split(const float *in, void *out, long long n, hipStream_t s) {
+    if (n <= 0 || n % 8) return fail(MFTX_E_ARG, "volume_query_split: a positive multiple of 8 floats");
+    if (!aligned16(in) || !aligned16(out)) return fail(MFTX_E_ALIGN, "volume_query_split: operands must be 16-byte aligned");
+    const long long n8 = n / 8;
+    hipLaunchKernelGGL(vt_query_split_kernel, dim3((unsigned)((n8 + 255) / 256)), dim3(256), 0, s, in, reinterpret_cast<uint4 *>(out), n8);
+    return check_launch("volume_query_split");
+}
+
+int launch_volume_tile(const float *f1, const float *f2s, int P, int h, int w, float *const lvl[4], hipStream_t s, const PairPtrs *f1p, long long f2_bstride,
+                       bool f1_split) {
     if (f1p && P > MFTX_MAX_GATHER) return fail(MFTX_E_ARG, "corr_pyramid: at most %d gathered pairs", MFTX_MAX_GATHER);
     const PyramidLayout L = pyramid_layout(h, w);
     VolTileArgs a{};
@@ -307,12 +331,14 @@
     if (wgs > 0x7fffffffLL) return fail(MFTX_E_ARG, "corr_pyramid: too many workgroups");
     static bool attr_set = false;
     if (!attr_set) {
-        if (hipFuncSetAttribute(reinterpret_cast<const void *>(volume_tile_kernel), hipFuncAttributeMaxDynamicSharedMemorySize, VT_LDS) != hipSuccess)
+        if (hipFuncSetAttribute(reinterpret_cast<const void *>(volume_tile_kernel<false>), hipFuncAttributeMaxDynamicSharedMemorySize, VT_LDS) != hipSuccess ||
+            hipFuncSetAttribute(reinterpret_cast<const void *>(volume_tile_kernel<true>), hipFuncAttributeMaxDynamicSharedMemorySize, VT_LDS) != hipSuccess)
             return fail(MFTX_E_STATE, "corr_pyramid: cannot reserve %d bytes of LDS", VT_LDS);
         attr_set = true;
     }
     ProfScope prof(PC_CORR_VOLUME, s, 2.0 * a.N * a.N * (double)VT_C * P);
-    hipLaunchKernelGGL(volume_tile_kernel, dim3((unsigned)wgs), dim3(512), VT_LDS, s, a);
+    if (f1_split) hipLaunchKernelGGL(volume_tile_kernel<true>, dim3((unsigned)wgs), dim3(512), VT_LDS, s, a);
+    else hipLaunchKernelGGL(volume_tile_kernel<false>, dim3((unsigned)wgs), dim3(512), VT_LDS, s, a);
     return check_launch("volume_tile");
 }
 
diff --git a/mft_amd/ops.py b/mft_amd/ops.py
--- a/mft_amd/ops.py
+++ b/mft_amd/ops.py
@@ -799,8 +799,25 @@
         return (self.arith == ARITH_SPLIT and not self.ondemand_corr and P <= self.MAX_GATHER and
                 getattr(self, "_tile_volume", 1) != 0 and getattr(self, "_gather", True))
 
+    def prepare_frame(self, fmap, inp, h, w, context=True, split=True):
+        lib = _lib.load()
+        N = h * w
+        dev = self.device
+        ctx = fsplit = scratch = None
+        if context:
+            ctx = tuple(torch.empty(N, c, dtype=torch.float32, device=dev) for c in (256, 128, 256, 128))
+            scratch = torch.empty(lib.mftx_raft_frame_prepare_bytes(h, w), dtype=torch.uint8, device=dev)
+        if split:
+            fsplit = torch.empty(N, 256, dtype=torch.float32, device=dev)
+        cp = [t.data_ptr() for t in ctx] if context else [None] * 4
+        check(lib.mftx_raft_frame_prepare(self._h, h, w, _chk(fmap, "fmap") if split else None, _chk(inp, "inp") if context else None,
+                                          *cp, fsplit.data_ptr() if split else None,
+                                          scratch.data_ptr() if context else None, scratch.numel() if context else 0, _stream()),
+              "mftx_raft_frame_prepare")
+        return ctx, fsplit
+
     def refine(self, fmap1, fmap2, net, inp, h, w, iters, pads=(0, 0, 0, 0), want_flow_lr=False, flow_init=None,
-               packed=None, planar=True):
+               packed=None, planar=True, prepared=None):
         lib = _lib.load()
         gathered = isinstance(fmap1, (list, tuple))
         P = len(fmap1) if gathered else fmap1.shape[0]
@@ -822,6 +839,22 @@
             if not self.can_gather(P) or not (len(fmap2) == len(net) == len(inp) == P):
                 raise MftxError("refine: per-pair map lists need the split arithmetic with the tile-resident volume and P <= 16")
             arrs = [_lib.ptr_array([_chk(t, "map") for t in lst]) for lst in (fmap1, fmap2, net, inp)]
+            if prepared:
+                ctx, f1s, f2s = prepared.get("ctx"), prepared.get("f1s"), prepared.get("f2s")
+                if (ctx is not None and len(ctx) != P) or (f1s is not None and len(f1s) != P):
+                    raise MftxError("refine: prepared parts for every pair, or none")
+                carr = _lib.ptr_array([_chk(t, "context part") for parts in ctx for t in parts]) if ctx is not None else (None, None)
+                sarr = _lib.ptr_array([_chk(t, "split map") for t in f1s]) if f1s is not None else (None, None)
+                check(lib.mftx_raft_refine_gather_ex(self._h, P, h, w, iters, arrs[0][0], arrs[1][0], arrs[2][0], arrs[3][0],
+                                                     carr[0], sarr[0], _chk(f2s, "split map") if f2s is not None else None,
+                                                     _chk(flow_init, "flow_init") if flow_init is not None else None,
+                                                     pl, pr, pt, pb,
+                                                     flow.data_ptr() if planar else None, occl.data_ptr() if planar else None,
+                                                     sigma.data_ptr() if planar else None,
+                                                     _chk(packed, "packed") if packed is not None else None,
+                                                     flow_lr.data_ptr() if want_flow_lr else None,
+                                                     ws.data_ptr(), ws.numel(), _stream()), "mftx_raft_refine_gather_ex")
+                return (flow, occl, sigma, flow_lr) if want_flow_lr else (flow, occl, sigma)
             check(lib.mftx_raft_refine_gather(self._h, P, h, w, iters, arrs[0][0], arrs[1][0], arrs[2][0], arrs[3][0],
                                               _chk(flow_init, "flow_init") if flow_init is not None else None,
                                               pl, pr, pt, pb,
@@ -831,6 +864,8 @@
                                               flow_lr.data_ptr() if want_flow_lr else None,
                                               ws.data_ptr(), ws.numel(), _stream()), "mftx_raft_refine_gather")
             return (flow, occl, sigma, flow_lr) if want_flow_lr else (flow, occl, sigma)
+        if prepared:
+            raise MftxError("refine: prepared parts go with per-pair map lists")
         check(lib.mftx_raft_refine(self._h, P, h, w, iters, _chk(fmap1, "fmap1"), _chk(fmap2, "fmap2"),
                                    _chk(net, "net"), _chk(inp, "inp"),
                                    _chk(flow_init, "flow_init") if flow_init is not None else None,
diff --git a/mft_amd/raft.py b/mft_amd/raft.py
--- a/mft_amd/raft.py
+++ b/mft_amd/raft.py
@@ -34,11 +34,16 @@
 
 
 class FrameFeatures:
-    __slots__ = ("fmap", "net", "inp", "h", "w", "pads", "shape", "ready")
+    __slots__ = ("fmap", "net", "inp", "h", "w", "pads", "shape", "ready", "ctx", "fsplit")
 
     def __init__(self, fmap, net, inp, h, w, pads, shape, ready=None):
         self.fmap, self.net, self.inp, self.h, self.w, self.pads, self.shape = fmap, net, inp, h, w, pads, shape
         self.ready = ready
+        self.ctx = None
+        self.fsplit = None
+
+    def tensors(self):
+        return [t for t in (self.fmap, self.net, self.inp, self.fsplit) + tuple(self.ctx or ()) if t is not None]
 
 
 class RAFTWrapper:
@@ -78,6 +83,9 @@
         self._ahead = []
         self.nominal_pairs = int(getattr(config, "nominal_pairs", 0) or 7)
         self._tile_choice = {}
+        fp = os.environ.get("MFTX_FRAME_PREPARE", "")
+        self._frame_prepare = bool(int(fp)) if fp else bool(getattr(config, "__dict__", {}).get("frame_prepare", True))
+        self._prepare_ok = {}
         self._frames = {}
         self._staging = {}
         ae = getattr(config, "__dict__", {}).get("async_encode", None)
@@ -112,6 +120,45 @@
         for e in self._all_engines():
             if getattr(e, "_tile_conv", None) != v:
                 e.set_option("tile_conv", v)
+
+    PREPARED_FRAMES = 34
+
+    def _prepare(self, f):
+        if not self._frame_prepare or f.net is None or not self.engine.can_gather(1) or f.h < 16 or f.w < 16:
+            return
+        opt = self._engine_options
+        if int(opt.get("presplit", 1)) == 0:
+            return
+        self._pin_kernels(f.h, f.w)
+        fits = self._prepare_ok.get((f.h, f.w))
+        if fits is None:
+            per_frame = f.h * f.w * 4096
+            need = self.PREPARED_FRAMES * per_frame
+            ws_bytes = int(ops._lib.load().mftx_raft_workspace_bytes_for(self.engine._h, self.nominal_pairs, f.h, f.w))
+            for k in range(self._fif):
+                e = self._lanes[k][0] if k < len(self._lanes) else (self.engine if k == 0 else None)
+                have = e._ws.numel() if e is not None and e._ws is not None else 0
+                need += max(0, ws_bytes - have)
+            free, total = torch.cuda.mem_get_info(self.device)
+            cached = torch.cuda.memory_reserved(self.device) - torch.cuda.memory_allocated(self.device)
+            fits = self._prepare_ok[(f.h, f.w)] = need <= free + cached - total // 10
+            if not fits:
+                logger.warning("frame_prepare: %.1f MB of prepared parts per cached frame of %d x %d cells do not fit beside the "
+                               "workspaces (%.1f GB free): computing them per pair", per_frame / 1e6, f.h, f.w, (free + cached) / 1e9)
+        if not fits:
+            return
+        context = getattr(self.engine, "_tile_conv", 1) == 2 and int(opt.get("fuse_gru", 1)) != 0
+        f.ctx, f.fsplit = self.engine.prepare_frame(f.fmap, f.inp, f.h, f.w, context=context, split=True)
+
+    def _prepared(self, fls, frs, flow_init):
+        if not self._frame_prepare or flow_init is not None:
+            return None
+        ctx = [f.ctx for f in fls] if all(f.ctx is not None for f in fls) and getattr(self.engine, "_tile_conv", 1) == 2 else None
+        f1s = [f.fsplit for f in fls] if all(f.fsplit is not None for f in fls) else None
+        f2s = frs[0].fsplit if all(f is frs[0] for f in frs) else None
+        if ctx is None and f1s is None and f2s is None:
+            return None
+        return {"ctx": ctx, "f1s": f1s, "f2s": f2s}
 
     def _all_engines(self):
         return list(dict.fromkeys([self.engine] + list(self._engines) + [e for e, _ in self._lanes]))
@@ -326,11 +373,13 @@
         for k in [k for k in self._frames if k not in keep]:
             del self._frames[k]
 
-    def _encode(self, img):
+    def _encode(self, img, prepare=False):
         if self._enc_stream is None:
             cur = torch.cuda.current_stream()
             self._encode_begin(cur)
             f = self.encode(img)
+            if prepare:
+                self._prepare(f)
             f.ready = cur.record_event()
             self._encode_end(f.ready, cur)
             return f
@@ -338,18 +387,21 @@
         if self._enc_waits_for_device_frames and isinstance(img, torch.Tensor) and img.is_cuda:
             self._encode_begin(main)
             f = self.encode(img)
+            if prepare:
+                self._prepare(f)
             f.ready = main.record_event()
             self._encode_end(f.ready, main)
             return f
         self._encode_begin(self._enc_stream)
         with torch.cuda.stream(self._enc_stream):
             f = self.encode(img)
+            if prepare:
+                self._prepare(f)
             f.ready = self._enc_stream.record_event()
         self._encode_end(f.ready, self._enc_stream)
         main.wait_stream(self._enc_stream)
-        for t in (f.fmap, f.net, f.inp):
-            if t is not None:
-                t.record_stream(main)
+        for t in f.tensors():
+            t.record_stream(main)
         return f
 
     def _encode_begin(self, stream):
@@ -365,7 +417,7 @@
             return self._encode(img)
         f = self._frames.get(key)
         if f is None or f.shape != img.shape[:2]:
-            f = self._encode(img)
+            f = self._encode(img, prepare=True)
             self._frames[key] = f
         return f
 
@@ -394,9 +446,11 @@
         packed = None
         H0, W0 = ref.shape
         want_planar = planar or packed_out is None or packed_out is False
+        self._pin_kernels(ref.h, ref.w)
+        prepared = self._prepared(fls, frs, flow_init) if gather else None
         if (self._fif > 1 and gather and flow_init is None and not self._check_finite
                 and (packed_out is None or isinstance(packed_out, bool))):
-            return self._refine_on_lane(fls, frs, fmap1, fmap2, net, inp, ref, iters, bool(packed_out), want_planar)
+            return self._refine_on_lane(fls, frs, fmap1, fmap2, net, inp, ref, iters, bool(packed_out), want_planar, prepared)
         if packed_out is not None and packed_out is not False:
             packed = packed_out if isinstance(packed_out, torch.Tensor) else \
                 torch.empty(P, H0, W0, 4, dtype=torch.float32, device=self.device)
@@ -409,7 +463,7 @@
             flow, occl, sigma = self._refine_split(fmap1, fmap2, net, inp, ref, iters, packed, want_planar)
         else:
             flow, occl, sigma = self.engine.refine(fmap1, fmap2, net, inp, ref.h, ref.w, iters, pads=ref.pads,
-                                                   flow_init=flow_init, packed=packed, planar=want_planar)
+                                                   flow_init=flow_init, packed=packed, planar=want_planar, prepared=prepared)
         if self._check_finite:
             bad = sum(ops.count_not_below(t.reshape(-1), float("inf")) for t in (packed, flow, occl, sigma) if t is not None)
             if bad:
@@ -423,7 +477,7 @@
             return [(flow[i], occl[i], sigma[i], packed[i]) for i in range(P)]
         return [(flow[i], occl[i], sigma[i]) for i in range(P)]
 
-    def _refine_on_lane(self, fls, frs, fmap1, fmap2, net, inp, geom, iters, want_packed, planar):
+    def _refine_on_lane(self, fls, frs, fmap1, fmap2, net, inp, geom, iters, want_packed, planar, prepared=None):
         P = len(fls)
         H0, W0 = geom.shape
         self._lanes_fit(P, geom.h, geom.w)
@@ -439,13 +493,12 @@
                 st.wait_event(f.ready)
             else:
                 st.wait_stream(main)
-            for t in (f.fmap, f.net, f.inp):
-                if t is not None:
-                    t.record_stream(st)
+            for t in f.tensors():
+                t.record_stream(st)
         with torch.cuda.stream(st):
             packed = torch.empty(P, H0, W0, 4, dtype=torch.float32, device=self.device) if want_packed else None
             flow, occl, sigma = eng.refine(fmap1, fmap2, net, inp, geom.h, geom.w, iters, pads=geom.pads,
-                                           flow_init=None, packed=packed, planar=planar)
+                                           flow_init=None, packed=packed, planar=planar, prepared=prepared)
             done = st.record_event()
         main.wait_event(done)
         self._ahead.append(done)
```

Result: faster. 190.0 frames/s, median of 6 (+1.6%).
